# UCL-CCS/Nbed

Measured on AMD Instinct MI355X. Metric: embedded_scf_cycles_per_sec, higher is better.
Workload: dtype f64

## Files before the change

### include/nbx.h

```cpp
#ifndef NBX_H
#define NBX_H

#include <stddef.h>
#include <stdint.h>

#ifdef __cplusplus
extern "C" {
#endif

#define NBX_VERSION 3

#define NBX_OK 0
#define NBX_E_INVALID (-1)
#define NBX_E_HIP (-2)
#define NBX_E_NOMEM (-3)
#define NBX_E_NOCONV (-4)
#define NBX_E_UNSUPPORTED (-5)

typedef struct nbx_ctx nbx_ctx;

int nbx_version(void);
int nbx_experimental(void);
const char* nbx_last_error(void);
int nbx_device_count(int* count);
// ... 10 lines not shown
int nbx_memcpy_d2d(nbx_ctx* ctx, void* d_dst, const void* d_src, size_t bytes);
int nbx_memset(nbx_ctx* ctx, void* d_ptr, int value, size_t bytes);

size_t nbx_jk_df_worksize(int64_t nao, int64_t ndm, int64_t nocc_max);
int nbx_jk_df(nbx_ctx* ctx, int64_t nao, int64_t naux, const double* d_b, int64_t ndm, const double* d_c,
              const int64_t* nocc, double* d_jk, void* d_work, size_t work_bytes);
int nbx_df_synth(nbx_ctx* ctx, int64_t nao, int64_t l0, int64_t l1, uint64_t seed, double scale, double* d_b);

#define NBX_PROF_JK_DENSE 0
#define NBX_PROF_AO2MO_Q1 1
#define NBX_PROF_AO2MO 2
#define NBX_PROF_EIGH 3
#define NBX_PROF_SVD 4
#define NBX_PROF_GEMM 5
#define NBX_PROF_LOC 6
int nbx_profile_enable(nbx_ctx* ctx, int on);
int nbx_profile_sample(nbx_ctx* ctx, int every);
int nbx_debug_fill_lds(nbx_ctx* ctx, double value);
int nbx_profile_read(nbx_ctx* ctx, int slot, double* ms_sum, int64_t* count);
int nbx_profile_reset(nbx_ctx* ctx);

int nbx_synth_eri(nbx_ctx* ctx, int64_t nao, int64_t p0, int64_t p1, uint64_t seed, double* d_eri);

size_t nbx_jk_dense_worksize(int64_t nao, int64_t np, int64_t ndm);
int nbx_jk_dense(nbx_ctx* ctx, int64_t nao, int64_t p0, int64_t p1, const double* d_eri,
                 const double* d_dm, int64_t ndm, double* d_jk, void* d_work, size_t work_bytes);

size_t nbx_jk_dense_sym_worksize(int64_t nao, int64_t p0, int64_t p1, int64_t ndm);
int nbx_jk_dense_sym(nbx_ctx* ctx, int64_t nao, int64_t p0, int64_t p1, const double* d_eri,
                     const double* d_dm, int64_t ndm, double* d_jk, void* d_work, size_t work_bytes);

int nbx_jk_packed_supported(int64_t nao);
int nbx_jk_packed_fold(int64_t nao);
size_t nbx_eri_packed_bytes(int64_t nao, int64_t p0, int64_t p1);
int nbx_eri_pack(nbx_ctx* ctx, int64_t nao, int64_t p0, int64_t p1, const double* d_eri, double* d_packed);
size_t nbx_jk_packed_worksize(int64_t nao, int64_t p0, int64_t p1, int64_t ndm);
int nbx_jk_packed(nbx_ctx* ctx, int64_t nao, int64_t p0, int64_t p1, const double* d_packed,
                  const double* d_dm, int64_t ndm, double* d_jk, void* d_work, size_t work_bytes);

size_t nbx_jk_dts_bytes(int64_t nao);
int nbx_jk_dts_init(nbx_ctx* ctx, int64_t nao, double* d_dts);
int nbx_jk_packed_fock(nbx_ctx* ctx, int64_t nao, const double* d_packed, const double* d_dm,
                       const double* d_hv, double* d_jk, double* d_fock, double* d_vhf, void* d_work,
                       size_t work_bytes, const double* d_dts);

int nbx_jk_synth(nbx_ctx* ctx, int64_t nao, int64_t p0, int64_t p1, uint64_t seed, const double* d_dm,
                 int64_t ndm, double* d_jk, void* d_work, size_t work_bytes);

size_t nbx_jk_synth_sym_worksize(int64_t nao, int64_t p0, int64_t p1, int64_t ndm);
int nbx_jk_synth_sym(nbx_ctx* ctx, int64_t nao, int64_t p0, int64_t p1, uint64_t seed,
                     const double* d_dm, int64_t ndm, double* d_jk, void* d_work, size_t work_bytes);

int nbx_gemm(nbx_ctx* ctx, char trans_a, char trans_b, int64_t m, int64_t n, int64_t k,
             double alpha, const double* d_a, int64_t lda, int64_t stride_a,
             const double* d_b, int64_t ldb, int64_t stride_b, double beta,
             double* d_c, int64_t ldc, int64_t stride_c, int64_t batch);

int nbx_fock_uhf(nbx_ctx* ctx, int64_t nao, const double* d_hcore, int hcore_ndim,
                 const double* d_vemb, const double* d_jk, double* d_fock, double* d_vhf);
int nbx_huzinaga_sym(nbx_ctx* ctx, int64_t nao, int64_t batch, const double* d_fds, double kappa,
                     double* d_hz, double* d_fock_io);
int nbx_huzinaga_fused(nbx_ctx* ctx, int64_t nao, int64_t batch, const double* d_f, const double* d_ds, double kappa,
                       double* d_hz, double* d_fock_out);
int nbx_trace_prod(nbx_ctx* ctx, int64_t nao, int64_t batch, const double* d_a, const double* d_b,
                   double* h_out);
int nbx_huz_cycle_scalars(nbx_ctx* ctx, int64_t nao, const double* d_hcore, int hcore_ndim,
                          const double* d_vemb, const double* d_vhf, const double* d_hz,
                          const double* d_dm, const double* d_dm_old, double* h_out);
int nbx_huz_cycle_scalars_dev(nbx_ctx* ctx, int64_t nao, const double* d_hcore, int hcore_ndim,
                              const double* d_vemb, const double* d_vhf, const double* d_hz,
                              const double* d_dm, const double* d_dm_old, double* d_out,
                              const int* d_tail, int64_t tail_n);
int nbx_huz_cycle_scalars_dts(nbx_ctx* ctx, int64_t nao, const double* d_hcore, int hcore_ndim,
                              const double* d_vemb, const double* d_vhf, const double* d_hz,
                              const double* d_dm, const double* d_dm_old, double* d_out, const int* d_tail,
                              int64_t tail_n, double* d_dts);
size_t nbx_diis_coef_doubles(int64_t space);
int nbx_diis_update(nbx_ctx* ctx, int64_t n, int64_t space, int64_t slot, int64_t nd,
                    const double* d_x, double* d_xprev, double* d_xs, double* d_es, double* d_h,
                    double* d_coef);
int nbx_diis_update_err(nbx_ctx* ctx, int64_t n, int64_t space, int64_t slot, int64_t nd,
                        const double* d_x, const double* d_err, double* d_xprev, double* d_xs,
                        double* d_es, double* d_h, double* d_coef);
int nbx_vo_sumsq(nbx_ctx* ctx, int64_t nao, const double* d_fmo, int64_t nocc_a, int64_t nocc_b,
                 double* d_out);
int nbx_axpby(nbx_ctx* ctx, int64_t n, double a, const double* d_x, double b, double* d_y);
int nbx_lincomb(nbx_ctx* ctx, int64_t n, int64_t nvec, const double* h_coef, const double* d_vecs,
                int64_t stride, double* d_out);
int nbx_dots(nbx_ctx* ctx, int64_t n, int64_t nvec, const double* d_x, const double* d_vecs,
             int64_t stride, double* h_out);
int nbx_transpose(nbx_ctx* ctx, int64_t rows, int64_t cols, int64_t batch, const double* d_a,
                  double* d_b);
int nbx_scale_cols(nbx_ctx* ctx, int64_t rows, int64_t cols, int64_t batch, const double* d_s,
                   double* d_a);

size_t nbx_eigh_worksize(int64_t n, int64_t batch);
int nbx_eigh(nbx_ctx* ctx, int64_t n, int64_t batch, const double* d_a, double* d_w, double* d_v,
             void* d_work, size_t work_bytes);
int nbx_eigh_warm(nbx_ctx* ctx, int64_t n, int64_t batch, const double* d_a, const double* d_v0,
                  double* d_w, double* d_v, void* d_work, size_t work_bytes);
int nbx_eigh_warm_ex(nbx_ctx* ctx, int64_t n, int64_t batch, const double* d_a, const double* d_v0,
                     double* d_w, double* d_v, void* d_work, size_t work_bytes, int refine_iters);
size_t nbx_eigh_status_offset(int64_t n, int64_t batch);
int nbx_eigh_status(nbx_ctx* ctx, int64_t n, int64_t batch, const void* d_work, int* h_sweeps);
size_t nbx_eigh_approx_worksize(int64_t n, int64_t batch);
int nbx_eigh_approx(nbx_ctx* ctx, int64_t n, int64_t batch, const double* d_a, double* d_w, double* d_v,
                    void* d_work, size_t work_bytes, int* d_status);
size_t nbx_sym_pow_worksize(int64_t n);
size_t nbx_sym_pow_ns_worksize(int64_t n);
int nbx_sym_pow_ns(nbx_ctx* ctx, int64_t n, const double* d_s, double p, double c, double* d_out, void* d_work,
                   size_t work_bytes, int max_iter, int check_every, int* h_iters);
int nbx_sym_pow(nbx_ctx* ctx, int64_t n, const double* d_s, double p, double* d_out,
                void* d_work, size_t work_bytes);

size_t nbx_svd_worksize(int64_t m, int64_t n);
int nbx_svd_right(nbx_ctx* ctx, int64_t m, int64_t n, const double* d_a, double* d_s, double* d_vt,
                  void* d_work, size_t work_bytes);
size_t nbx_geig_refine_worksize(int64_t n, int64_t batch);
int nbx_geig_refine(nbx_ctx* ctx, int64_t n, int64_t batch, const double* d_f, const double* d_s,
                    const double* d_c0, double* d_w, double* d_c, int* d_status, void* d_work,
                    size_t work_bytes, int max_iter);

size_t nbx_ao2mo_pair_sym_worksize(int64_t nao, int64_t n, int64_t n4, int64_t n6);
size_t nbx_eri_rs_bytes(int64_t nao);
int nbx_eri_pack_rs(nbx_ctx* ctx, int64_t nao, const double* d_eri, double* d_out);
size_t nbx_ao2mo_pair_sym_rs_worksize(int64_t nao, int64_t n, int64_t n4, int64_t n6);
int nbx_ao2mo_pair_sym_rs(nbx_ctx* ctx, int64_t nao, const double* d_eri_rs, const double* d_c12, int64_t n,
                          const double* d_c3, int64_t n3, const double* d_c4, int64_t n4, double* d_out,
                          const double* d_c5, int64_t n5, const double* d_c6, int64_t n6, double* d_out2,
                          void* d_work, size_t work_bytes);
int nbx_ao2mo_pair_sym(nbx_ctx* ctx, int64_t nao, const double* d_eri, const double* d_c12, int64_t n,
                       const double* d_c3, int64_t n3, const double* d_c4, int64_t n4, double* d_out,
                       const double* d_c5, int64_t n5, const double* d_c6, int64_t n6, double* d_out2,
                       void* d_work, size_t work_bytes);

int nbx_svd_status(nbx_ctx* ctx, int64_t m, int64_t n, const void* d_work, int* h_sweeps);

#define NBX_LOC_PM 0
#define NBX_LOC_BOYS 1
size_t nbx_loc_worksize(int kind, int batch, int64_t nao, int64_t n, int64_t natm);
int nbx_loc_pm(nbx_ctx* ctx, int batch, int64_t nao, int64_t n, int64_t natm, const int64_t* h_ao_offsets,
               const double* d_x, const double* d_y, double* d_u, int max_sweeps, double tol, void* d_work,
               size_t work_bytes);
int nbx_loc_boys(nbx_ctx* ctx, int batch, int64_t n, const double* d_q, double* d_u, int max_sweeps, double tol,
                 void* d_work, size_t work_bytes);
int nbx_loc_status(nbx_ctx* ctx, int batch, const void* d_work, int* h_sweeps, double* h_f);

size_t nbx_ao2mo_worksize(int64_t nao, int64_t ni, int64_t n2, int64_t n3, int64_t n4);
int nbx_ao2mo(nbx_ctx* ctx, int64_t nao, const double* d_eri, const double* d_c1, int64_t n1,
              int64_t i0, int64_t i1, const double* d_c2, int64_t n2, const double* d_c3,
              int64_t n3, const double* d_c4, int64_t n4, double* d_out, void* d_work,
              size_t work_bytes);
size_t nbx_ao2mo_pair_worksize(int64_t nao, int64_t ni, int64_t n2, int64_t n4, int64_t n6);
int nbx_ao2mo_pair(nbx_ctx* ctx, int64_t nao, const double* d_eri, const double* d_c1, int64_t n1,
                   int64_t i0, int64_t i1, const double* d_c2, int64_t n2, const double* d_c3,
                   int64_t n3, const double* d_c4, int64_t n4, double* d_out, const double* d_c5,
                   int64_t n5, const double* d_c6, int64_t n6, double* d_out2, void* d_work,
                   size_t work_bytes);
size_t nbx_ao2mo_synth_worksize(int64_t nao, int64_t n1, int64_t n2, int64_t n3, int64_t n4);
size_t nbx_ao2mo_synth_pair_worksize(int64_t nao, int64_t n1, int64_t n2, int64_t n3, int64_t n4,
                                     int64_t n5, int64_t n6);
int nbx_ao2mo_synth_pair(nbx_ctx* ctx, int64_t nao, uint64_t seed, int64_t r0, int64_t r1,
                         const double* d_c1, int64_t n1, const double* d_c2, int64_t n2,
                         const double* d_c3, int64_t n3, const double* d_c4, int64_t n4, double* d_out,
                         const double* d_c5, int64_t n5, const double* d_c6, int64_t n6, double* d_out2,
                         void* d_work, size_t work_bytes);
// ... 104 lines not shown
```

### nbed_amd/_nbx.py

```python

from __future__ import annotations

import ctypes
import os
from ctypes import POINTER, c_char, c_char_p, c_double, c_int, c_int64, c_size_t, c_uint64, c_void_p
from pathlib import Path

LIB_NAME = "libnbx.so"
LIB_PATH = Path(__file__).resolve().parent / LIB_NAME

NBX_VERSION = 3
NBX_OK = 0
NBX_E_INVALID = -1
NBX_E_HIP = -2
NBX_E_NOMEM = -3
NBX_E_NOCONV = -4
NBX_E_UNSUPPORTED = -5
LOC_PM, LOC_BOYS = 0, 1

HUZ_JK_PACKED, HUZ_JK_SYM = 0, 1
XC_CODES = {"slater": 0, "lda": 1, "lda,vwn_rpa": 1, "lda,vwn": 2, "lda,vwn5": 2, "svwn": 2, "b3lyp": 3}

PROF_JK_DENSE, PROF_AO2MO_Q1, PROF_AO2MO, PROF_EIGH, PROF_SVD, PROF_GEMM = range(6)


class NbxError(RuntimeError):

    def __init__(self, code: int, message: str):
        super().__init__(f"libnbx error {code}: {message}")
        self.code = code


class NbxUnavailableError(RuntimeError):
    """libnbx.so is not built or no MI355X is visible: the HIP path cannot run."""


class HuzState(ctypes.Structure):

    _fields_ = [
        ("nao", c_int64), ("nocc_a", c_int64), ("nocc_b", c_int64),
        ("d_packed", c_void_p), ("d_hv", c_void_p), ("d_ds", c_void_p), ("d_sb", c_void_p), ("d_x", c_void_p),
        ("d_dts", c_void_p), ("d_jk", c_void_p), ("d_fock", c_void_p), ("d_vhf", c_void_p), ("d_fock2", c_void_p),
        ("d_tmp", c_void_p), ("d_fo", c_void_p),
        ("d_jk_work", c_void_p), ("jk_work_bytes", c_size_t),
        ("d_eig_work", c_void_p), ("eig_work_bytes", c_size_t),
        ("d_geig_work", c_void_p), ("geig_work_bytes", c_size_t),
        ("diis_space", c_int64), ("d_diis_xs", c_void_p), ("d_diis_es", c_void_p), ("d_diis_h", c_void_p),
        ("d_diis_coef", c_void_p), ("d_diis_xprev", c_void_p),
        ("jk_kind", c_int64), ("jk_p0", c_int64), ("jk_p1", c_int64), ("d_eri", c_void_p),
    ]


_P = c_void_p
SIGNATURES = {
    "nbx_version": (c_int, []),
    "nbx_experimental": (c_int, []),
    "nbx_last_error": (c_char_p, []),
    "nbx_device_count": (c_int, [POINTER(c_int)]),
    "nbx_ctx_create": (c_int, [c_int, _P, c_int, POINTER(_P)]),
    "nbx_ctx_destroy": (c_int, [_P]),
    "nbx_ctx_set_stream": (c_int, [_P, _P]),
    "nbx_sync": (c_int, [_P]),
    "nbx_malloc": (c_int, [_P, c_size_t, POINTER(_P)]),
    "nbx_free": (c_int, [_P, _P]),
    "nbx_memcpy_h2d": (c_int, [_P, _P, _P, c_size_t]),
    "nbx_memcpy_d2h": (c_int, [_P, _P, _P, c_size_t]),
    "nbx_gather_to_host": (c_int, [_P, c_int64, _P, _P, _P, c_int]),
    "nbx_jk_df_worksize": (c_size_t, [c_int64, c_int64, c_int64]),
    "nbx_jk_df": (c_int, [_P, c_int64, c_int64, _P, c_int64, _P, POINTER(c_int64), _P, _P, c_size_t]),
    "nbx_df_synth": (c_int, [_P, c_int64, c_int64, c_int64, c_uint64, c_double, _P]),
    "nbx_memcpy_d2d": (c_int, [_P, _P, _P, c_size_t]),
    "nbx_memset": (c_int, [_P, _P, c_int, c_size_t]),
    "nbx_profile_enable": (c_int, [_P, c_int]),
    "nbx_profile_sample": (c_int, [_P, c_int]),
    "nbx_debug_fill_lds": (c_int, [_P, c_double]),
    "nbx_profile_read": (c_int, [_P, c_int, POINTER(c_double), POINTER(c_int64)]),
    "nbx_profile_reset": (c_int, [_P]),
    "nbx_synth_eri": (c_int, [_P, c_int64, c_int64, c_int64, c_uint64, _P]),
    "nbx_jk_dense_worksize": (c_size_t, [c_int64, c_int64, c_int64]),
    "nbx_jk_dense": (c_int, [_P, c_int64, c_int64, c_int64, _P, _P, c_int64, _P, _P, c_size_t]),
    "nbx_jk_dense_sym_worksize": (c_size_t, [c_int64, c_int64, c_int64, c_int64]),
    "nbx_jk_packed_supported": (c_int, [c_int64]),
    "nbx_jk_packed_fold": (c_int, [c_int64]),
    "nbx_eri_packed_bytes": (c_size_t, [c_int64, c_int64, c_int64]),
    "nbx_eri_pack": (c_int, [_P, c_int64, c_int64, c_int64, _P, _P]),
    "nbx_jk_packed_worksize": (c_size_t, [c_int64, c_int64, c_int64, c_int64]),
    "nbx_huzinaga_fused": (c_int, [_P, c_int64, c_int64, _P, _P, c_double, _P, _P]),
    "nbx_jk_packed_fock": (c_int, [_P, c_int64, _P, _P, _P, _P, _P, _P, _P, c_size_t, _P]),
    "nbx_jk_dts_bytes": (c_size_t, [c_int64]),
    "nbx_jk_dts_init": (c_int, [_P, c_int64, _P]),
    "nbx_jk_packed": (c_int, [_P, c_int64, c_int64, c_int64, _P, _P, c_int64, _P, _P, c_size_t]),
    "nbx_jk_dense_sym": (c_int, [_P, c_int64, c_int64, c_int64, _P, _P, c_int64, _P, _P, c_size_t]),
    "nbx_jk_synth_sym_worksize": (c_size_t, [c_int64, c_int64, c_int64, c_int64]),
    "nbx_jk_synth_sym": (c_int, [_P, c_int64, c_int64, c_int64, c_uint64, _P, c_int64, _P, _P, c_size_t]),
    "nbx_jk_synth": (c_int, [_P, c_int64, c_int64, c_int64, c_uint64, _P, c_int64, _P, _P, c_size_t]),
    "nbx_gemm": (c_int, [_P, c_char, c_char, c_int64, c_int64, c_int64, c_double, _P, c_int64, c_int64,
                         _P, c_int64, c_int64, c_double, _P, c_int64, c_int64, c_int64]),
    "nbx_fock_uhf": (c_int, [_P, c_int64, _P, c_int, _P, _P, _P, _P]),
    "nbx_huzinaga_sym": (c_int, [_P, c_int64, c_int64, _P, c_double, _P, _P]),
    "nbx_trace_prod": (c_int, [_P, c_int64, c_int64, _P, _P, POINTER(c_double)]),
    "nbx_huz_cycle_scalars": (c_int, [_P, c_int64, _P, c_int, _P, _P, _P, _P, _P, POINTER(c_double)]),
    "nbx_huz_cycle_scalars_dev": (c_int, [_P, c_int64, _P, c_int, _P, _P, _P, _P, _P, _P, _P, c_int64]),
    "nbx_huz_cycle_scalars_dts": (c_int, [_P, c_int64, _P, c_int, _P, _P, _P, _P, _P, _P, _P, c_int64, _P]),
    "nbx_diis_coef_doubles": (c_size_t, [c_int64]),
    "nbx_diis_update": (c_int, [_P, c_int64, c_int64, c_int64, c_int64, _P, _P, _P, _P, _P, _P]),
    "nbx_diis_update_err": (c_int, [_P, c_int64, c_int64, c_int64, c_int64, _P, _P, _P, _P, _P, _P, _P]),
    "nbx_vo_sumsq": (c_int, [_P, c_int64, _P, c_int64, c_int64, _P]),
    "nbx_axpby": (c_int, [_P, c_int64, c_double, _P, c_double, _P]),
    "nbx_lincomb": (c_int, [_P, c_int64, c_int64, POINTER(c_double), _P, c_int64, _P]),
    "nbx_dots": (c_int, [_P, c_int64, c_int64, _P, _P, c_int64, POINTER(c_double)]),
    "nbx_transpose": (c_int, [_P, c_int64, c_int64, c_int64, _P, _P]),
    "nbx_scale_cols": (c_int, [_P, c_int64, c_int64, c_int64, _P, _P]),
    "nbx_eigh_worksize": (c_size_t, [c_int64, c_int64]),
    "nbx_eigh": (c_int, [_P, c_int64, c_int64, _P, _P, _P, _P, c_size_t]),
    "nbx_eigh_warm": (c_int, [_P, c_int64, c_int64, _P, _P, _P, _P, _P, c_size_t]),
    "nbx_geig_refine_worksize": (c_size_t, [c_int64, c_int64]),
    "nbx_geig_refine": (c_int, [_P, c_int64, c_int64, _P, _P, _P, _P, _P, _P, _P, c_size_t, c_int]),
    "nbx_eigh_warm_ex": (c_int, [_P, c_int64, c_int64, _P, _P, _P, _P, _P, c_size_t, c_int]),
    "nbx_eigh_status_offset": (c_size_t, [c_int64, c_int64]),
    "nbx_eigh_approx_worksize": (c_size_t, [c_int64, c_int64]),
    "nbx_eigh_approx": (c_int, [_P, c_int64, c_int64, _P, _P, _P, _P, c_size_t, _P]),
    "nbx_eigh_status": (c_int, [_P, c_int64, c_int64, _P, POINTER(c_int)]),
    "nbx_sym_pow_worksize": (c_size_t, [c_int64]),
    "nbx_sym_pow": (c_int, [_P, c_int64, _P, c_double, _P, _P, c_size_t]),
    "nbx_sym_pow_ns_worksize": (c_size_t, [c_int64]),
    "nbx_sym_pow_ns": (c_int, [_P, c_int64, _P, c_double, c_double, _P, _P, c_size_t, c_int, c_int, POINTER(c_int)]),
    "nbx_svd_worksize": (c_size_t, [c_int64, c_int64]),
    "nbx_svd_right": (c_int, [_P, c_int64, c_int64, _P, _P, _P, _P, c_size_t]),
    "nbx_svd_status": (c_int, [_P, c_int64, c_int64, _P, POINTER(c_int)]),
    "nbx_loc_worksize": (c_size_t, [c_int, c_int, c_int64, c_int64, c_int64]),
    "nbx_loc_pm": (c_int, [_P, c_int, c_int64, c_int64, c_int64, _P, _P, _P, _P, c_int, c_double, _P, c_size_t]),
    "nbx_loc_boys": (c_int, [_P, c_int, c_int64, _P, _P, c_int, c_double, _P, c_size_t]),
    "nbx_loc_status": (c_int, [_P, c_int, _P, POINTER(c_int), POINTER(c_double)]),
    "nbx_ao2mo_worksize": (c_size_t, [c_int64, c_int64, c_int64, c_int64, c_int64]),
    "nbx_ao2mo": (c_int, [_P, c_int64, _P, _P, c_int64, c_int64, c_int64, _P, c_int64, _P, c_int64, _P,
                          c_int64, _P, _P, c_size_t]),
    "nbx_ao2mo_pair_worksize": (c_size_t, [c_int64, c_int64, c_int64, c_int64, c_int64]),
    "nbx_ao2mo_pair": (c_int, [_P, c_int64, _P, _P, c_int64, c_int64, c_int64, _P, c_int64, _P, c_int64, _P, c_int64,
                               _P, _P, c_int64, _P, c_int64, _P, _P, c_size_t]),
    "nbx_ao2mo_pair_sym_worksize": (c_size_t, [c_int64, c_int64, c_int64, c_int64]),
    "nbx_ao2mo_pair_sym": (c_int, [_P, c_int64, _P, _P, c_int64, _P, c_int64, _P, c_int64, _P, _P, c_int64, _P, c_int64,
                                   _P, _P, c_size_t]),
    "nbx_eri_rs_bytes": (c_size_t, [c_int64]),
    "nbx_eri_pack_rs": (c_int, [_P, c_int64, _P, _P]),
    "nbx_ao2mo_pair_sym_rs_worksize": (c_size_t, [c_int64, c_int64, c_int64, c_int64]),
    "nbx_ao2mo_pair_sym_rs": (c_int, [_P, c_int64, _P, _P, c_int64, _P, c_int64, _P, c_int64, _P, _P, c_int64, _P,
                                      c_int64, _P, _P, c_size_t]),
    "nbx_ao2mo_synth_pair_worksize": (c_size_t, [c_int64] * 7),
    "nbx_ao2mo_synth_pair": (c_int, [_P, c_int64, c_uint64, c_int64, c_int64, _P, c_int64, _P, c_int64, _P, c_int64,
                                     _P, c_int64, _P, _P, c_int64, _P, c_int64, _P, _P, c_size_t]),
    "nbx_ao2mo_synth_worksize": (c_size_t, [c_int64, c_int64, c_int64, c_int64, c_int64]),
    "nbx_ao2mo_synth": (c_int, [_P, c_int64, c_uint64, c_int64, c_int64, _P, c_int64, _P, c_int64, _P, c_int64, _P,
                                c_int64, _P, _P, c_size_t]),
    "nbx_chem_to_phys": (c_int, [_P, c_int64, c_int64, c_int64, c_int64, _P, _P]),
    "nbx_spinorb_scatter_h1": (c_int, [_P, c_int64, _P, c_double, _P]),
    "nbx_spinorb_scatter_range": (c_int, [_P, c_int64, _P, c_double, c_double, c_int64, c_int64, _P]),
    "nbx_spinorb_scatter": (c_int, [_P, c_int64, _P, _P, c_double, c_double, _P, _P]),
    "nbx_threshold_scale": (c_int, [_P, c_int64, c_double, c_double, _P]),
    "nbx_becke_share": (c_int, [_P, c_int64, _P, c_int64, _P, _P, _P, c_int64, _P]),
    "nbx_eval_ao": (c_int, [_P, c_int64, _P, c_int64, _P, _P, _P, _P, _P, c_int64, c_int64, _P, _P]),
    "nbx_xc_rho": (c_int, [_P, c_int64, c_int64, _P, _P, _P, _P, _P]),
    "nbx_xc_functional_worksize": (c_size_t, [c_int64]),
    "nbx_xc_functional": (c_int, [_P, c_int, c_int64, _P, _P, _P, c_double, _P, _P, _P, _P, c_size_t]),
    "nbx_xc_vmat_worksize": (c_size_t, [c_int64, c_int64]),
    "nbx_xc_vmat": (c_int, [_P, c_int64, c_int64, _P, _P, _P, _P, _P, _P, c_size_t]),
    "nbx_purify_worksize": (c_size_t, [c_int64, c_int64]),
    "nbx_purify": (c_int, [_P, c_int64, c_int64, _P, c_int64, c_int64, _P, _P, c_size_t, c_int, _P]),
    "nbx_host_1e": (c_int, [c_int, _P, _P, _P, _P, _P, _P, _P, c_int, _P, _P, c_int, _P, _P, _P]),
    "nbx_host_eri": (c_int, [c_int, _P, _P, _P, _P, _P, _P, _P, c_double, c_int, _P]),
    "nbx_host_dipole": (c_int, [c_int, _P, _P, _P, _P, _P, _P, _P, c_int, _P]),
    "nbx_huz_cycle": (c_int, [_P, POINTER(HuzState), _P, _P, _P, _P, _P, _P, _P, c_int, c_int, c_int, c_int, c_int,
                              c_int, _P, _P]),
    "nbx_huz_cycle_jk": (c_int, [_P, POINTER(HuzState), _P]),
    "nbx_mu_cycle": (c_int, [_P, POINTER(HuzState), _P, _P, _P, _P, _P, _P, _P, _P, _P, c_int, c_int, c_int, c_int, c_int,
                             c_int, _P, _P]),
    "nbx_mu_cycle_solve": (c_int, [_P, POINTER(HuzState), _P, _P, _P, _P, _P, _P, _P, c_int, c_int, c_int, c_int, c_int,
                                   _P]),
    "nbx_mu_cycle_fock": (c_int, [_P, POINTER(HuzState), _P, _P, _P, _P, _P, c_int, _P, _P]),
    "nbx_mu_cycle_fock_post": (c_int, [_P, POINTER(HuzState), _P, _P, _P, _P, _P, c_int, _P, _P]),
    "nbx_huz_cycle_post": (c_int, [_P, POINTER(HuzState), _P, _P, _P, _P, _P, _P, _P, c_int, c_int, c_int, c_int, c_int,
                                   _P, _P]),
}

_lib = None


def load_library(path: os.PathLike | None = None) -> ctypes.CDLL:
    global _lib
    if _lib is not None and path is None:
# ... 34 lines not shown
```

### nbed_amd/backend.py

```python

from __future__ import annotations

import ctypes
import os
import time
from ctypes import c_double, c_int

import numpy as np

from . import _nbx
from ._nbx import NbxError, NbxUnavailableError

_default_backend = None


def get_backend(device: int | None = None):
    global _default_backend
    if _default_backend is None:
        _default_backend = HipBackend(device)
    return _default_backend


def set_backend(backend) -> None:
    global _default_backend
# ... 660 lines not shown
                       int(refine_iters), int(diis_mode), int(diis_slot), int(diis_nd), self._p(h_out),
                       self._p(out["status"]))
        return _PendingScalars(self.torch, None, 2, host=h_out)

    def mu_cycle_state(self, nao, nelec, packed, h1e, s_b, x, eri=None, p0: int = 0, p1: int | None = None):
        return self.huz_cycle_state(nao, nelec, packed, h1e, None, s_b, x, None, diis_space=8, eri=eri, p0=p0, p1=p1)

    def _pin_slot(self, n: int):
        h_out = self._pin_ring[self._pin_next][:n]
        h_out[n - 1] = 0.0
        self._pin_next = (self._pin_next + 1) % self._PIN_SLOTS
        return h_out

    def mu_cycle(self, h, dm_in, fock_in, c_in, out, tracked: bool, refine_iters: int, diis_on: bool, diis_slot: int,
                 diis_nd: int, want_grad: bool = True, reduce=None):
        ndt = 2 if want_grad else 0
        h_out = self._pin_slot(4 + 2 + ndt + 1)
        mode = 1 if tracked else 0
        if reduce is None:
            self._call("nbx_mu_cycle", ctypes.byref(h.st), self._p(dm_in), self._p(fock_in), self._p(c_in),
                       self._p(out["dm"]), self._p(out["fock"]), self._p(out["vhf"]), self._p(out["c"]), self._p(out["v"]),
                       self._p(out["w"]), mode, int(refine_iters), 1 if diis_on else 0, int(diis_slot), int(diis_nd),
                       1 if want_grad else 0, self._p(h_out), self._p(out["status"]))
        else:
            self._call("nbx_mu_cycle_solve", ctypes.byref(h.st), self._p(dm_in), self._p(fock_in), self._p(c_in),
                       self._p(out["dm"]), self._p(out["c"]), self._p(out["v"]), self._p(out["w"]), mode,
                       int(refine_iters), 1 if diis_on else 0, int(diis_slot), int(diis_nd), self._p(out["status"]))
            self._call("nbx_huz_cycle_jk", ctypes.byref(h.st), self._p(out["dm"]))
            reduce(h.jk)
            self._call("nbx_mu_cycle_fock_post", ctypes.byref(h.st), self._p(out["dm"]), self._p(dm_in),
                       self._p(out["c"]) if want_grad else None, self._p(out["fock"]), self._p(out["vhf"]), mode,
                       self._p(out["status"]), self._p(h_out))
        return _PendingScalars(self.torch, None, 2, host=h_out, ndtail=ndt)

    def mu_cycle_fock(self, h, dm, out, reduce=None):
        h_out = self._pin_slot(4 + 1)
        if reduce is None:
            self._call("nbx_mu_cycle_fock", ctypes.byref(h.st), self._p(dm), self._p(dm), None, self._p(out["fock"]),
                       self._p(out["vhf"]), -1, None, self._p(h_out))
        else:
            self._call("nbx_huz_cycle_jk", ctypes.byref(h.st), self._p(dm))
            reduce(h.jk)
            self._call("nbx_mu_cycle_fock_post", ctypes.byref(h.st), self._p(dm), self._p(dm), None,
                       self._p(out["fock"]), self._p(out["vhf"]), -1, None, self._p(h_out))
        return _PendingScalars(self.torch, None, 0, host=h_out)

    def df_synth(self, nao: int, l0: int, l1: int, scale: float | None = None, seed: int | None = None):
        from . import synth

        out = self.empty((l1 - l0, nao, nao))
        chunk = 32768
        for a in range(l0, l1, chunk):
            b = min(l1, a + chunk)
            self._call("nbx_df_synth", nao, a, b, int(synth.SEED if seed is None else seed),
                       float(synth.df_scale(nao) if scale is None else scale), self._p(out[a - l0:]))
        return out

    def jk_df(self, b, c, nocc):
        c3 = c if c.dim() == 3 else c.unsqueeze(0)
        ndm, n = int(c3.shape[0]), int(c3.shape[-1])
        occ = [int(x) for x in (nocc if hasattr(nocc, "__len__") else [nocc])]
        if len(occ) != ndm:
            raise ValueError(f"jk_df: {ndm} coefficient matrices but {len(occ)} occupation counts")
        out = self.empty((1 + ndm, n, n))
        nbytes = int(self.lib.nbx_jk_df_worksize(n, ndm, max(occ) if occ else 0))
        work = self._workspace("jk_df", nbytes)
        self._call("nbx_jk_df", n, int(b.shape[0]), self._p(b), ndm, self._p(c3), (ctypes.c_int64 * ndm)(*occ), self._p(out),
                   self._p(work), nbytes)
        return out

    def async_to_host(self, d_vals):
        return _PendingScalars(self.torch, d_vals, 0, ncore=int(d_vals.numel()))

    def diis_coef_buffer(self, space: int):
        return self.zeros(int(self.lib.nbx_diis_coef_doubles(space)))

    def diis_update(self, space: int, slot: int, nd: int, x, xprev, xs, es, h, coef):
        self._call("nbx_diis_update", x.numel(), space, slot, nd, self._p(x), self._p(xprev), self._p(xs),
                   self._p(es), self._p(h), self._p(coef))
        return xprev

    def diis_update_err(self, space: int, slot: int, nd: int, x, err, out, xs, es, h, coef):
        self._call("nbx_diis_update_err", x.numel(), space, slot, nd, self._p(x), self._p(err), self._p(out),
                   self._p(xs), self._p(es), self._p(h), self._p(coef))
        return out

    def vo_sumsq(self, fmo, nocc):
        out = self.empty(2)
        self._call("nbx_vo_sumsq", fmo.shape[-1], self._p(fmo), int(nocc[0]), int(nocc[1]), self._p(out))
        return out

    def axpby(self, a: float, x, b: float, y):
        self._call("nbx_axpby", x.numel(), a, self._p(x), b, self._p(y))
        return y

    def add(self, x, y):
        out = y.clone()
        return self.axpby(1.0, x, 1.0, out)

    def lincomb(self, coef, vecs, out=None):
        nvec, n = vecs.shape[0], vecs[0].numel()
        if out is None:
            out = self.empty(vecs.shape[1:])
        c = (c_double * nvec)(*[float(x) for x in coef])
        self._call("nbx_lincomb", n, nvec, c, self._p(vecs), n, self._p(out))
        return out

    def dots(self, x, vecs) -> np.ndarray:
        nvec, n = vecs.shape[0], x.numel()
        out = (c_double * nvec)()
        self._call("nbx_dots", n, nvec, self._p(x), self._p(vecs), vecs[0].numel(), out)
        return np.array(out[:], dtype=np.float64)

    def transpose(self, a):
        if a.dim() == 2:
            rows, cols, batch = a.shape[0], a.shape[1], 1
            out = self.empty((cols, rows))
        else:
            batch, rows, cols = a.shape
            out = self.empty((batch, cols, rows))
        self._call("nbx_transpose", rows, cols, batch, self._p(a), self._p(out))
        return out

    def scale_cols(self, a, s):
        rows, cols = a.shape[-2], a.shape[-1]
        batch = 1 if a.dim() == 2 else a.shape[0]
        self._call("nbx_scale_cols", rows, cols, batch, self._p(s), self._p(a))
        return a

    def eigh(self, a, check: bool = False, v0=None, refine_iters: int = 3):
        n = a.shape[-1]
        batch = 1 if a.dim() == 2 else a.shape[0]
        nbytes = self.lib.nbx_eigh_worksize(n, batch)
        work = self._workspace("eigh", nbytes)
        w = self.empty(a.shape[:-1])
        v = self.torch.empty_like(a)
        self._call("nbx_eigh_warm_ex", n, batch, self._p(a), self._p(v0), self._p(w), self._p(v), self._p(work),
                   work.numel(), int(refine_iters))
        off = self.lib.nbx_eigh_status_offset(n, batch)
        self.last_eigh_status_d = work[off:off + 4 * batch].view(self.torch.int32)
        if check:
            sweeps = (c_int * batch)()
            self._call("nbx_eigh_status", n, batch, self._p(work), sweeps)
            self.last_eigh_sweeps = list(sweeps)
        return w, v

    def eigh_approx(self, a):
        torch = self.torch
        a3 = a if a.dim() == 3 else a.reshape(1, *a.shape)
        batch, n = int(a3.shape[0]), int(a3.shape[-1])
        nbytes = int(self.lib.nbx_eigh_approx_worksize(n, batch))
        work = self._workspace("eigh_approx", nbytes)
        w = self.empty(a.shape[:-1])
        v = torch.empty_like(a)
        status = torch.empty(batch, dtype=torch.int32, device=self.device)
        self._call("nbx_eigh_approx", n, batch, self._p(a), self._p(w), self._p(v), self._p(work), nbytes, self._p(status))
        return w, v, status

    def geig_refine(self, fock, ovlp_b, c0, refine_iters: int = 1):
        n = fock.shape[-1]
        batch = 1 if fock.dim() == 2 else fock.shape[0]
        nbytes = self.lib.nbx_geig_refine_worksize(n, batch)
        work = self._workspace("geig", nbytes)
        w = self.empty(fock.shape[:-1])
        c = self.torch.empty_like(fock)
        status = self.torch.empty(batch, dtype=self.torch.int32, device=self.device)
# ... 346 lines not shown
```

### nbed_amd/csrc/ctx.hip

```cpp
#include "nbx_common.h"

static thread_local char g_err[512] = "";

void nbx_set_error(const char* fmt, ...) {
    va_list ap;
    va_start(ap, fmt);
    vsnprintf(g_err, sizeof(g_err), fmt, ap);
    va_end(ap);
}

extern "C" {

int nbx_version(void) { return NBX_VERSION; }

int nbx_experimental(void) {
#ifdef NBX_EXPERIMENTAL
    return 1;
#else
    return 0;
#endif
}

const char* nbx_last_error(void) { return g_err; }

int nbx_device_count(int* count) {
    NBX_CHECK_ARG(count != nullptr);
    int n = 0;
    hipError_t e = hipGetDeviceCount(&n);
    if (e != hipSuccess) {
        *count = 0;
        nbx_set_error("nbx_device_count: %s", hipGetErrorString(e));
        (void)hipGetLastError();
        return NBX_E_HIP;
    }
    *count = n;
    return NBX_OK;
}

int nbx_ctx_create(int device, void* stream, int private_stream, nbx_ctx** out) {
    NBX_CHECK_ARG(out != nullptr);
    NBX_CHECK_ARG(device >= 0);
    int n = 0;
    NBX_HIP(hipGetDeviceCount(&n));
    if (device >= n) {
        nbx_set_error("nbx_ctx_create: device %d not present (%d visible)", device, n);
        return NBX_E_INVALID;
    }
    NBX_HIP(hipSetDevice(device));
    {
        int lds_per_cu = 0;
        NBX_HIP(hipDeviceGetAttribute(&lds_per_cu, hipDeviceAttributeMaxSharedMemoryPerMultiprocessor, device));
        if (lds_per_cu <= 0 || lds_per_cu > 0x28000) {
            nbx_set_error("nbx_ctx_create: device %d reports %d bytes of LDS per CU; libnbx is built for gfx950 (163840) and "
                          "its packed J/K kernel relies on reads beyond 0x30000 returning zero", device, lds_per_cu);
            return NBX_E_UNSUPPORTED;
        }
    }
    nbx_ctx* c = new nbx_ctx();
    c->device = device;
    c->own_stream = (private_stream != 0);
    if (c->own_stream) {
        hipError_t e = hipStreamCreateWithFlags(&c->stream, hipStreamNonBlocking);
        if (e != hipSuccess) {
            delete c;
            nbx_set_error("nbx_ctx_create: hipStreamCreate -> %s", hipGetErrorString(e));
            return NBX_E_HIP;
        }
    } else {
        c->stream = reinterpret_cast<hipStream_t>(stream);
    }
    c->d_scratch = nullptr;
    c->h_pinned = nullptr;
    c->d_counters = nullptr;
    if (hipMalloc(reinterpret_cast<void**>(&c->d_scratch), NBX_SCRATCH_DOUBLES * sizeof(double)) != hipSuccess ||
        hipHostMalloc(reinterpret_cast<void**>(&c->h_pinned), NBX_SCRATCH_DOUBLES * sizeof(double), 0) != hipSuccess ||
        hipMalloc(reinterpret_cast<void**>(&c->d_counters), NBX_COUNTERS * sizeof(int)) != hipSuccess ||
        hipMemsetAsync(c->d_counters, 0, NBX_COUNTERS * sizeof(int), c->stream) != hipSuccess) {
        nbx_set_error("nbx_ctx_create: scratch allocation failed");
        if (c->d_scratch) (void)hipFree(c->d_scratch);
        if (c->h_pinned) (void)hipHostFree(c->h_pinned);
        if (c->d_counters) (void)hipFree(c->d_counters);
        if (c->own_stream) (void)hipStreamDestroy(c->stream);
        delete c;
        return NBX_E_NOMEM;
    }
    *out = c;
    return NBX_OK;
}

int nbx_ctx_destroy(nbx_ctx* ctx) {
    if (ctx == nullptr) return NBX_OK;
    (void)hipSetDevice(ctx->device);
    (void)hipStreamSynchronize(ctx->stream);
    (void)nbx_profile_reset(ctx);
    if (ctx->d_scratch) (void)hipFree(ctx->d_scratch);
    if (ctx->h_pinned) (void)hipHostFree(ctx->h_pinned);
    if (ctx->d_counters) (void)hipFree(ctx->d_counters);
    if (ctx->own_stream) (void)hipStreamDestroy(ctx->stream);
    delete ctx;
    return NBX_OK;
}

int nbx_ctx_set_stream(nbx_ctx* ctx, void* stream) {
    NBX_CHECK_ARG(ctx != nullptr);
    if (ctx->own_stream) {
        (void)hipStreamSynchronize(ctx->stream);
        (void)hipStreamDestroy(ctx->stream);
        ctx->own_stream = false;
    }
    ctx->stream = reinterpret_cast<hipStream_t>(stream);
    return NBX_OK;
}

int nbx_sync(nbx_ctx* ctx) {
    NBX_CHECK_ARG(ctx != nullptr);
    NBX_HIP(hipStreamSynchronize(ctx->stream));
    return NBX_OK;
}

int nbx_malloc(nbx_ctx* ctx, size_t bytes, void** d_ptr) {
    NBX_CHECK_ARG(ctx != nullptr && d_ptr != nullptr);
    NBX_HIP(hipSetDevice(ctx->device));
    hipError_t e = hipMalloc(d_ptr, bytes ? bytes : 8);
    if (e != hipSuccess) {
        nbx_set_error("nbx_malloc(%zu bytes): %s", bytes, hipGetErrorString(e));
        (void)hipGetLastError();
        return NBX_E_NOMEM;
    }
    return NBX_OK;
}

int nbx_free(nbx_ctx* ctx, void* d_ptr) {
    NBX_CHECK_ARG(ctx != nullptr);
    if (d_ptr == nullptr) return NBX_OK;
    NBX_HIP(hipFree(d_ptr));
    return NBX_OK;
}

int nbx_memcpy_h2d(nbx_ctx* ctx, void* d_dst, const void* h_src, size_t bytes) {
    NBX_CHECK_ARG(ctx != nullptr && (bytes == 0 || (d_dst != nullptr && h_src != nullptr)));
    if (bytes == 0) return NBX_OK;
    NBX_HIP(hipMemcpyAsync(d_dst, h_src, bytes, hipMemcpyHostToDevice, ctx->stream));
// ... 148 lines not shown
```

### nbed_amd/csrc/eigh_refine.hip

```cpp
#include "nbx_common.h"

namespace {

constexpr int RF_THREADS = 256;
constexpr int RF_WGS = 16;
constexpr int RF_MAX_ITER = 6;
constexpr int RF_UNROLL = 4;
constexpr double RF_TOL = 3.0e-8;
constexpr double RF_GIVE_UP = 0.25;
constexpr double RF_CLUSTER_NOISE = 1.0e-14;
constexpr double RF_NOISE = 8.0 * 1.1102230246251565e-16;
constexpr int RF_PART = 6;

__device__ __forceinline__ void publish(double* p, double v) {
    __hip_atomic_store(p, v, __ATOMIC_RELAXED, __HIP_MEMORY_SCOPE_AGENT);
}
__device__ __forceinline__ double peek(const double* p) {
    return __hip_atomic_load(p, __ATOMIC_RELAXED, __HIP_MEMORY_SCOPE_AGENT);
}

__global__ __launch_bounds__(RF_THREADS) void refine_e_kernel(int N, const double* __restrict__ A,
                                                              const double* __restrict__ S,
                                                              const double* __restrict__ G, double* __restrict__ Ep,
                                                              double* __restrict__ lam_out, int* __restrict__ status,
                                                              double* __restrict__ norm_a, int iter, int max_iter,
                                                              double* __restrict__ partial, int* __restrict__ counters,
                                                              int* __restrict__ final_status = nullptr,
                                                              const double* __restrict__ norm_part = nullptr,
                                                              int norm_tiles = 0) {
    extern __shared__ double sm[];
    double* lam = sm;
    double* red = sm + N;
    const int b = blockIdx.y, wg = blockIdx.x, nwg = gridDim.x;
    if (iter > 0 && status[b] != 0) return;
    const int64_t n2 = (int64_t)N * N;
    if (A != nullptr) A += b * n2;
    S += b * n2;
    G += b * n2;
    Ep += b * n2;
    double* part = partial + (int64_t)b * nwg * RF_PART;
    int* counter = counters + b;
    for (int i = threadIdx.x; i < N; i += RF_THREADS) lam[i] = S[(int64_t)i * N + i] / G[(int64_t)i * N + i];
    const int wave = threadIdx.x >> 6, lane = threadIdx.x & 63;
    constexpr int NW = RF_THREADS / 64;
    const int total = N * N;
    const int first = wg * RF_THREADS + threadIdx.x, stride = nwg * RF_THREADS;
    const float inv_n = 1.0f / (float)N;
    auto row_of = [&](int e) {
        int i = (int)((float)e * inv_n);
        i -= (i * N > e) ? 1 : 0;
        i += ((i + 1) * N <= e) ? 1 : 0;
        return i;
    };
    double off2 = 0.0, r2 = 0.0, a2 = 0.0;
    if (norm_part != nullptr) {
        const double* ps = norm_part + (int64_t)b * 2 * norm_tiles * 2;
        const double* pg = ps + (int64_t)norm_tiles * 2;
        for (int w = threadIdx.x; w < norm_tiles; w += RF_THREADS) {
            off2 += ps[2 * w];
            a2 += ps[2 * w + 1];
            r2 += pg[2 * w];
        }
    }
    __syncthreads();
    for (int e0 = first; e0 < total && norm_part == nullptr; e0 += stride * RF_UNROLL) {
        double sv[RF_UNROLL], gv[RF_UNROLL], av[RF_UNROLL];
#pragma unroll
        for (int u = 0; u < RF_UNROLL; ++u) {
            const int e = e0 + u * stride;
            const bool in = e < total;
            sv[u] = in ? S[e] : 0.0;
            gv[u] = in ? G[e] : 0.0;
            av[u] = (in && iter == 0) ? (A != nullptr ? A[e] : sv[u]) : 0.0;
        }
#pragma unroll
        for (int u = 0; u < RF_UNROLL; ++u) {
            const int e = e0 + u * stride;
            if (e < total) {
                const int i = row_of(e), j = e - i * N;
                const double r = (i == j) ? 1.0 - gv[u] : -gv[u];
                if (i != j) {
                    const double n1 = fabs(sv[u] - lam[j] * gv[u]), n2 = fabs(sv[u] - lam[i] * gv[u]);
                    const double nm = fmin(n1, n2);
                    off2 = fma(nm, nm, off2);
                }
                r2 = fma(r, r, r2);
                a2 = fma(av[u], av[u], a2);
            }
        }
    }
    off2 = nbx_wave_sum_dpp(off2);
    r2 = nbx_wave_sum_dpp(r2);
    a2 = nbx_wave_sum_dpp(a2);
    __syncthreads();
    if (lane == 0) {
        red[wave] = off2;
        red[NW + wave] = r2;
        red[2 * NW + wave] = a2;
    }
    __syncthreads();
    if (threadIdx.x == 0 && norm_part != nullptr) {
        double t0 = 0.0, t1 = 0.0, t2 = 0.0;
        for (int w = 0; w < NW; ++w) {
            t0 += red[w];
            t1 += red[NW + w];
            t2 += red[2 * NW + w];
        }
        red[3 * NW + 3] = 0.0;
        red[3 * NW + 0] = t0;
        red[3 * NW + 1] = t1;
        red[3 * NW + 2] = t2;
    } else if (threadIdx.x == 0) {
        double t0 = 0.0, t1 = 0.0, t2 = 0.0;
        for (int w = 0; w < NW; ++w) {
            t0 += red[w];
            t1 += red[NW + w];
            t2 += red[2 * NW + w];
        }
        publish(part + wg * RF_PART + 0, t0);
        publish(part + wg * RF_PART + 1, t1);
        publish(part + wg * RF_PART + 2, t2);
        __hip_atomic_fetch_add(counter, 1, __ATOMIC_RELEASE, __HIP_MEMORY_SCOPE_AGENT);
        int spins = 0;
        while (__hip_atomic_load(counter, __ATOMIC_ACQUIRE, __HIP_MEMORY_SCOPE_AGENT) < nwg && ++spins < (1 << 20))
            __builtin_amdgcn_s_sleep(2);
        red[3 * NW + 3] = (spins >= (1 << 20)) ? 1.0 : 0.0;
        t0 = t1 = t2 = 0.0;
        for (int w = 0; w < nwg; ++w) {
            t0 += peek(part + w * RF_PART + 0);
            t1 += peek(part + w * RF_PART + 1);
            t2 += peek(part + w * RF_PART + 2);
        }
        red[3 * NW + 0] = t0;
        red[3 * NW + 1] = t1;
        red[3 * NW + 2] = t2;
    }
    int unsorted = 0;
    if (final_status != nullptr)
        for (int i = threadIdx.x + 1; i < N; i += RF_THREADS) unsorted |= lam[i - 1] > lam[i] ? 1 : 0;
    unsorted = __syncthreads_or(unsorted);
    off2 = red[3 * NW + 0];
    r2 = red[3 * NW + 1];
    a2 = red[3 * NW + 2];
    double na;
    if (iter == 0) {
        na = sqrt(a2);
        if (wg == 0 && threadIdx.x == 0) norm_a[b] = na;
    } else {
        na = norm_a[b];
    }
    const double om_s = 2.0 * sqrt(off2), om_r = 2.0 * sqrt(r2);
    double emax = 0.0, cmax = 0.0, nmax = 0.0;
    for (int e0 = first; e0 < total; e0 += stride * RF_UNROLL) {
        double sv[RF_UNROLL], gv[RF_UNROLL], st[RF_UNROLL];
        int ri[RF_UNROLL];
#pragma unroll
        for (int u = 0; u < RF_UNROLL; ++u) {
            const int e = e0 + u * stride;
            const bool in = e < total;
            ri[u] = in ? row_of(e) : 0;
            sv[u] = in ? S[e] : 0.0;
            gv[u] = in ? G[e] : 0.0;
            st[u] = in ? S[(int64_t)(e - ri[u] * N) * N + ri[u]] : 0.0;
        }
#pragma unroll
        for (int u = 0; u < RF_UNROLL; ++u) {
            const int e = e0 + u * stride;
            if (e < total) {
                const int i = ri[u], j = e - i * N;
                const double sx = 0.5 * (sv[u] + st[u]), g = gv[u];
                double ev;
                if (i == j) {
                    ev = 0.5 * (1.0 - g);
                    emax = fmax(emax, fabs(ev));
                    Ep[e] = 1.0 + ev;
                } else {
                    const double li = lam[i], lj = lam[j];
                    const double d = lj - li;
                    if (fabs(d) > om_s + fmax(fabs(li), fabs(lj)) * om_r) {
                        const double num = sx - lj * g;
                        ev = num / d;
                        nmax = fmax(nmax, fabs(num));
                    } else {
                        ev = -0.5 * g;
                        cmax = fmax(cmax, fabs(sx));
                    }
                    emax = fmax(emax, fabs(ev));
                    Ep[e] = ev;
                }
            }
        }
    }
    emax = -nbx_wave_min_dpp(-emax);
    cmax = -nbx_wave_min_dpp(-cmax);
    nmax = -nbx_wave_min_dpp(-nmax);
    __syncthreads();
    if (lane == 0) {
        red[wave] = emax;
        red[NW + wave] = cmax;
        red[2 * NW + wave] = nmax;
    }
    __syncthreads();
    if (threadIdx.x == 0) {
        for (int w = 0; w < NW; ++w) {
            emax = fmax(emax, red[w]);
            cmax = fmax(cmax, red[NW + w]);
            nmax = fmax(nmax, red[2 * NW + w]);
        }
        if (red[3 * NW + 3] != 0.0) emax = 1.0e300;
        publish(part + wg * RF_PART + 3, emax);
        publish(part + wg * RF_PART + 4, cmax);
        publish(part + wg * RF_PART + 5, nmax);
        const int arrived = __hip_atomic_fetch_add(counter, 1, __ATOMIC_ACQ_REL, __HIP_MEMORY_SCOPE_AGENT);
        if (arrived == (norm_part != nullptr ? 1 : 2) * nwg - 1) {
            for (int w = 0; w < nwg; ++w) {
                emax = fmax(emax, peek(part + w * RF_PART + 3));
                cmax = fmax(cmax, peek(part + w * RF_PART + 4));
                nmax = fmax(nmax, peek(part + w * RF_PART + 5));
            }
            const bool at_noise = nmax <= RF_NOISE * sqrt((double)N) * na && emax < 1.0e-3;
            int st = 0;
            if (!(emax < RF_GIVE_UP)) st = -1;
            else if ((emax < RF_TOL || at_noise) && cmax <= RF_CLUSTER_NOISE * na) st = iter + 1;
            else if (iter == max_iter - 1) st = -1;
            if (final_status != nullptr) {
                if (st > 0 && unsorted) st = -3;
                final_status[b] = st > 0 ? 1000 + st : (st < 0 ? st : -2);
            }
            status[b] = st;
            __hip_atomic_store(counter, 0, __ATOMIC_RELEASE, __HIP_MEMORY_SCOPE_AGENT);
        }
    }
    if (wg == 0)
        for (int i = threadIdx.x; i < N; i += RF_THREADS) lam_out[(int64_t)b * N + i] = lam[i];
}

constexpr int RF_ROWS = 8;
__global__ __launch_bounds__(256) void refine_finish_kernel(int N, const double* __restrict__ xb0,
                                                            const double* __restrict__ xb1,
                                                            const double* __restrict__ lam_in,
                                                            const int* __restrict__ status, double* __restrict__ w,
                                                            double* __restrict__ v, int* __restrict__ jacobi_status) {
    extern __shared__ double sm[];
    double* lam = sm;
    int* rank = reinterpret_cast<int*>(sm + N);
    const int b = blockIdx.y;
    const int st = status[b];
    if (st <= 0) {
        if (blockIdx.x == 0 && threadIdx.x == 0 && jacobi_status != nullptr) jacobi_status[b] = st < 0 ? st : -2;
        return;
    }
    const int64_t n2 = (int64_t)N * N;
    const double* X = ((st & 1) ? xb1 : xb0) + b * n2;
    for (int i = threadIdx.x; i < N; i += blockDim.x) lam[i] = lam_in[(int64_t)b * N + i];
    __syncthreads();
    int unsorted = 0;
    for (int i = threadIdx.x + 1; i < N; i += blockDim.x) unsorted |= lam[i - 1] > lam[i] ? 1 : 0;
    unsorted = __syncthreads_or(unsorted);
    for (int i = threadIdx.x; i < N; i += blockDim.x) {
        const double li = lam[i];
        int r = i;
        if (unsorted) {
            r = 0;
            for (int j = 0; j < N; ++j) {
                const double lj = lam[j];
                r += (lj < li || (lj == li && j < i)) ? 1 : 0;
            }
        }
        rank[i] = r;
        if (blockIdx.x == 0) w[(int64_t)b * N + r] = li;
    }
    if (blockIdx.x == 0 && threadIdx.x == 0 && jacobi_status != nullptr) jacobi_status[b] = 1000 + st;
    __syncthreads();
    const int r0 = blockIdx.x * RF_ROWS;
    for (int rr = 0; rr < RF_ROWS; ++rr) {
        const int r = r0 + rr;
        if (r >= N) break;
        for (int i = threadIdx.x; i < N; i += blockDim.x)
            v[b * n2 + (int64_t)r * N + rank[i]] = X[(int64_t)r * N + i];
    }
}

size_t align256(size_t x) { return (x + 255) & ~(size_t)255; }

struct RefineLayout {
    size_t xb0, xb1, y, s, g, ep, lam, norm, partial, status, npart, total;
};

RefineLayout rlayout(int64_t n, int64_t batch) {
    RefineLayout L;
    const size_t mat = align256((size_t)(n * n * batch) * sizeof(double));
    size_t off = 0;
    L.xb0 = off; off += mat;
    L.xb1 = off; off += mat;
    L.y = off; off += mat;
    L.s = off; off += mat;
    L.g = off; off += mat;
    L.ep = off; off += mat;
    L.lam = off; off += align256((size_t)(n * batch) * sizeof(double));
    L.norm = off; off += align256((size_t)batch * sizeof(double));
    L.partial = off; off += align256((size_t)(batch * RF_WGS * RF_PART) * sizeof(double));
    L.status = off; off += align256((size_t)batch * sizeof(int));
    L.npart = off; off += align256((size_t)nbx_gemm_small_norm_doubles(n, n, batch) * sizeof(double));
    L.total = off;
    return L;
}

}

bool nbx_eigh_refine_supported(int64_t n, int64_t batch) {
    return n >= 2 && n <= 4096 && batch <= NBX_COUNTERS;
}

size_t nbx_eigh_refine_worksize(int64_t n, int64_t batch) { return rlayout(n, batch).total; }

int nbx_eigh_refine(nbx_ctx* ctx, int64_t n, int64_t batch, const double* d_a, const double* d_v0, double* d_w,
                    double* d_v, void* d_work, int* d_jacobi_status, const int** d_status_out, int max_iter) {
    NBX_CHECK_ARG(max_iter >= 1 && max_iter <= RF_MAX_ITER);
    const RefineLayout L = rlayout(n, batch);
    char* base = static_cast<char*>(d_work);
    double* xb[2] = {reinterpret_cast<double*>(base + L.xb0), reinterpret_cast<double*>(base + L.xb1)};
    double* y = reinterpret_cast<double*>(base + L.y);
    double* s = reinterpret_cast<double*>(base + L.s);
    double* g = reinterpret_cast<double*>(base + L.g);
    double* ep = reinterpret_cast<double*>(base + L.ep);
    double* lam = reinterpret_cast<double*>(base + L.lam);
    double* norm = reinterpret_cast<double*>(base + L.norm);
    double* partial = reinterpret_cast<double*>(base + L.partial);
    int* status = reinterpret_cast<int*>(base + L.status);
    double* npart = reinterpret_cast<double*>(base + L.npart);
    const int norm_tiles = (int)(nbx_cdiv(n, 16) * nbx_cdiv(n, 16));
    const int64_t n2 = n * n;
    const bool small = nbx_gemm_small_supported(n, n, n, batch);
    for (int it = 0; it < max_iter; ++it) {
        const double* src = (it == 0) ? d_v0 : xb[it & 1];
        double* dst = xb[(it + 1) & 1];
        const int* gate = (it == 0) ? nullptr : status;
        int rc = nbx_gemm_gated(ctx, 'N', 'N', n, n, n, 1.0, d_a, n, n2, src, n, n2, 0.0, y, n, n2, batch, gate, 0, 0);
        if (rc != NBX_OK) return rc;
        if (small) {
            rc = nbx_gemm_small_gated(ctx, 'T', 'N', n, n, n, 1.0, src, n, n2, y, n, n2, 0.0, s, n, n2, batch, gate, 0, 0,
                                      src, g, npart);
            if (rc != NBX_OK) return rc;
        } else {
            rc = nbx_gemm_gated(ctx, 'T', 'N', n, n, n, 1.0, src, n, n2, y, n, n2, 0.0, s, n, n2, batch, gate, 0, 0);
            if (rc != NBX_OK) return rc;
            rc = nbx_gemm_gated(ctx, 'T', 'N', n, n, n, 1.0, src, n, n2, src, n, n2, 0.0, g, n, n2, batch, gate, 0, 0);
            if (rc != NBX_OK) return rc;
        }
        hipLaunchKernelGGL(refine_e_kernel, dim3(RF_WGS, (unsigned)batch), dim3(RF_THREADS),
                           (size_t)(n + 3 * (RF_THREADS / 64) + 8) * sizeof(double), ctx->stream, (int)n, d_a, s, g, ep,
                           lam, status, norm, it, max_iter, partial, ctx->d_counters, static_cast<int*>(nullptr),
                           small ? npart : static_cast<const double*>(nullptr), norm_tiles);
        NBX_LAUNCH_CHECK();
        rc = nbx_gemm_gated(ctx, 'N', 'N', n, n, n, 1.0, src, n, n2, ep, n, n2, 0.0, dst, n, n2, batch, status, 0, it + 1);
        if (rc != NBX_OK) return rc;
    }
    hipLaunchKernelGGL(refine_finish_kernel, dim3((unsigned)nbx_cdiv(n, RF_ROWS), (unsigned)batch), dim3(256),
                       (size_t)n * sizeof(double) + (size_t)n * sizeof(int), ctx->stream, (int)n, xb[0], xb[1], lam,
                       status, d_w, d_v, d_jacobi_status);
    NBX_LAUNCH_CHECK();
    *d_status_out = status;
    return NBX_OK;
}

namespace {
struct GeigLayout {
    size_t cb0, cb1, yt, zt, s, g, ep, lam, norm, partial, status, npart, total;
};
GeigLayout glayout(int64_t n, int64_t batch) {
    GeigLayout L;
    const size_t mat = align256((size_t)(n * n * batch) * sizeof(double));
    size_t off = 0;
    L.cb0 = off; off += mat;
    L.cb1 = off; off += mat;
    L.yt = off; off += mat;
    L.zt = off; off += mat;
    L.s = off; off += mat;
    L.g = off; off += mat;
    L.ep = off; off += mat;
    L.lam = off; off += align256((size_t)(n * batch) * sizeof(double));
    L.norm = off; off += align256((size_t)batch * sizeof(double));
    L.partial = off; off += align256((size_t)(batch * RF_WGS * RF_PART) * sizeof(double));
    L.status = off; off += align256((size_t)batch * sizeof(int));
    L.npart = off; off += align256((size_t)nbx_gemm_small_norm_doubles(n, n, batch) * sizeof(double));
    L.total = off;
    return L;
}
}

extern "C" size_t nbx_geig_refine_worksize(int64_t n, int64_t batch) {
    if (n <= 0 || batch <= 0) return 0;
    return glayout(n, batch).total;
}

extern "C" int nbx_geig_refine(nbx_ctx* ctx, int64_t n, int64_t batch, const double* d_f, const double* d_s,
                               const double* d_c0, double* d_w, double* d_c, int* d_status, void* d_work,
                               size_t work_bytes, int max_iter) {
    NBX_CHECK_ARG(ctx && d_f && d_s && d_c0 && d_w && d_c && d_status);
    NBX_CHECK_ARG(n >= 2 && n <= 4096 && batch >= 1 && batch <= NBX_COUNTERS);
    NBX_CHECK_ARG(max_iter >= 1 && max_iter <= RF_MAX_ITER);
    const GeigLayout L = glayout(n, batch);
    if (d_work == nullptr || work_bytes < L.total) {
        nbx_set_error("nbx_geig_refine: workspace %zu < %zu bytes", work_bytes, L.total);
        return NBX_E_NOMEM;
    }
    char* base = static_cast<char*>(d_work);
    double* cb[2] = {reinterpret_cast<double*>(base + L.cb0), reinterpret_cast<double*>(base + L.cb1)};
    double* yt = reinterpret_cast<double*>(base + L.yt);
    double* zt = reinterpret_cast<double*>(base + L.zt);
    double* s = reinterpret_cast<double*>(base + L.s);
    double* g = reinterpret_cast<double*>(base + L.g);
    double* ep = reinterpret_cast<double*>(base + L.ep);
    double* lam = reinterpret_cast<double*>(base + L.lam);
    double* norm = reinterpret_cast<double*>(base + L.norm);
    double* partial = reinterpret_cast<double*>(base + L.partial);
    int* status = reinterpret_cast<int*>(base + L.status);
    double* npart = reinterpret_cast<double*>(base + L.npart);
    const int norm_tiles = (int)(nbx_cdiv(n, 16) * nbx_cdiv(n, 16));
    const int64_t n2 = n * n;
    const bool pair = nbx_gemm_small_supported(n, n, n, 2 * batch);
    const bool direct = max_iter == 1 && d_c != d_c0;
    for (int it = 0; it < max_iter; ++it) {
        const double* src = (it == 0) ? d_c0 : cb[it & 1];
        double* dst = direct ? d_c : cb[(it + 1) & 1];
        const int* gate = (it == 0) ? nullptr : status;
        int rc;
        if (pair) {
            rc = nbx_gemm_small_gated(ctx, 'T', 'N', n, n, n, 1.0, src, n, n2, d_f, n, n2, 0.0, yt, n, n2, batch, gate, 0,
                                      0, d_s, zt);
            if (rc != NBX_OK) return rc;
            rc = nbx_gemm_small_gated(ctx, 'T', 'T', n, n, n, 1.0, src, n, n2, yt, n, n2, 0.0, s, n, n2, batch, gate, 0, 0,
                                      zt, g, npart);
            if (rc != NBX_OK) return rc;
        } else {
            rc = nbx_gemm_gated(ctx, 'T', 'N', n, n, n, 1.0, src, n, n2, d_f, n, n2, 0.0, yt, n, n2, batch, gate, 0, 0);
            if (rc != NBX_OK) return rc;
            rc = nbx_gemm_gated(ctx, 'T', 'N', n, n, n, 1.0, src, n, n2, d_s, n, n2, 0.0, zt, n, n2, batch, gate, 0, 0);
            if (rc != NBX_OK) return rc;
            rc = nbx_gemm_gated(ctx, 'T', 'T', n, n, n, 1.0, src, n, n2, yt, n, n2, 0.0, s, n, n2, batch, gate, 0, 0);
            if (rc != NBX_OK) return rc;
            rc = nbx_gemm_gated(ctx, 'T', 'T', n, n, n, 1.0, src, n, n2, zt, n, n2, 0.0, g, n, n2, batch, gate, 0, 0);
            if (rc != NBX_OK) return rc;
        }
        hipLaunchKernelGGL(refine_e_kernel, dim3(RF_WGS, (unsigned)batch), dim3(RF_THREADS),
                           (size_t)(n + 3 * (RF_THREADS / 64) + 8) * sizeof(double), ctx->stream, (int)n,
                           static_cast<const double*>(nullptr), s, g, ep, direct ? d_w : lam, status, norm, it, max_iter,
                           partial, ctx->d_counters, direct ? d_status : static_cast<int*>(nullptr),
                           pair ? npart : static_cast<const double*>(nullptr), norm_tiles);
        NBX_LAUNCH_CHECK();
        rc = nbx_gemm_gated(ctx, 'N', 'N', n, n, n, 1.0, src, n, n2, ep, n, n2, 0.0, dst, n, n2, batch, status, 0, it + 1);
        if (rc != NBX_OK) return rc;
    }
    if (direct) return NBX_OK;
    hipLaunchKernelGGL(refine_finish_kernel, dim3((unsigned)nbx_cdiv(n, RF_ROWS), (unsigned)batch), dim3(256),
                       (size_t)n * sizeof(double) + (size_t)n * sizeof(int), ctx->stream, (int)n, cb[0], cb[1], lam,
                       status, d_w, d_c, d_status);
    NBX_LAUNCH_CHECK();
    return NBX_OK;
}
```

### nbed_amd/csrc/elementwise.hip

```cpp
#include "nbx_common.h"
#include "jk_m4_layout.h"
#include "jk_s4_layout.h"

namespace {

constexpr int TILE = 32;

__global__ void final_reduce_kernel(const double* __restrict__ partial, int nblocks, int nout,
                                    double* __restrict__ out, int sqrt_from, const int* __restrict__ tail = nullptr,
                                    int tail_n = 0) {
    __shared__ double red[17];
    if ((int)threadIdx.x < tail_n) out[nout + threadIdx.x] = (double)tail[threadIdx.x];
    for (int o = 0; o < nout; ++o) {
        double t = 0.0;
        for (int b = threadIdx.x; b < nblocks; b += blockDim.x) t += partial[(int64_t)b * nout + o];
        t = nbx_block_sum(t, red);
        if (threadIdx.x == 0) out[o] = (o >= sqrt_from) ? sqrt(t) : t;
        __syncthreads();
    }
}

__device__ __forceinline__ void load_tile(const double* __restrict__ M, int N, int r0, int c0,
                                          double (*lds)[TILE + 1]) {
    for (int r = threadIdx.y; r < TILE; r += blockDim.y) {
// ... 628 lines not shown
                    const double tmp = A0[k][lane];
                    A0[k][lane] = A0[piv][lane];
                    A0[piv][lane] = tmp;
                }
                if (lane == 0) {
                    const double tmp = rhs_s[k];
                    rhs_s[k] = rhs_s[piv];
                    rhs_s[piv] = tmp;
                }
            }
            __syncthreads();
            const double inv = 1.0 / A0[k][k];
            const int rem = m - 1 - k;
            double upd[DIIS_SLOTS];
            double rupd = 0.0;
#pragma unroll
            for (int e = 0; e < DIIS_SLOTS; ++e) {
                const int idx = lane + 64 * e;
                upd[e] = 0.0;
                if (idx < rem * rem) {
                    const int i = k + 1 + idx / rem, jj = k + 1 + idx % rem;
                    const double f = A0[i][k] * inv;
                    upd[e] = A0[i][jj] - f * A0[k][jj];
                }
            }
            if (lane < rem) {
                const double f = A0[k + 1 + lane][k] * inv;
                rupd = rhs_s[k + 1 + lane] - f * rhs_s[k];
            }
            __syncthreads();
#pragma unroll
            for (int e = 0; e < DIIS_SLOTS; ++e) {
                const int idx = lane + 64 * e;
                if (idx < rem * rem) A0[k + 1 + idx / rem][k + 1 + idx % rem] = upd[e];
            }
            if (lane < rem) rhs_s[k + 1 + lane] = rupd;
            __syncthreads();
        }
        __syncthreads();
        if (!lu_failed) {
            for (int i = m - 1; i >= 0; --i) {
                double t = (lane > i && lane < m) ? A0[i][lane] * c_out[lane] : 0.0;
                t = nbx_wave_sum(t);
                if (lane == 0) c_out[i] = (rhs_s[i] - t) / A0[i][i];
                __syncthreads();
            }
        }
        __syncthreads();
    }
    if (singular || lu_failed) {
        if (lane < m) {
            double t = 0.0;
            for (int k = 0; k < m; ++k)
                if (!singular || fabs(w[k]) > 1e-14) t += V[lane][k] * (1.0 / w[k]) * V[0][k];
            c_out[lane] = t;
        }
        __syncthreads();
    }
    if (lane >= 1 && lane < m) coef[lane - 1] = c_out[lane];
}

__device__ __forceinline__ void diis_rotation(double app, double aqq, double apq, double& cs, double& sn) {
    const double d = aqq - app, b = 2.0 * apq;
    const double inv = __builtin_amdgcn_rcp(fmax(fabs(d), fabs(b)));
    const double ds = d * inv, bs = b * inv;
    const float dsf = (float)ds, bsf = (float)bs;
    const float rt = __builtin_amdgcn_sqrtf(fmaf(dsf, dsf, bsf * bsf));
    const float den = dsf + (ds >= 0.0 ? rt : -rt);
    double t = (double)(bsf * __builtin_amdgcn_rcpf(den));
    const float rgp = __builtin_amdgcn_rcpf((float)fma(bs, t, ds));
    double g = fma(fma(bs, t, 2.0 * ds), t, -bs);
    t = fma(-0.5 * g, (double)rgp, t);
    g = fma(fma(bs, t, 2.0 * ds), t, -bs);
    t = fma(-0.5 * g, (double)rgp, t);
    const double x = fma(t, t, 1.0), h = 0.5 * x;
    double y = (double)__builtin_amdgcn_rsqf((float)x);
    y = y * fma(-(h * y), y, 1.5);
    y = y * fma(-(h * y), y, 1.5);
    const bool rot = fabs(apq) > 1e-290;
    cs = rot ? y : 1.0;
    sn = rot ? t * y : 0.0;
}

__device__ __forceinline__ void diis_jacobi8(double& a, double& v, int m, double fro, int lane, double* As,
                                             double* Vs) {
    const int r = lane >> 3, c = lane & 7;
    for (int sweep = 0; sweep < 40; ++sweep) {
        const double off = nbx_wave_sum_dpp((r < c) ? a * a : 0.0);
        if (off <= 1e-31 * fro) break;
        const double mind = nbx_wave_min_dpp((r == c && r < m) ? fabs(a) : 1.0e300);
        if (mind - sqrt(2.0 * off) > 1.0e-14) break;
#pragma unroll
        for (int step = 0; step < 7; ++step) {
            auto mate = [&](int k) {
                int x = 2 * step - k;
                x += x < 0 ? 7 : 0;
                x -= x >= 7 ? 7 : 0;
                return k == 7 ? step : (k == step ? 7 : x);
            };
            const int mc = mate(c), mr = mate(r);
            As[lane] = a;
            Vs[lane] = v;
            __syncthreads();
            const double a_cc = As[9 * c], a_mm = As[9 * mc], a_cm = As[8 * min(c, mc) + max(c, mc)];
            const double a_rr = As[9 * r], a_nn = As[9 * mr], a_rn = As[8 * min(r, mr) + max(r, mr)];
            const double a_rmc = As[8 * r + mc], a_mrc = As[8 * mr + c], a_mrmc = As[8 * mr + mc];
            const double v_rmc = Vs[8 * r + mc];
            __syncthreads();
            double cc, sc, cr, sr;
            diis_rotation(c < mc ? a_cc : a_mm, c < mc ? a_mm : a_cc, a_cm, cc, sc);
            diis_rotation(r < mr ? a_rr : a_nn, r < mr ? a_nn : a_rr, a_rn, cr, sr);
            const double ks_c = (c < mc) ? -sc : sc, ks_r = (r < mr) ? -sr : sr;
            const double x = cc * a + ks_c * a_rmc;
            const double y = cc * a_mrc + ks_c * a_mrmc;
            a = (ks_r != 0.0 && mr == c) ? 0.0 : cr * x + ks_r * y;
            v = cc * v + ks_c * v_rmc;
        }
    }
}

constexpr int DIIS8_PER_LANE = 4;
__global__ __launch_bounds__(64) void diis_solve8_lincomb_kernel(const double* __restrict__ partial, int nblocks,
                                                                 int nd, int slot, double* __restrict__ H, int ldh,
                                                                 double* __restrict__ coef,
                                                                 double* __restrict__ state, int64_t n,
                                                                 const double* __restrict__ vecs, int64_t stride,
                                                                 double* __restrict__ out) {
    __shared__ double As[64], Vs[64], Ts[64];
    __shared__ double A0[8][9], rhs_s[8], c_out[8];
    __shared__ int lu_failed;
    const int lane = threadIdx.x, r = lane >> 3, c = lane & 7;
    const int m = nd + 1;
    const int64_t i0 = (int64_t)blockIdx.x * (64 * DIIS8_PER_LANE) + lane;
    const bool inside = r < m && c < m;
    const bool new_row = inside && r == slot + 1 && c >= 1, new_col = inside && c == slot + 1 && r >= 1;
    const double hold = (inside && !new_row && !new_col) ? H[(int64_t)r * ldh + c] : 0.0;
    double xv[DIIS8_PER_LANE][7];
#pragma unroll
    for (int j = 0; j < DIIS8_PER_LANE; ++j)
#pragma unroll
        for (int k = 0; k < 7; ++k) xv[j][k] = (k < nd && i0 + 64 * j < n) ? vecs[k * stride + i0 + 64 * j] : 0.0;
    const double v_prev = state[lane];
    const bool warm = __double_as_longlong(state[64]) == DIIS_STATE_MAGIC && state[65] <= (double)(nd + 1);
    double acc = 0.0;
    if (c >= 1 && c <= nd) {
#pragma unroll 4
        for (int b = r; b < nblocks; b += 8) acc += partial[(int64_t)b * nd + c - 1];
    }
    As[lane] = acc;
    __syncthreads();
    double row_c = 0.0, row_r = 0.0;
#pragma unroll
    for (int g = 0; g < 8; ++g) {
        row_c += As[8 * g + c];
        row_r += As[8 * g + r];
    }
    __syncthreads();
    double a = new_row ? row_c : (new_col ? row_r : hold);
    if (blockIdx.x == 0 && (new_row || new_col)) H[(int64_t)r * ldh + c] = a;
    A0[r][c] = a;
    if (lane == 0) lu_failed = 0;
    double v = (r == c) ? 1.0 : 0.0;
    if (warm) {
        Vs[lane] = v_prev;
        __syncthreads();
        double gram = 0.0;
#pragma unroll
        for (int k = 0; k < 8; ++k) gram = fma(Vs[8 * k + r], Vs[8 * k + c], gram);
        Ts[lane] = gram;
        __syncthreads();
        double vg = 0.0;
#pragma unroll
        for (int k = 0; k < 8; ++k) vg = fma(Vs[8 * r + k], Ts[8 * k + c], vg);
        v = 1.5 * v_prev - 0.5 * vg;
        __syncthreads();
        Vs[lane] = v;
        As[lane] = a;
        __syncthreads();
        double hv = 0.0;
#pragma unroll
        for (int k = 0; k < 8; ++k) hv = fma(As[8 * r + k], Vs[8 * k + c], hv);
        Ts[lane] = hv;
        __syncthreads();
        double vhv = 0.0;
#pragma unroll
        for (int k = 0; k < 8; ++k) vhv = fma(Vs[8 * k + r], Ts[8 * k + c], vhv);
        __syncthreads();
        Ts[lane] = vhv;
        __syncthreads();
        a = 0.5 * (vhv + Ts[8 * c + r]);
        __syncthreads();
    }
    const double fro = nbx_wave_sum_dpp(a * a);
    diis_jacobi8(a, v, m, fro, lane, As, Vs);
    As[lane] = a;
    Vs[lane] = v;
    if (blockIdx.x == 0) {
        state[DIIS_STATE_HALF + lane] = v;
        if (lane == 0) state[DIIS_STATE_HALF + 64] = __longlong_as_double(DIIS_STATE_MAGIC);
        if (lane == 1) state[DIIS_STATE_HALF + 65] = (double)m;
    }
    __syncthreads();
    const bool singular = __any(r == c && r < m && fabs(a) < 1e-14);
    if (!singular) {
        if (lane < m) rhs_s[lane] = (lane == 0) ? 1.0 : 0.0;
        __syncthreads();
        for (int k = 0; k < m; ++k) {
            double best = (lane >= k && lane < m) ? fabs(A0[lane][k]) : -1.0;
            int piv = lane;
#pragma unroll
            for (int o = 4; o > 0; o >>= 1) {
                const double ob = __shfl_xor(best, o);
                const int op = __shfl_xor(piv, o);
                if (ob > best || (ob == best && op < piv)) {
                    best = ob;
                    piv = op;
                }
            }
            best = nbx_readlane_f64(best, 0);
            piv = __builtin_amdgcn_readlane(piv, 0);
            if (best == 0.0) {
                if (lane == 0) lu_failed = 1;
                break;
            }
            if (piv != k) {
                if (lane < m) {
                    const double tmp = A0[k][lane];
                    A0[k][lane] = A0[piv][lane];
                    A0[piv][lane] = tmp;
                }
                if (lane == 0) {
                    const double tmp = rhs_s[k];
                    rhs_s[k] = rhs_s[piv];
                    rhs_s[piv] = tmp;
                }
            }
            __syncthreads();
            const double inv = 1.0 / A0[k][k];
            const bool below = r > k && r < m, right = c > k && c < m;
            double upd = 0.0, rupd = 0.0;
            if (below && right) upd = A0[r][c] - (A0[r][k] * inv) * A0[k][c];
            if (below && c == 0) rupd = rhs_s[r] - (A0[r][k] * inv) * rhs_s[k];
            __syncthreads();
            if (below && right) A0[r][c] = upd;
            if (below && c == 0) rhs_s[r] = rupd;
            __syncthreads();
        }
        __syncthreads();
        if (!lu_failed) {
            for (int i = m - 1; i >= 0; --i) {
                const double t = nbx_wave_sum_dpp((lane > i && lane < m) ? A0[i][lane] * c_out[lane] : 0.0);
                if (lane == 0) c_out[i] = (rhs_s[i] - t) / A0[i][i];
                __syncthreads();
            }
        }
        __syncthreads();
    }
    if (singular || lu_failed) {
        const double w = As[9 * c], v0 = Vs[c];
        const bool keep = c < m && (!singular || fabs(w) > 1e-14);
        const double t = nbx_sum8_dpp(keep ? v * (1.0 / w) * v0 : 0.0);
        if (c == 0 && r < m) c_out[r] = t;
        __syncthreads();
    }
    if (blockIdx.x == 0 && lane >= 1 && lane < m) coef[lane - 1] = c_out[lane];
    double cf[7];
#pragma unroll
    for (int k = 0; k < 7; ++k) cf[k] = (k < nd) ? c_out[k + 1] : 0.0;
#pragma unroll
    for (int j = 0; j < DIIS8_PER_LANE; ++j) {
        const int64_t i = i0 + 64 * j;
        if (i < n) {
            double t = 0.0;
#pragma unroll
            for (int k = 0; k < 7; ++k)
                if (k < nd) t = fma(cf[k], xv[j][k], t);
            out[i] = t;
        }
    }
}

__global__ void lincomb_dev_kernel(int64_t n, int nvec, const double* __restrict__ coef,
                                   const double* __restrict__ vecs, int64_t stride, double* __restrict__ out) {
    for (int64_t i = (int64_t)blockIdx.x * blockDim.x + threadIdx.x; i < n; i += (int64_t)gridDim.x * blockDim.x) {
        double t = 0.0;
        for (int k = 0; k < nvec; ++k) t = fma(coef[k], vecs[k * stride + i], t);
        out[i] = t;
    }
}

__global__ void transpose_kernel(const double* __restrict__ A, double* __restrict__ B, int64_t rows, int64_t cols) {
    __shared__ double t[TILE][TILE + 1];
    const int64_t b = blockIdx.z;
    A += b * rows * cols;
    B += b * rows * cols;
    const int64_t r0 = (int64_t)blockIdx.y * TILE, c0 = (int64_t)blockIdx.x * TILE;
    for (int r = threadIdx.y; r < TILE; r += blockDim.y) {
        const int64_t gr = r0 + r, gc = c0 + threadIdx.x;
        if (gr < rows && gc < cols) t[r][threadIdx.x] = A[gr * cols + gc];
    }
    __syncthreads();
    for (int c = threadIdx.y; c < TILE; c += blockDim.y) {
        const int64_t gc = c0 + c, gr = r0 + threadIdx.x;
        if (gr < rows && gc < cols) B[gc * rows + gr] = t[threadIdx.x][c];
    }
}

__global__ void vo_sumsq_kernel(const double* __restrict__ fmo, int N, int nocc_a, int nocc_b,
                                double* __restrict__ partial) {
    __shared__ double red[17];
    const int x = blockIdx.y;
    const int nocc = x == 0 ? nocc_a : nocc_b;
    const int nvir = N - nocc;
    const int64_t total = (int64_t)nvir * nocc;
    double t = 0.0;
    for (int64_t e = (int64_t)blockIdx.x * blockDim.x + threadIdx.x; e < total; e += (int64_t)gridDim.x * blockDim.x) {
        const int a = nocc + (int)(e / nocc), i = (int)(e % nocc);
        const double v = fmo[((int64_t)x * N + a) * N + i];
        t = fma(v, v, t);
    }
    t = nbx_block_sum(t, red);
    if (threadIdx.x == 0) partial[(int64_t)blockIdx.x * 2 + x] = t;
}

__global__ void scale_cols_kernel(int64_t rows, int64_t cols, const double* __restrict__ s, double* __restrict__ a) {
    const int64_t b = blockIdx.y;
    const int64_t i = (int64_t)blockIdx.x * blockDim.x + threadIdx.x;
    if (i >= rows * cols) return;
    a[b * rows * cols + i] *= s[b * cols + (i % cols)];
}

__global__ void spinorb_h2_kernel(int n, const double* __restrict__ tb, double tol, double scale,
                                  double* __restrict__ h2, int64_t idx0, int64_t count) {
    const int64_t nq = 2 * (int64_t)n;
    const int64_t n4 = (int64_t)n * n * n * n;
    for (int64_t off = (int64_t)blockIdx.x * blockDim.x + threadIdx.x; off < count;
         off += (int64_t)gridDim.x * blockDim.x) {
        const int64_t idx = idx0 + off;
        const int64_t S = idx % nq;
        int64_t t = idx / nq;
        const int64_t R = t % nq;
        t /= nq;
        const int64_t Q = t % nq;
        const int64_t P = t / nq;
        const int sp = (int)(P & 1), sq = (int)(Q & 1), sr = (int)(R & 1), ss = (int)(S & 1);
        int blk = -1;
        if (sp == sq && sq == sr && sr == ss) blk = sp;
        else if (sp == 0 && sq == 1 && sr == 1 && ss == 0) blk = 2;
        else if (sp == 1 && sq == 0 && sr == 0 && ss == 1) blk = 3;
        double v = 0.0;
        if (blk >= 0) {
            const int64_t p = P >> 1, q = Q >> 1, r = R >> 1, s = S >> 1;
            v = tb[blk * n4 + ((p * n + q) * n + r) * n + s];
            if (fabs(v) < tol) v = 0.0;
            v *= scale;
        }
        h2[off] = v;
    }
}

// ... 136 lines not shown
        m4 = (wl[2] << 8) | wl[3];
    }
    NBX_CHECK_ARG(d_dts == nullptr || lpt4 > 0);
    NBX_CHECK_ARG(tail_n >= 0 && tail_n <= 64 && (tail_n == 0 || d_tail != nullptr));
    NBX_CHECK_ARG(dtail_n >= 0 && dtail_n <= 64 && (dtail_n == 0 || d_dtail != nullptr));
    NBX_CHECK_ARG(hcore_ndim == 2 || hcore_ndim == 3);
    const bool fine = nbx_cdiv(nao, 16) * nbx_cdiv(nao, 16) * 4 <= NBX_SCRATCH_DOUBLES - 64;
    const int64_t g = nbx_cdiv(nao, fine ? 16 : TILE);
    NBX_CHECK_ARG(g * g * 4 <= NBX_SCRATCH_DOUBLES - 64);
    if (fine)
        hipLaunchKernelGGL(huz_scalars_kernel<16>, dim3((unsigned)g, (unsigned)g), dim3(16, 8), 0, ctx->stream, d_hcore,
                           hcore_ndim == 3 ? 1 : 0, d_vemb, d_vhf, d_hz, d_dm, d_dm_old, (int)nao, ctx->d_scratch,
                           d_out, d_tail, (int)tail_n, ctx->d_counters + NBX_COUNTERS - 1, d_dts, nb4, lpt4, m4, d_dtail,
                           (int)dtail_n);
    else
        hipLaunchKernelGGL(huz_scalars_kernel<TILE>, dim3((unsigned)g, (unsigned)g), dim3(TILE, 8), 0, ctx->stream,
                           d_hcore, hcore_ndim == 3 ? 1 : 0, d_vemb, d_vhf, d_hz, d_dm, d_dm_old, (int)nao,
                           ctx->d_scratch, d_out, d_tail, (int)tail_n, ctx->d_counters + NBX_COUNTERS - 1, d_dts, nb4,
                           lpt4, m4, d_dtail, (int)dtail_n);
    NBX_LAUNCH_CHECK();
    return NBX_OK;
}

int nbx_density_scalars_launch(nbx_ctx* ctx, int64_t nao, const double* d_hcore, int hcore_ndim, const double* d_vemb,
                               const double* d_vhf, const double* d_hz, const double* d_c, int64_t nocc_a, int64_t nocc_b,
                               double* d_dm_out, const double* d_dm_old, double* d_out, const int* d_tail, int64_t tail_n,
                               double* d_dts) {
    NBX_CHECK_ARG(ctx && d_hcore && d_vhf && d_c && d_dm_out && d_dm_old && d_out && nao > 0);
    const bool fine = nbx_cdiv(nao, 16) * nbx_cdiv(nao, 16) * 4 <= NBX_SCRATCH_DOUBLES - 64;
    if (!fine || nocc_a <= 0 || nocc_b <= 0 || nocc_a > 64 || nocc_b > 64) return NBX_E_UNSUPPORTED;
    int m4 = 0, nb4 = d_dts ? s4_nb(nao) : 0, lpt4 = d_dts ? s4_lpt(nao) : 0;
    if (d_dts && (nbx_jk_m8_covers(nao) || nbx_jk_m4_covers(nao))) {
        int wl[4];
        if (nbx_jk_m8_covers(nao)) nbx_jk_m8_weight_layout(nao, wl);
        else nbx_jk_m4_weight_layout(nao, wl);
        nb4 = wl[0];
        lpt4 = wl[1];
        m4 = (wl[2] << 8) | wl[3];
    }
    NBX_CHECK_ARG(d_dts == nullptr || lpt4 > 0);
    NBX_CHECK_ARG(tail_n >= 0 && tail_n <= 64 && (tail_n == 0 || d_tail != nullptr));
    NBX_CHECK_ARG(hcore_ndim == 2 || hcore_ndim == 3);
    const int64_t g = nbx_cdiv(nao, 16);
    hipLaunchKernelGGL((huz_scalars_kernel<16, true>), dim3((unsigned)g, (unsigned)g), dim3(16, 8), 0, ctx->stream, d_hcore,
                       hcore_ndim == 3 ? 1 : 0, d_vemb, d_vhf, d_hz, d_dm_out, d_dm_old, (int)nao, ctx->d_scratch, d_out,
                       d_tail, (int)tail_n, ctx->d_counters + NBX_COUNTERS - 1, d_dts, nb4, lpt4, m4, nullptr, 0, d_c,
                       (int)nocc_a, (int)nocc_b, d_dm_out);
    NBX_LAUNCH_CHECK();
    return NBX_OK;
}

int nbx_antisym(nbx_ctx* ctx, int64_t nao, int64_t batch, const double* d_a, double* d_out) {
    NBX_CHECK_ARG(ctx && d_a && d_out && d_a != d_out && nao > 0 && batch > 0 && batch < 65536);
    const unsigned g = (unsigned)nbx_cdiv(nao, TILE);
    hipLaunchKernelGGL(antisym_kernel, dim3(g, g, (unsigned)batch), dim3(TILE, 8), 0, ctx->stream, d_a, (int)nao, d_out);
    NBX_LAUNCH_CHECK();
    return NBX_OK;
}

extern "C" {

size_t nbx_diis_coef_doubles(int64_t space) { return space > 0 ? (size_t)(space + DIIS_STATE_DOUBLES) : 0; }

int nbx_diis_update(nbx_ctx* ctx, int64_t n, int64_t space, int64_t slot, int64_t nd, const double* d_x,
                    double* d_xprev, double* d_xs, double* d_es, double* d_h, double* d_coef) {
    return nbx_diis_update_err(ctx, n, space, slot, nd, d_x, nullptr, d_xprev, d_xs, d_es, d_h, d_coef);
}

int nbx_diis_update_err(nbx_ctx* ctx, int64_t n, int64_t space, int64_t slot, int64_t nd, const double* d_x,
                        const double* d_err, double* d_xprev, double* d_xs, double* d_es, double* d_h,
                        double* d_coef) {
    return nbx_diis_update_anti(ctx, n, space, slot, nd, d_x, d_err, 0, d_xprev, d_xs, d_es, d_h, d_coef);
}

}

int nbx_diis_update_anti(nbx_ctx* ctx, int64_t n, int64_t space, int64_t slot, int64_t nd, const double* d_x,
                         const double* d_err, int64_t anti_n, double* d_xprev, double* d_xs, double* d_es, double* d_h,
                         double* d_coef) {
    NBX_CHECK_ARG(ctx && d_x && d_xprev && d_xs && d_es && d_h && d_coef && n > 0);
    NBX_CHECK_ARG(anti_n == 0 || (d_err != nullptr && anti_n > 0 && n % (anti_n * anti_n) == 0));
    NBX_CHECK_ARG(space >= 1 && space <= DIIS_MAX_SPACE && slot >= 0 && slot < space && nd >= 1 && nd <= space &&
                  slot < nd);
    const unsigned blocks = grid1d(n, 256, 128);
    NBX_CHECK_ARG((int64_t)blocks * nd <= NBX_SCRATCH_DOUBLES - 64);
    hipLaunchKernelGGL(diis_push_kernel, dim3(blocks), dim3(256), 0, ctx->stream, n, (int)nd, (int)slot, d_x,
                       d_xprev, d_err, d_xs, d_es, ctx->d_scratch, d_coef + space, (int)anti_n);
    NBX_LAUNCH_CHECK();
    if (nd <= 7 && nbx_cdiv(n, 64 * DIIS8_PER_LANE) <= 65535) {
        hipLaunchKernelGGL(diis_solve8_lincomb_kernel, dim3((unsigned)nbx_cdiv(n, 64 * DIIS8_PER_LANE)), dim3(64), 0,
                           ctx->stream, ctx->d_scratch, (int)blocks, (int)nd, (int)slot, d_h, (int)(space + 1), d_coef,
                           d_coef + space, n, d_xs, n, d_xprev);
        NBX_LAUNCH_CHECK();
        return NBX_OK;
    }
    hipLaunchKernelGGL(diis_solve_kernel, dim3(1), dim3(64), 0, ctx->stream, ctx->d_scratch, (int)blocks, (int)nd,
                       (int)slot, d_h, (int)(space + 1), d_coef);
    NBX_LAUNCH_CHECK();
    hipLaunchKernelGGL(lincomb_dev_kernel, dim3(grid1d(n, 256)), dim3(256), 0, ctx->stream, n, (int)nd, d_coef, d_xs,
                       n, d_xprev);
    NBX_LAUNCH_CHECK();
    return NBX_OK;
}

extern "C" {

int nbx_vo_sumsq(nbx_ctx* ctx, int64_t nao, const double* d_fmo, int64_t nocc_a, int64_t nocc_b, double* d_out) {
    NBX_CHECK_ARG(ctx && d_fmo && d_out && nao > 0 && nocc_a >= 0 && nocc_a <= nao && nocc_b >= 0 && nocc_b <= nao);
    const int64_t na = (nao - nocc_a) * nocc_a, nb = (nao - nocc_b) * nocc_b;
    if ((na > nb ? na : nb) <= 16384) {
        hipLaunchKernelGGL(vo_sumsq_kernel, dim3(1, 2), dim3(256), 0, ctx->stream, d_fmo, (int)nao, (int)nocc_a, (int)nocc_b,
                           d_out);
        NBX_LAUNCH_CHECK();
        return NBX_OK;
    }
    const int blocks = 32;
    hipLaunchKernelGGL(vo_sumsq_kernel, dim3(blocks, 2), dim3(256), 0, ctx->stream, d_fmo, (int)nao, (int)nocc_a,
                       (int)nocc_b, ctx->d_scratch);
    NBX_LAUNCH_CHECK();
    hipLaunchKernelGGL(final_reduce_kernel, dim3(1), dim3(256), 0, ctx->stream, ctx->d_scratch, blocks, 2, d_out, 2);
    NBX_LAUNCH_CHECK();
    return NBX_OK;
}

int nbx_axpby(nbx_ctx* ctx, int64_t n, double a, const double* d_x, double b, double* d_y) {
    NBX_CHECK_ARG(ctx && n >= 0);
    if (n == 0) return NBX_OK;
    NBX_CHECK_ARG(d_x && d_y);
    hipLaunchKernelGGL(axpby_kernel, dim3(grid1d(n, 256)), dim3(256), 0, ctx->stream, n, a, d_x, b, d_y);
    NBX_LAUNCH_CHECK();
    return NBX_OK;
}

int nbx_lincomb(nbx_ctx* ctx, int64_t n, int64_t nvec, const double* h_coef, const double* d_vecs,
                int64_t stride, double* d_out) {
    NBX_CHECK_ARG(ctx && n >= 0 && nvec > 0 && nvec <= MAX_LINCOMB && h_coef && d_vecs && d_out);
    if (n == 0) return NBX_OK;
    Coefs cf;
    for (int k = 0; k < MAX_LINCOMB; ++k) cf.c[k] = k < nvec ? h_coef[k] : 0.0;
    hipLaunchKernelGGL(lincomb_kernel, dim3(grid1d(n, 256)), dim3(256), 0, ctx->stream, n, (int)nvec, cf, d_vecs,
                       stride, d_out);
    NBX_LAUNCH_CHECK();
    return NBX_OK;
}

int nbx_dots(nbx_ctx* ctx, int64_t n, int64_t nvec, const double* d_x, const double* d_vecs, int64_t stride,
             double* h_out) {
    NBX_CHECK_ARG(ctx && n > 0 && nvec > 0 && nvec <= MAX_LINCOMB && d_x && d_vecs && h_out);
    const unsigned blocks = grid1d(n, 256, 128);
    hipLaunchKernelGGL(dots_kernel, dim3(blocks), dim3(256), 0, ctx->stream, n, (int)nvec, d_x, d_vecs, stride,
                       ctx->d_scratch);
    NBX_LAUNCH_CHECK();
    return finish_reduction(ctx, (int)blocks, (int)nvec, h_out);
}

int nbx_transpose(nbx_ctx* ctx, int64_t rows, int64_t cols, int64_t batch, const double* d_a, double* d_b) {
    NBX_CHECK_ARG(ctx && rows >= 0 && cols >= 0 && batch >= 0);
    if (rows == 0 || cols == 0 || batch == 0) return NBX_OK;
    NBX_CHECK_ARG(d_a && d_b && d_a != d_b);
    const int64_t gy = nbx_cdiv(rows, TILE), gx = nbx_cdiv(cols, TILE);
    if (gy > 65535) {
        nbx_set_error("nbx_transpose: more than 65535*32 rows per matrix is unsupported");
        return NBX_E_UNSUPPORTED;
    }
    for (int64_t b0 = 0; b0 < batch; b0 += 65535) {
        const int64_t nb = (batch - b0) < 65535 ? (batch - b0) : 65535;
        hipLaunchKernelGGL(transpose_kernel, dim3((unsigned)gx, (unsigned)gy, (unsigned)nb), dim3(TILE, 8), 0,
                           ctx->stream, d_a + b0 * rows * cols, d_b + b0 * rows * cols, rows, cols);
// ... 66 lines not shown
```

### nbed_amd/csrc/jk_m8.hip

```cpp
#include <cstdlib>
#include <type_traits>

#include "jk_m8_layout.h"
#include "jk_m4_walk.h"
#include "nbx_common.h"

#pragma clang diagnostic ignored "-Winline-asm"

namespace {

constexpr int M8_THREADS = 512;
typedef __attribute__((address_space(3))) void* m8_lds_vp;
typedef double m8_d2 __attribute__((ext_vector_type(2)));

__host__ __device__ __forceinline__ int m8_tri_row(int64_t T) {
    int64_t p = (int64_t)((sqrt(8.0 * (double)T + 1.0) - 1.0) * 0.5);
    while (p * (p + 1) / 2 > T) --p;
    while ((p + 1) * (p + 2) / 2 <= T) ++p;
    return (int)p;
}

template <int K0, int K1, class F>
__device__ __forceinline__ void m8_for(F&& f) {
    if constexpr (K0 < K1) {
// ... 386 lines not shown
                sy += v[u].y;
            }
        }
        for (; w < W; w += 16) {
            const double2 v = at(w);
            sx += v.x;
            sy += v.y;
        }
        part[grp][l] = sx;
        part[grp][32 + l] = sy;
        __syncthreads();
        if (grp == 0) {
            double tx = part[0][l], ty = part[0][32 + l];
#pragma unroll
            for (int g = 1; g < 16; ++g) {
                tx += part[g][l];
                ty += part[g][32 + l];
            }
            *reinterpret_cast<double2*>(j2sum + e) = make_double2(tx, ty);
        }
        return;
    }
    const int row = (int)blockIdx.x % N, x = ((int)blockIdx.x / N) % ndm, bz = (int)blockIdx.x / (N * ndm);
    const int lane = threadIdx.x & 63, chunk = threadIdx.x >> 6;
    const int c = bz * 64 + lane;
    double t = 0.0;
    if (c < N) {
        const double* src = kpart2 + (int64_t)x * N + c;
        const int64_t stride = (int64_t)ndm * N;
        const int first = max(max(row + 1, c), p0);
        auto at = [&](int P) { return src[((int64_t)P * (P + 1) / 2 + row - t_begin) * stride]; };
        int P = first + chunk;
        for (; P + 7 * 8 < p0 + np; P += 8 * 8) {
            double v[8];
#pragma unroll
            for (int u = 0; u < 8; ++u) v[u] = at(P + 8 * u);
#pragma unroll
            for (int u = 0; u < 8; ++u) t += v[u];
        }
        for (; P < p0 + np; P += 8) t += at(P);
    }
    part[chunk][lane] = t;
    __syncthreads();
    if (chunk == 0 && c < N) {
        double tot = ((part[0][lane] + part[1][lane]) + (part[2][lane] + part[3][lane])) +
                     ((part[4][lane] + part[5][lane]) + (part[6][lane] + part[7][lane]));
        if (row >= p0 && row < p0 + np && c <= row) {
            const int trow = (int)(m4_tri(row) - t_begin);
            const int w_lo = m8_wg_of(rg, W, trow), w_hi = m8_wg_of(rg, W, trow + row);
            for (int w = w_lo; w <= w_hi; ++w) {
                if (rg.first[w + 1] <= rg.first[w]) continue;
                const int slot = row - m8_tri_row(t_begin + rg.first[w]);
                tot += kpart1[(((int64_t)w * S + slot) * ndm + x) * N + c];
            }
        }
        kpf[((int64_t)x * N + row) * N + c] = tot;
    }
}

template <class G>
__global__ __launch_bounds__(256) void m8_finish_kernel(const double* __restrict__ kpf, const double* __restrict__ j2sum,
                                                        double* __restrict__ jout, double* __restrict__ kout, int ndm,
                                                        const double* __restrict__ hv, double* __restrict__ fock,
                                                        double* __restrict__ vhf) {
    constexpr int N = G::N;
    const int i = blockIdx.x * 256 + threadIdx.x;
    if (i >= N * N) return;
    const int r = i / N, c = i - r * N;
    const int hi = r > c ? r : c, lo = r > c ? c : r;
    const double j = jout[i] + j2sum[m8_stage_index<G>(hi, lo)];
    for (int x = 0; x < ndm; ++x) {
        const double k = kpf[((int64_t)x * N + r) * N + c] + kpf[((int64_t)x * N + c) * N + r];
        const int64_t o = (int64_t)x * N * N + i;
        kout[o] = k;
        if (fock != nullptr) {
            const double v = j - k;
            fock[o] = hv[o] + v;
            if (vhf != nullptr) vhf[o] = v;
        }
    }
    jout[i] = j;
}

size_t m8_align256(size_t x) { return (x + 255) & ~(size_t)255; }

struct M8Plan {
    int wgs, S, lmax;
    size_t wt_off, k1_off, k2_off, jp_off, js_off, kpf_off, total, lds_bytes;
};

template <class G>
const M8Ranges& m8_ranges(int64_t p0, int64_t np, int* wgs_out) {
    static thread_local M8Ranges rg;
    static thread_local int64_t key_p0 = -1, key_np = -1;
    static thread_local int wgs = 0;
    if (key_p0 != p0 || key_np != np) {
        static const int tile_cost = getenv("NBX_M8_TC") ? atoi(getenv("NBX_M8_TC")) : 120;
        const int64_t t_begin = m4_tri((int)p0), t_end = m4_tri((int)(p0 + np));
        const int64_t ntiles = t_end - t_begin;
        wgs = (int)(ntiles < M8_CUS ? (ntiles > 0 ? ntiles : 1) : M8_CUS);
        auto cost_of_row = [&](int p) {
            return (int64_t)(m8_len<G>(p) / 16 + tile_cost);
        };
        int64_t total = 0;
        for (int p = (int)p0; p < (int)(p0 + np); ++p) total += (int64_t)(p + 1) * cost_of_row(p);
        int w = 0;
        int64_t before = 0;
        int64_t trel = 0;
        for (int p = (int)p0; p < (int)(p0 + np); ++p) {
            const int64_t c = cost_of_row(p);
            for (int q = 0; q <= p; ++q, ++trel) {
                while (w < wgs && before * wgs >= (int64_t)w * total) rg.first[w++] = (int)trel;
                before += c;
            }
        }
        while (w <= M8_CUS) rg.first[w++] = (int)ntiles;
        for (int k = 0; k < M8_MAXCH; ++k) rg.wmin[k] = wgs;
        for (int v = wgs - 1; v >= 0; --v) {
            if (rg.first[v + 1] <= rg.first[v]) continue;
            const int nkmax = m8_nk<G>(m8_tri_row(t_begin + rg.first[v + 1] - 1));
            for (int k = 0; k < nkmax && k < M8_MAXCH; ++k) rg.wmin[k] = v;
        }
        key_p0 = p0;
        key_np = np;
    }
    *wgs_out = wgs;
    return rg;
}

template <class G>
M8Plan m8_plan(int64_t p0, int64_t np, int64_t ndm) {
    M8Plan pl;
    const int64_t t_begin = m4_tri((int)p0), t_end = m4_tri((int)(p0 + np));
    const int64_t ntiles = t_end - t_begin;
    const M8Ranges& rg = m8_ranges<G>(p0, np, &pl.wgs);
    int S = 1, lmax = 1;
    for (int w = 0; w < pl.wgs; ++w) {
        const int64_t a = t_begin + rg.first[w], b = t_begin + rg.first[w + 1];
        if (b <= a) continue;
        const int rows = m8_tri_row(b - 1) - m8_tri_row(a) + 1;
        S = rows > S ? rows : S;
        lmax = (int)(b - a) > lmax ? (int)(b - a) : lmax;
    }
    pl.S = S;
    pl.lmax = lmax;
    pl.lds_bytes = (size_t)(G::RING * G::BUF + G::FIXED) * sizeof(double);
    const size_t jlen = (size_t)G::NCH * G::LP * M4_PROD_THREADS * 2;
    size_t off = 0;
    pl.wt_off = off; off += m8_align256(jlen * sizeof(double));
    pl.k1_off = off; off += m8_align256((size_t)((int64_t)pl.wgs * pl.S * ndm * G::N) * sizeof(double));
    pl.k2_off = off; off += m8_align256((size_t)(ntiles * ndm * G::N) * sizeof(double));
    pl.jp_off = off; off += m8_align256((size_t)pl.wgs * jlen * sizeof(double));
    pl.js_off = off; off += m8_align256(jlen * sizeof(double));
    pl.kpf_off = off; off += m8_align256((size_t)(ndm * G::N * G::N) * sizeof(double));
    pl.total = off;
    return pl;
}

template <int NB, int LP>
int m8_run(nbx_ctx* ctx, int64_t p0, int64_t p1, const double* d_packed, const double* d_dm, int64_t ndm, double* d_jk,
           void* d_work, const double* d_hv, double* d_fock, double* d_vhf, const double* d_wt_in) {
    using G = M8Geom<NB, LP>;
    const int64_t np = p1 - p0, N = G::N, n2 = N * N;
    const M8Plan pl = m8_plan<G>(p0, np, ndm);
    int wgs_;
    const M8Ranges& rg = m8_ranges<G>(p0, np, &wgs_);
    if (pl.lds_bytes > (size_t)M8_LDS_BYTES) {
        nbx_set_error("nbx_jk_m8: %zu bytes of LDS for N = %lld", pl.lds_bytes, (long long)N);
        return NBX_E_UNSUPPORTED;
    }
    char* base = static_cast<char*>(d_work);
    double* wt = reinterpret_cast<double*>(base + pl.wt_off);
    double* k1 = reinterpret_cast<double*>(base + pl.k1_off);
    double* k2 = reinterpret_cast<double*>(base + pl.k2_off);
    double* jp = reinterpret_cast<double*>(base + pl.jp_off);
    double* js = reinterpret_cast<double*>(base + pl.js_off);
    double* kpf = reinterpret_cast<double*>(base + pl.kpf_off);
    if (np < N) {
        const int rc = nbx_memset(ctx, d_jk, 0, (size_t)n2 * sizeof(double));
        if (rc != NBX_OK) return rc;
    }
    constexpr int JSLOTS = G::NCH * G::LP * M4_PROD_THREADS;
    if (d_wt_in != nullptr) {
        wt = const_cast<double*>(d_wt_in);
    } else {
        hipLaunchKernelGGL(m8_weights_kernel<G>, dim3((unsigned)nbx_cdiv(JSLOTS, 256)), dim3(256), 0, ctx->stream, d_dm, (int)ndm, wt);
        NBX_LAUNCH_CHECK();
    }
    const int64_t t_begin = m4_tri((int)p0);
    {
        nbx_prof_scope prof(ctx, NBX_PROF_JK_DENSE);
        static bool attr_set = false;
        if (!attr_set) {
            const hipError_t e1 = hipFuncSetAttribute(reinterpret_cast<const void*>(&jk_m8_kernel<NB, 1, LP>),
                                                      hipFuncAttributeMaxDynamicSharedMemorySize, M8_LDS_BYTES);
            const hipError_t e2 = hipFuncSetAttribute(reinterpret_cast<const void*>(&jk_m8_kernel<NB, 2, LP>),
                                                      hipFuncAttributeMaxDynamicSharedMemorySize, M8_LDS_BYTES);
            if (e1 != hipSuccess || e2 != hipSuccess) {
                nbx_set_error("nbx_jk_m8: hipFuncSetAttribute(%d bytes of LDS): %s", M8_LDS_BYTES,
                              hipGetErrorString(e1 != hipSuccess ? e1 : e2));
                return NBX_E_HIP;
            }
            attr_set = true;
        }
        if (ndm == 2)
            hipLaunchKernelGGL((jk_m8_kernel<NB, 2, LP>), dim3((unsigned)pl.wgs), dim3(M8_THREADS), pl.lds_bytes, ctx->stream,
                               d_packed, d_dm, wt, d_jk, k1, k2, jp, t_begin, rg, pl.S);
        else
            hipLaunchKernelGGL((jk_m8_kernel<NB, 1, LP>), dim3((unsigned)pl.wgs), dim3(M8_THREADS), pl.lds_bytes, ctx->stream,
                               d_packed, d_dm, wt, d_jk, k1, k2, jp, t_begin, rg, pl.S);
    }
    NBX_LAUNCH_CHECK();
    {
        const int jblocks = (int)nbx_cdiv(JSLOTS, 32);
        const int nkb = (int)(N * ndm * nbx_cdiv(N, 64));
        hipLaunchKernelGGL(m8_reduce_kernel<G>, dim3((unsigned)(nkb + jblocks)), dim3(512), 0, ctx->stream, k1, k2, jp, kpf, js,
                           (int)p0, (int)np, (int)ndm, t_begin, rg, pl.wgs, pl.S);
        NBX_LAUNCH_CHECK();
    }
    hipLaunchKernelGGL(m8_finish_kernel<G>, dim3((unsigned)nbx_cdiv(n2, 256)), dim3(256), 0, ctx->stream, kpf, js, d_jk, d_jk + n2,
                       (int)ndm, d_hv, d_fock, d_vhf);
    NBX_LAUNCH_CHECK();
    return NBX_OK;
}

}

#ifndef NBX_M8_SIZES
#define NBX_M8_SIZES(X) X(25) X(26) X(27) X(28) X(29) X(30) X(31) X(32) X(33) X(34) X(35) X(36) X(37)
#endif
#ifdef NBX_M8_LP
#define M8_LP(NB_) NBX_M8_LP
#else
#define M8_LP(NB_) m8_lp(NB_)
#endif
#define M8_DISPATCH(N_, EXPR)            \
    switch ((int)((N_) / 4)) {           \
        NBX_M8_SIZES(M8_CASE_##EXPR)     \
        default: break;                  \
    }
bool nbx_jk_m8_covers(int64_t N) {
    static const bool on = getenv("NBX_JK_M8") == nullptr || atoi(getenv("NBX_JK_M8")) != 0;
    if (!on || N % 4 != 0) return false;
#define M8_CASE_covers(NB_) case NB_: return true;
    M8_DISPATCH(N, covers)
#undef M8_CASE_covers
    return false;
}

size_t nbx_jk_m8_packed_bytes(int64_t N, int64_t p0, int64_t p1) {
    const int64_t t0 = m4_tri((int)p0), t1 = m4_tri((int)p1);
#define M8_CASE_bytes(NB_) \
    case NB_: return (size_t)(m8_tile_offset<M8Geom<NB_, M8_LP(NB_)>>(t1) - m8_tile_offset<M8Geom<NB_, M8_LP(NB_)>>(t0)) * sizeof(double) + 256;
    M8_DISPATCH(N, bytes)
#undef M8_CASE_bytes
    return 0;
}

size_t nbx_jk_m8_worksize(int64_t N, int64_t p0, int64_t p1, int64_t ndm) {
#define M8_CASE_work(NB_) case NB_: return m8_plan<M8Geom<NB_, M8_LP(NB_)>>(p0, p1 - p0, ndm).total;
    M8_DISPATCH(N, work)
#undef M8_CASE_work
    return 0;
}

int nbx_jk_m8_pack(nbx_ctx* ctx, int64_t N, int64_t nsrc, int64_t p0, int64_t p1, const double* d_eri, double* d_packed) {
    NBX_CHECK_ARG(nbx_jk_m8_covers(N) && d_eri && d_packed && nsrc <= N && nsrc > N - 4 && p1 <= nsrc);
    const int64_t ntiles = m4_tri((int)p1) - m4_tri((int)p0);
#define M8_CASE_pack(NB_)                                                                                                  \
    case NB_:                                                                                                              \
        hipLaunchKernelGGL((m8_pack_kernel<M8Geom<NB_, M8_LP(NB_)>>), dim3((unsigned)ntiles), dim3(256), 0, ctx->stream, d_eri, \
                           d_packed, (int)p0, (int64_t)m4_tri((int)p0), (int)nsrc);                                        \
        break;
    M8_DISPATCH(N, pack)
#undef M8_CASE_pack
    NBX_LAUNCH_CHECK();
    return NBX_OK;
}

size_t nbx_jk_m8_weights_bytes(int64_t N) {
#define M8_CASE_wbytes(NB_) \
    case NB_: return (size_t)(M8Geom<NB_, M8_LP(NB_)>::NCH * M8_LP(NB_) * M4_PROD_THREADS * 2) * sizeof(double);
    M8_DISPATCH(N, wbytes)
#undef M8_CASE_wbytes
    return 0;
}

void nbx_jk_m8_weight_layout(int64_t N, int out[4]) {
    out[0] = out[1] = out[2] = out[3] = 0;
#define M8_CASE_wl(NB_)                                   \
    case NB_: {                                           \
        using G = M8Geom<NB_, M8_LP(NB_)>;                 \
        if (G::NCH <= 4) {                                \
            out[0] = G::row0(1);                          \
            out[1] = G::row0(2);                          \
            out[2] = G::row0(3);                          \
            out[3] = G::LP;                               \
        }                                                 \
        break;                                            \
    }
    M8_DISPATCH(N, wl)
#undef M8_CASE_wl
}

int nbx_jk_m8(nbx_ctx* ctx, int64_t N, int64_t p0, int64_t p1, const double* d_packed, const double* d_dm, int64_t ndm,
              double* d_jk, void* d_work, const double* d_hv, double* d_fock, double* d_vhf, const double* d_wt) {
    NBX_CHECK_ARG(nbx_jk_m8_covers(N));
#define M8_CASE_run(NB_) \
    case NB_: return m8_run<NB_, M8_LP(NB_)>(ctx, p0, p1, d_packed, d_dm, ndm, d_jk, d_work, d_hv, d_fock, d_vhf, d_wt);
    M8_DISPATCH(N, run)
#undef M8_CASE_run
    return NBX_E_UNSUPPORTED;
}
```

### nbed_amd/csrc/nbx_common.h

```cpp
#pragma once

#include <hip/hip_runtime.h>

#include <cstdarg>
#include <cstdint>
#include <cstdio>
#include <cstring>
#include <vector>

#include "nbx.h"

constexpr int NBX_PROF_SLOTS = 8;
constexpr int NBX_PROF_MAX_EVENTS = 4096;

struct nbx_prof_slot {
    std::vector<hipEvent_t> start, stop;
    double ms_sum = 0.0;
    int64_t count = 0;
    int64_t seen = 0;
};

struct nbx_ctx {
    int device;
    hipStream_t stream;
    bool own_stream;
    double* d_scratch;
    double* h_pinned;
    int* d_counters;
    bool profiling = false;
    unsigned prof_mask = ~0u;
    int prof_every = 1;
    nbx_prof_slot prof[NBX_PROF_SLOTS];
};

bool nbx_eigh_lds_supported(int64_t n);
size_t nbx_eigh_lds_worksize(int64_t n, int64_t batch);
int nbx_eigh_lds(nbx_ctx* ctx, int64_t n, int64_t batch, const double* d_a, const double* d_v0, double* d_w,
                 double* d_v, void* d_work, size_t work_bytes, int refine_iters, const int* d_skip = nullptr);
const int* nbx_eigh_lds_status_ptr(int64_t n, int64_t batch, const void* d_work);
size_t nbx_eigh_lds_status_offset(int64_t n, int64_t batch);
int* nbx_eigh_lds_skip_ptr(int64_t n, int64_t batch, void* d_work);
int nbx_apply_rotation_log_t(nbx_ctx* ctx, int n, int np_even, int steps, const void* d_rot, const int* d_flags,
                             const int* d_nsteps, const int* d_rank, double* d_vt);

int nbx_jk_dense_sym_fock(nbx_ctx* ctx, int64_t nao, const double* d_eri, const double* d_dm, const double* d_hv, double* d_jk,
                          double* d_fock, double* d_vhf, void* d_work, size_t work_bytes);

int nbx_gemm_q1_synth(nbx_ctx* ctx, int64_t m, int64_t n, int64_t k, const double* d_a, int64_t lda, uint64_t seed,
                      double scale, int64_t r, int64_t s0, double* d_y, int64_t ldy, int64_t stride_y, int64_t batch);
bool nbx_gemm_small_supported(int64_t m, int64_t n, int64_t k, int64_t batch);
int nbx_gemm_pair_scatter(nbx_ctx* ctx, int64_t pair_n, int64_t m, int64_t n, int64_t k, const double* d_a, int64_t lda,
                          const double* d_b, int64_t ldb, int64_t stride_b, double* d_c);
int nbx_gemm_tri(nbx_ctx* ctx, int64_t unit, int64_t tri_m0, int64_t nbatch, int64_t n, int64_t k, const double* d_a,
                 int64_t lda, int64_t stride_a, const double* d_b, int64_t ldb, double* d_c, int64_t ldc,
                 int64_t a_symn = 0);
int nbx_gemm_gated(nbx_ctx* ctx, char trans_a, char trans_b, int64_t m, int64_t n, int64_t k, double alpha,
                   const double* d_a, int64_t lda, int64_t stride_a, const double* d_b, int64_t ldb, int64_t stride_b,
                   double beta, double* d_c, int64_t ldc, int64_t stride_c, int64_t batch, const int* d_gate,
                   int gate_a, int gate_b);
int nbx_gemm_small_gated(nbx_ctx* ctx, char trans_a, char trans_b, int64_t m, int64_t n, int64_t k, double alpha,
                         const double* d_a, int64_t lda, int64_t stride_a, const double* d_b, int64_t ldb,
                         int64_t stride_b, double beta, double* d_c, int64_t ldc, int64_t stride_c, int64_t batch,
                         const int* d_gate, int gate_a, int gate_b, const double* d_b2 = nullptr,
                         double* d_c2 = nullptr, double* d_norm_part = nullptr);
inline int64_t nbx_gemm_small_norm_doubles(int64_t m, int64_t n, int64_t batch) {
    return batch * 2 * ((m + 15) / 16) * ((n + 15) / 16) * 2;
}

int nbx_density_scalars_launch(nbx_ctx* ctx, int64_t nao, const double* d_hcore, int hcore_ndim, const double* d_vemb,
                               const double* d_vhf, const double* d_hz, const double* d_c, int64_t nocc_a, int64_t nocc_b,
                               double* d_dm_out, const double* d_dm_old, double* d_out, const int* d_tail, int64_t tail_n,
                               double* d_dts);
int nbx_diis_update_anti(nbx_ctx* ctx, int64_t n, int64_t space, int64_t slot, int64_t nd, const double* d_x,
                         const double* d_err, int64_t anti_n, double* d_xprev, double* d_xs, double* d_es, double* d_h,
                         double* d_coef);
int nbx_cycle_scalars_launch(nbx_ctx* ctx, int64_t nao, const double* d_hcore, int hcore_ndim, const double* d_vemb,
                             const double* d_vhf, const double* d_hz, const double* d_dm, const double* d_dm_old,
                             double* d_out, const int* d_tail, int64_t tail_n, double* d_dts, const double* d_dtail,
                             int64_t dtail_n);
int nbx_antisym(nbx_ctx* ctx, int64_t nao, int64_t batch, const double* d_a, double* d_out);

bool nbx_jk_sym_supported(int64_t nao);
int nbx_jk_sym_reduce(nbx_ctx* ctx, const double* k1, const double* k2, double* d_k, int64_t N, int64_t p0, int64_t np,
                      int64_t ndm, int64_t t_begin, int L, int S, const double* d_j = nullptr,
                      const double* d_hv = nullptr, double* d_fock = nullptr, double* d_vhf = nullptr,
                      int k2_tile_order = 0, int k_lower = 0);

bool nbx_eigh_refine_supported(int64_t n, int64_t batch);
size_t nbx_eigh_refine_worksize(int64_t n, int64_t batch);
int nbx_eigh_refine(nbx_ctx* ctx, int64_t n, int64_t batch, const double* d_a, const double* d_v0, double* d_w,
                    double* d_v, void* d_work, int* d_jacobi_status, const int** d_status_out, int max_iter);
constexpr int NBX_EIGH_REFINE_ITERS = 3;
constexpr int NBX_EIGH_REFINE_MAX = 6;

size_t nbx_eigh_tridiag_worksize(int64_t n, int64_t batch);
int nbx_eigh_tridiag(nbx_ctx* ctx, int64_t n, int64_t batch, const double* d_a, double* d_w, double* d_v,
                     void* d_work, size_t work_bytes, double* h_quality);
int nbx_eigh_tridiag_dev(nbx_ctx* ctx, int64_t n, int64_t batch, const double* d_a, double* d_w, double* d_v,
                         void* d_work, size_t work_bytes, int* d_status, int* d_skip);

struct nbx_prof_scope {
    nbx_ctx* ctx;
    int slot;
    hipEvent_t stop = nullptr;
    nbx_prof_scope(nbx_ctx* c, int s) : ctx(c), slot(s) {
        if (!ctx->profiling || !((ctx->prof_mask >> slot) & 1u) ||
            (int)ctx->prof[slot].start.size() >= NBX_PROF_MAX_EVENTS)
            return;
        if (ctx->prof[slot].seen++ % ctx->prof_every != 0) return;
        hipEvent_t a, b;
        if (hipEventCreate(&a) != hipSuccess) return;
        if (hipEventCreate(&b) != hipSuccess) { (void)hipEventDestroy(a); return; }
        (void)hipEventRecord(a, ctx->stream);
        ctx->prof[slot].start.push_back(a);
        ctx->prof[slot].stop.push_back(b);
        stop = b;
    }
    ~nbx_prof_scope() {
        if (stop) (void)hipEventRecord(stop, ctx->stream);
    }
};

constexpr int NBX_SCRATCH_DOUBLES = 4096;
constexpr int NBX_COUNTERS = 1024;

void nbx_set_error(const char* fmt, ...);

#define NBX_CHECK_ARG(cond)                                                     \
    do {                                                                        \
        if (!(cond)) {                                                          \
            nbx_set_error("%s: invalid argument: %s", __func__, #cond);         \
            return NBX_E_INVALID;                                               \
        }                                                                       \
    } while (0)

#define NBX_HIP(call)                                                           \
    do {                                                                        \
        hipError_t e_ = (call);                                                 \
        if (e_ != hipSuccess) {                                                 \
            nbx_set_error("%s: %s -> %s", __func__, #call, hipGetErrorString(e_)); \
            return NBX_E_HIP;                                                   \
        }                                                                       \
    } while (0)

#define NBX_LAUNCH_CHECK() NBX_HIP(hipGetLastError())

static inline int64_t nbx_cdiv(int64_t a, int64_t b) { return (a + b - 1) / b; }

__device__ __forceinline__ double nbx_wave_sum(double v) {
#pragma unroll
    for (int off = 32; off > 0; off >>= 1) v += __shfl_xor(v, off, 64);
    return v;
}

template <int CTRL>
__device__ __forceinline__ double nbx_dpp_f64(double v) {
    const int lo = __builtin_amdgcn_update_dpp(0, __double2loint(v), CTRL, 0xf, 0xf, false);
    const int hi = __builtin_amdgcn_update_dpp(0, __double2hiint(v), CTRL, 0xf, 0xf, false);
    return __hiloint2double(hi, lo);
}
constexpr int NBX_DPP_XOR1 = 0xB1, NBX_DPP_XOR2 = 0x4E, NBX_DPP_HALF_MIRROR = 0x141, NBX_DPP_MIRROR = 0x140;

__device__ __forceinline__ double nbx_readlane_f64(double v, int l) {
    return __hiloint2double(__builtin_amdgcn_readlane(__double2hiint(v), l),
                            __builtin_amdgcn_readlane(__double2loint(v), l));
}

__device__ __forceinline__ double nbx_sum8_dpp(double v) {
    v += nbx_dpp_f64<NBX_DPP_XOR1>(v);
    v += nbx_dpp_f64<NBX_DPP_XOR2>(v);
    v += nbx_dpp_f64<NBX_DPP_HALF_MIRROR>(v);
    return v;
}

__device__ __forceinline__ double nbx_wave_sum_dpp(double v) {
    v = nbx_sum8_dpp(v);
    v += nbx_dpp_f64<NBX_DPP_MIRROR>(v);
    return (nbx_readlane_f64(v, 0) + nbx_readlane_f64(v, 16)) + (nbx_readlane_f64(v, 32) + nbx_readlane_f64(v, 48));
}

__device__ __forceinline__ double nbx_wave_min_dpp(double v) {
    v = fmin(v, nbx_dpp_f64<NBX_DPP_XOR1>(v));
    v = fmin(v, nbx_dpp_f64<NBX_DPP_XOR2>(v));
    v = fmin(v, nbx_dpp_f64<NBX_DPP_HALF_MIRROR>(v));
    v = fmin(v, nbx_dpp_f64<NBX_DPP_MIRROR>(v));
    return fmin(fmin(nbx_readlane_f64(v, 0), nbx_readlane_f64(v, 16)),
                fmin(nbx_readlane_f64(v, 32), nbx_readlane_f64(v, 48)));
}

__device__ __forceinline__ double nbx_block_sum(double v, double* smem) {
    const int lane = threadIdx.x & 63;
    const int wave = threadIdx.x >> 6;
    const int nwave = (blockDim.x + 63) >> 6;
    v = nbx_wave_sum(v);
    __syncthreads();
    if (lane == 0) smem[wave] = v;
    __syncthreads();
    if (threadIdx.x == 0) {
        double t = 0.0;
        for (int w = 0; w < nwave; ++w) t += smem[w];
        smem[16] = t;
    }
    __syncthreads();
    return smem[16];
}
```

### nbed_amd/csrc/scf_cycle.hip

```cpp
#include <cstdlib>

#include "nbx_common.h"

static int huz_jk_slab(nbx_ctx* ctx, const nbx_huz_state* st, const double* d_dm_in, int64_t p0, int64_t p1) {
    const int64_t N = st->nao;
    if (st->jk_kind == NBX_HUZ_JK_PACKED) {
        NBX_CHECK_ARG(st->d_packed || p0 == p1);
        return nbx_jk_packed(ctx, N, p0, p1, st->d_packed, d_dm_in, 2, st->d_jk, st->d_jk_work, st->jk_work_bytes);
    }
    NBX_CHECK_ARG(st->jk_kind == NBX_HUZ_JK_SYM);
    NBX_CHECK_ARG(st->d_eri || p0 == p1);
    return nbx_jk_dense_sym(ctx, N, p0, p1, st->d_eri, d_dm_in, 2, st->d_jk, st->d_jk_work, st->jk_work_bytes);
}

static bool huz_whole_tensor(const nbx_huz_state* st) { return st->jk_p0 == 0 && st->jk_p1 == st->nao; }

static int huz_cycle_rest(nbx_ctx* ctx, const nbx_huz_state* st, const double* d_dm_in, const double* d_c_in,
                          double* d_dm_out, double* d_c_out, double* d_v_out, double* d_w_out, double* d_hz_out,
                          int mode, int refine_iters, int diis_mode, int diis_slot, int diis_nd, double* h_out,
                          int* d_status_out);

static int cycle_density(nbx_ctx* ctx, int64_t N, int64_t nocc_a, int64_t nocc_b, const double* d_c, double* d_dm) {
    const int64_t n2 = N * N;
    int rc = NBX_OK;
    if (nocc_a == nocc_b && nocc_a > 0)
        return nbx_gemm(ctx, 'N', 'T', N, N, nocc_a, 1.0, d_c, N, n2, d_c, N, n2, 0.0, d_dm, N, n2, 2);
    const int64_t nocc[2] = {nocc_a, nocc_b};
    for (int x = 0; x < 2; ++x) {
        if (nocc[x] > 0) {
            rc = nbx_gemm(ctx, 'N', 'T', N, N, nocc[x], 1.0, d_c + x * n2, N, 0, d_c + x * n2, N, 0, 0.0, d_dm + x * n2,
                          N, 0, 1);
        } else {
            rc = nbx_memset(ctx, d_dm + x * n2, 0, (size_t)n2 * sizeof(double));
        }
        if (rc != NBX_OK) return rc;
    }
    return rc;
}

extern "C" int nbx_huz_cycle_jk(nbx_ctx* ctx, const nbx_huz_state* st, const double* d_dm_in) {
    NBX_CHECK_ARG(ctx && st && d_dm_in);
    NBX_CHECK_ARG(st->nao > 0 && st->d_jk && st->d_jk_work);
    const int64_t p0 = st->jk_p0, p1 = st->jk_p1;
    NBX_CHECK_ARG(p0 >= 0 && p0 <= p1 && p1 <= st->nao);
    return huz_jk_slab(ctx, st, d_dm_in, p0, p1);
}

extern "C" int nbx_huz_cycle_post(nbx_ctx* ctx, const nbx_huz_state* st, const double* d_dm_in, const double* d_c_in,
                                  double* d_dm_out, double* d_c_out, double* d_v_out, double* d_w_out, double* d_hz_out,
                                  int mode, int refine_iters, int diis_mode, int diis_slot, int diis_nd, double* h_out,
                                  int* d_status_out) {
    NBX_CHECK_ARG(ctx && st && d_dm_in && d_dm_out && d_c_out && d_w_out && d_hz_out && h_out);
    NBX_CHECK_ARG(st->nao > 0 && st->d_hv && st->d_ds && st->d_jk && st->d_fock && st->d_vhf && st->d_fock2);
    int rc = nbx_fock_uhf(ctx, st->nao, st->d_hv, 3, nullptr, st->d_jk, st->d_fock, st->d_vhf);
    if (rc != NBX_OK) return rc;
    return huz_cycle_rest(ctx, st, d_dm_in, d_c_in, d_dm_out, d_c_out, d_v_out, d_w_out, d_hz_out, mode, refine_iters,
                          diis_mode, diis_slot, diis_nd, h_out, d_status_out);
}

extern "C" int nbx_huz_cycle(nbx_ctx* ctx, const nbx_huz_state* st, const double* d_dm_in, const double* d_c_in,
                             double* d_dm_out, double* d_c_out, double* d_v_out, double* d_w_out, double* d_hz_out,
                             int mode, int refine_iters, int diis_mode, int diis_slot, int diis_nd, int dts_ready,
                             double* h_out, int* d_status_out) {
    NBX_CHECK_ARG(ctx && st && d_dm_in && d_dm_out && d_c_out && d_w_out && d_hz_out && h_out);
    NBX_CHECK_ARG(st->nao > 0 && st->d_hv && st->d_ds && st->d_jk && st->d_fock && st->d_vhf && st->d_fock2 &&
                  st->d_jk_work);
    const int64_t N = st->nao;
    int rc;

    if (st->jk_kind == NBX_HUZ_JK_PACKED && huz_whole_tensor(st)) {
        NBX_CHECK_ARG(st->d_packed);
        rc = nbx_jk_packed_fock(ctx, N, st->d_packed, d_dm_in, st->d_hv, st->d_jk, st->d_fock, st->d_vhf, st->d_jk_work,
                                st->jk_work_bytes, (dts_ready && st->d_dts) ? st->d_dts : nullptr);
        if (rc != NBX_OK) return rc;
    } else {
        rc = NBX_E_UNSUPPORTED;
        if (st->jk_kind == NBX_HUZ_JK_SYM && huz_whole_tensor(st) && st->d_eri)
            rc = nbx_jk_dense_sym_fock(ctx, N, st->d_eri, d_dm_in, st->d_hv, st->d_jk, st->d_fock, st->d_vhf, st->d_jk_work,
                                       st->jk_work_bytes);
        if (rc == NBX_E_UNSUPPORTED) {
            rc = nbx_huz_cycle_jk(ctx, st, d_dm_in);
            if (rc != NBX_OK) return rc;
            rc = nbx_fock_uhf(ctx, N, st->d_hv, 3, nullptr, st->d_jk, st->d_fock, st->d_vhf);
        }
        if (rc != NBX_OK) return rc;
    }
    return huz_cycle_rest(ctx, st, d_dm_in, d_c_in, d_dm_out, d_c_out, d_v_out, d_w_out, d_hz_out, mode, refine_iters,
                          diis_mode, diis_slot, diis_nd, h_out, d_status_out);
}

static int huz_cycle_rest(nbx_ctx* ctx, const nbx_huz_state* st, const double* d_dm_in, const double* d_c_in,
                          double* d_dm_out, double* d_c_out, double* d_v_out, double* d_w_out, double* d_hz_out,
                          int mode, int refine_iters, int diis_mode, int diis_slot, int diis_nd, double* h_out,
                          int* d_status_out) {
    NBX_CHECK_ARG(mode == 0 || mode == 1 || mode == 2);
    NBX_CHECK_ARG(diis_mode >= 0 && diis_mode <= 2);
    const int64_t N = st->nao, n2 = N * N;
    int rc;
    rc = nbx_huzinaga_fused(ctx, N, 2, st->d_fock, st->d_ds, 1.0, d_hz_out, st->d_fock2);
    if (rc != NBX_OK) return rc;

    const double* f_use = st->d_fock2;
    if (diis_mode == 1) {
        NBX_CHECK_ARG(st->d_diis_xprev);
        rc = nbx_memcpy_d2d(ctx, st->d_diis_xprev, st->d_fock2, (size_t)(2 * n2) * sizeof(double));
        if (rc != NBX_OK) return rc;
    } else if (diis_mode == 2) {
        NBX_CHECK_ARG(st->d_diis_xprev && st->d_diis_xs && st->d_diis_es && st->d_diis_h && st->d_diis_coef);
        rc = nbx_diis_update(ctx, 2 * n2, st->diis_space, diis_slot, diis_nd, st->d_fock2, st->d_diis_xprev,
                             st->d_diis_xs, st->d_diis_es, st->d_diis_h, st->d_diis_coef);
        if (rc != NBX_OK) return rc;
        f_use = st->d_diis_xprev;
    }

    const int* d_status = nullptr;
    if (mode == 2) {
        NBX_CHECK_ARG(st->d_x && st->d_eig_work && st->d_tmp && st->d_fo && d_status_out);
        NBX_CHECK_ARG(st->eig_work_bytes >= nbx_purify_worksize(N, 2));
        double* fo = d_v_out ? d_v_out : st->d_fo;
        rc = nbx_gemm(ctx, 'N', 'N', N, N, N, 1.0, st->d_x, N, 0, f_use, N, n2, 0.0, st->d_tmp, N, n2, 2);
        if (rc != NBX_OK) return rc;
        rc = nbx_gemm(ctx, 'N', 'N', N, N, N, 1.0, st->d_tmp, N, n2, st->d_x, N, 0, 0.0, fo, N, n2, 2);
        if (rc != NBX_OK) return rc;
        rc = nbx_purify(ctx, N, 2, fo, st->nocc_a, st->nocc_b, st->d_tmp, st->d_eig_work, st->eig_work_bytes,
                        refine_iters, d_status_out);
        if (rc != NBX_OK) return rc;
        rc = nbx_gemm(ctx, 'N', 'N', N, N, N, 1.0, st->d_x, N, 0, st->d_tmp, N, n2, 0.0, st->d_fo, N, n2, 2);
        if (rc != NBX_OK) return rc;
        rc = nbx_gemm(ctx, 'N', 'N', N, N, N, 1.0, st->d_fo, N, n2, st->d_x, N, 0, 0.0, d_dm_out, N, n2, 2);
        if (rc != NBX_OK) return rc;
        return nbx_huz_cycle_scalars_dts(ctx, N, st->d_hv, 3, nullptr, st->d_vhf, d_hz_out, d_dm_out, d_dm_in, h_out,
                                         d_status_out, 2, st->d_dts);
    }
    if (mode == 1) {
        NBX_CHECK_ARG(d_c_in && st->d_sb && st->d_geig_work && d_status_out);
        rc = nbx_geig_refine(ctx, N, 2, f_use, st->d_sb, d_c_in, d_w_out, d_c_out, d_status_out, st->d_geig_work,
                             st->geig_work_bytes, refine_iters);
        if (rc != NBX_OK) return rc;
        d_status = d_status_out;
    } else {
        NBX_CHECK_ARG(st->d_x && st->d_eig_work && st->d_tmp && st->d_fo && d_v_out);
        rc = nbx_gemm(ctx, 'N', 'N', N, N, N, 1.0, st->d_x, N, 0, f_use, N, n2, 0.0, st->d_tmp, N, n2, 2);
        if (rc != NBX_OK) return rc;
        rc = nbx_gemm(ctx, 'N', 'N', N, N, N, 1.0, st->d_tmp, N, n2, st->d_x, N, 0, 0.0, st->d_fo, N, n2, 2);
        if (rc != NBX_OK) return rc;
        rc = nbx_eigh_warm_ex(ctx, N, 2, st->d_fo, d_c_in, d_w_out, d_v_out, st->d_eig_work, st->eig_work_bytes,
                              refine_iters);
        if (rc != NBX_OK) return rc;
        rc = nbx_gemm(ctx, 'N', 'N', N, N, N, 1.0, st->d_x, N, 0, d_v_out, N, n2, 0.0, d_c_out, N, n2, 2);
        if (rc != NBX_OK) return rc;
        d_status = reinterpret_cast<const int*>(static_cast<const char*>(st->d_eig_work) +
                                                nbx_eigh_status_offset(N, 2));
    }

    static const bool fused_density = getenv("NBX_FUSED_DENSITY") == nullptr || atoi(getenv("NBX_FUSED_DENSITY")) != 0;
    if (fused_density) {
        rc = nbx_density_scalars_launch(ctx, N, st->d_hv, 3, nullptr, st->d_vhf, d_hz_out, d_c_out, st->nocc_a, st->nocc_b,
                                        d_dm_out, d_dm_in, h_out, d_status, 2, st->d_dts);
        if (rc != NBX_E_UNSUPPORTED) return rc;
    }
    rc = cycle_density(ctx, N, st->nocc_a, st->nocc_b, d_c_out, d_dm_out);
    if (rc != NBX_OK) return rc;
    return nbx_huz_cycle_scalars_dts(ctx, N, st->d_hv, 3, nullptr, st->d_vhf, d_hz_out, d_dm_out, d_dm_in, h_out,
                                     d_status, 2, st->d_dts);
}


extern "C" int nbx_mu_cycle_solve(nbx_ctx* ctx, const nbx_huz_state* st, const double* d_dm_in, const double* d_fock_in,
                                  const double* d_c_in, double* d_dm_out, double* d_c_out, double* d_v_out,
                                  double* d_w_out, int mode, int refine_iters, int diis_on, int diis_slot, int diis_nd,
                                  int* d_status_out) {
    NBX_CHECK_ARG(ctx && st && d_dm_in && d_fock_in && d_dm_out && d_c_out && d_w_out);
    NBX_CHECK_ARG(st->nao > 0 && st->d_sb && st->d_tmp && st->d_fo && st->d_fock2);
    NBX_CHECK_ARG(mode == 0 || mode == 1);
    const int64_t N = st->nao, n2 = N * N;
    int rc;
    const double* f_use = d_fock_in;
    if (diis_on) {
        NBX_CHECK_ARG(st->d_diis_xprev && st->d_diis_xs && st->d_diis_es && st->d_diis_h && st->d_diis_coef);
        rc = nbx_gemm(ctx, 'N', 'N', N, N, N, 1.0, st->d_sb, N, 0, d_dm_in, N, n2, 0.0, st->d_tmp, N, n2, 2);
        if (rc != NBX_OK) return rc;
        rc = nbx_gemm(ctx, 'N', 'N', N, N, N, 1.0, st->d_tmp, N, n2, d_fock_in, N, n2, 0.0, st->d_fo, N, n2, 2);
// ... 103 lines not shown
```

Measured before the change: 4404.

## Fuse Huzinaga projection into JK finish and add single-kernel refine update

Adds a fused m8 JK path whose finish kernel also applies the Huzinaga projection, so the cycle skips the separate huzinaga_fused launch. Adds a refine_update kernel that computes the correction matrix and applies it through an MFMA f64 product in one launch when a single refine iteration is requested. Also adds a one-wave DIIS Jacobi variant that uses wave barriers instead of block syncs, and a DIIS update using an antisymmetric error. The aim is fewer kernel launches and fewer full-matrix round trips per SCF cycle, at the cost of more specialised code paths and extra workspace.

```diff
diff --git a/include/nbx.h b/include/nbx.h
--- a/include/nbx.h
+++ b/include/nbx.h
@@ -116,6 +116,9 @@
 int nbx_diis_update_err(nbx_ctx* ctx, int64_t n, int64_t space, int64_t slot, int64_t nd,
                         const double* d_x, const double* d_err, double* d_xprev, double* d_xs,
                         double* d_es, double* d_h, double* d_coef);
+int nbx_diis_update_anti(nbx_ctx* ctx, int64_t n, int64_t space, int64_t slot, int64_t nd,
+                         const double* d_x, const double* d_err, int64_t anti_n, double* d_xprev,
+                         double* d_xs, double* d_es, double* d_h, double* d_coef);
 int nbx_vo_sumsq(nbx_ctx* ctx, int64_t nao, const double* d_fmo, int64_t nocc_a, int64_t nocc_b,
                  double* d_out);
 int nbx_axpby(nbx_ctx* ctx, int64_t n, double a, const double* d_x, double b, double* d_y);
diff --git a/nbed_amd/_nbx.py b/nbed_amd/_nbx.py
--- a/nbed_amd/_nbx.py
+++ b/nbed_amd/_nbx.py
@@ -105,6 +105,7 @@
     "nbx_diis_coef_doubles": (c_size_t, [c_int64]),
     "nbx_diis_update": (c_int, [_P, c_int64, c_int64, c_int64, c_int64, _P, _P, _P, _P, _P, _P]),
     "nbx_diis_update_err": (c_int, [_P, c_int64, c_int64, c_int64, c_int64, _P, _P, _P, _P, _P, _P, _P]),
+    "nbx_diis_update_anti": (c_int, [_P, c_int64, c_int64, c_int64, c_int64, _P, _P, c_int64, _P, _P, _P, _P, _P]),
     "nbx_vo_sumsq": (c_int, [_P, c_int64, _P, c_int64, c_int64, _P]),
     "nbx_axpby": (c_int, [_P, c_int64, c_double, _P, c_double, _P]),
     "nbx_lincomb": (c_int, [_P, c_int64, c_int64, POINTER(c_double), _P, c_int64, _P]),
diff --git a/nbed_amd/backend.py b/nbed_amd/backend.py
--- a/nbed_amd/backend.py
+++ b/nbed_amd/backend.py
@@ -766,6 +766,11 @@
 
     def diis_update_err(self, space: int, slot: int, nd: int, x, err, out, xs, es, h, coef):
         self._call("nbx_diis_update_err", x.numel(), space, slot, nd, self._p(x), self._p(err), self._p(out),
+                   self._p(xs), self._p(es), self._p(h), self._p(coef))
+        return out
+
+    def diis_update_anti(self, space: int, slot: int, nd: int, x, a, out, xs, es, h, coef):
+        self._call("nbx_diis_update_anti", x.numel(), space, slot, nd, self._p(x), self._p(a), a.shape[-1], self._p(out),
                    self._p(xs), self._p(es), self._p(h), self._p(coef))
         return out
 
diff --git a/nbed_amd/csrc/ctx.hip b/nbed_amd/csrc/ctx.hip
--- a/nbed_amd/csrc/ctx.hip
+++ b/nbed_amd/csrc/ctx.hip
@@ -58,6 +58,8 @@
     }
     nbx_ctx* c = new nbx_ctx();
     c->device = device;
+    if (hipDeviceGetAttribute(&c->compute_units, hipDeviceAttributeMultiprocessorCount, device) != hipSuccess)
+        c->compute_units = 0;
     c->own_stream = (private_stream != 0);
     if (c->own_stream) {
         hipError_t e = hipStreamCreateWithFlags(&c->stream, hipStreamNonBlocking);
diff --git a/nbed_amd/csrc/eigh_refine.hip b/nbed_amd/csrc/eigh_refine.hip
--- a/nbed_amd/csrc/eigh_refine.hip
+++ b/nbed_amd/csrc/eigh_refine.hip
@@ -17,6 +17,46 @@
 }
 __device__ __forceinline__ double peek(const double* p) {
     return __hip_atomic_load(p, __ATOMIC_RELAXED, __HIP_MEMORY_SCOPE_AGENT);
+}
+
+struct refine_e_elem {
+    double ep, e_abs, c_abs, n_abs;
+};
+__device__ __forceinline__ refine_e_elem refine_e_element(int i, int j, double s_ij, double s_ji, double g,
+                                                          const double* lam, double om_s, double om_r) {
+    const double sx = 0.5 * (s_ij + s_ji);
+    refine_e_elem o;
+    o.c_abs = o.n_abs = 0.0;
+    if (i == j) {
+        const double ev = 0.5 * (1.0 - g);
+        o.e_abs = fabs(ev);
+        o.ep = 1.0 + ev;
+        return o;
+    }
+    const double li = lam[i], lj = lam[j];
+    const double d = lj - li;
+    double ev;
+    if (fabs(d) > om_s + fmax(fabs(li), fabs(lj)) * om_r) {
+        const double num = sx - lj * g;
+        ev = num / d;
+        o.n_abs = fabs(num);
+    } else {
+        ev = -0.5 * g;
+        o.c_abs = fabs(sx);
+    }
+    o.e_abs = fabs(ev);
+    o.ep = ev;
+    return o;
+}
+
+__device__ __forceinline__ int refine_verdict(double emax, double cmax, double nmax, int N, double na, int iter,
+                                              int max_iter) {
+    const bool at_noise = nmax <= RF_NOISE * sqrt((double)N) * na && emax < 1.0e-3;
+    int st = 0;
+    if (!(emax < RF_GIVE_UP)) st = -1;
+    else if ((emax < RF_TOL || at_noise) && cmax <= RF_CLUSTER_NOISE * na) st = iter + 1;
+    else if (iter == max_iter - 1) st = -1;
+    return st;
 }
 
 __global__ __launch_bounds__(RF_THREADS) void refine_e_kernel(int N, const double* __restrict__ A,
@@ -168,26 +208,11 @@
             const int e = e0 + u * stride;
             if (e < total) {
                 const int i = ri[u], j = e - i * N;
-                const double sx = 0.5 * (sv[u] + st[u]), g = gv[u];
-                double ev;
-                if (i == j) {
-                    ev = 0.5 * (1.0 - g);
-                    emax = fmax(emax, fabs(ev));
-                    Ep[e] = 1.0 + ev;
-                } else {
-                    const double li = lam[i], lj = lam[j];
-                    const double d = lj - li;
-                    if (fabs(d) > om_s + fmax(fabs(li), fabs(lj)) * om_r) {
-                        const double num = sx - lj * g;
-                        ev = num / d;
-                        nmax = fmax(nmax, fabs(num));
-                    } else {
-                        ev = -0.5 * g;
-                        cmax = fmax(cmax, fabs(sx));
-                    }
-                    emax = fmax(emax, fabs(ev));
-                    Ep[e] = ev;
-                }
+                const refine_e_elem el = refine_e_element(i, j, sv[u], st[u], gv[u], lam, om_s, om_r);
+                Ep[e] = el.ep;
+                emax = fmax(emax, el.e_abs);
+                cmax = fmax(cmax, el.c_abs);
+                nmax = fmax(nmax, el.n_abs);
             }
         }
     }
@@ -218,11 +243,7 @@
                 cmax = fmax(cmax, peek(part + w * RF_PART + 4));
                 nmax = fmax(nmax, peek(part + w * RF_PART + 5));
             }
-            const bool at_noise = nmax <= RF_NOISE * sqrt((double)N) * na && emax < 1.0e-3;
-            int st = 0;
-            if (!(emax < RF_GIVE_UP)) st = -1;
-            else if ((emax < RF_TOL || at_noise) && cmax <= RF_CLUSTER_NOISE * na) st = iter + 1;
-            else if (iter == max_iter - 1) st = -1;
+            int st = refine_verdict(emax, cmax, nmax, N, na, iter, max_iter);
             if (final_status != nullptr) {
                 if (st > 0 && unsorted) st = -3;
                 final_status[b] = st > 0 ? 1000 + st : (st < 0 ? st : -2);
@@ -233,6 +254,162 @@
     }
     if (wg == 0)
         for (int i = threadIdx.x; i < N; i += RF_THREADS) lam_out[(int64_t)b * N + i] = lam[i];
+}
+
+constexpr int RU_MAX_N = 256;
+constexpr int RU_WAVES = RF_THREADS / 64;
+typedef double rf_v4f64 __attribute__((ext_vector_type(4)));
+__global__ __launch_bounds__(RF_THREADS) void refine_update_kernel(int N, const double* __restrict__ X,
+                                                                   const double* __restrict__ S,
+                                                                   const double* __restrict__ G, double* __restrict__ Xout,
+                                                                   double* __restrict__ lam_out, int* __restrict__ status,
+                                                                   int* __restrict__ final_status,
+                                                                   double* __restrict__ partial, int* __restrict__ counters,
+                                                                   const double* __restrict__ norm_part, int norm_tiles) {
+    __shared__ double lam[RU_MAX_N];
+    __shared__ double Es[RU_MAX_N * 16];
+    __shared__ double red[3 * RU_WAVES];
+    const int b = blockIdx.z, tid = threadIdx.x, wave = tid >> 6, lane = tid & 63, fr = lane & 15, fk = lane >> 4;
+    const int64_t n2 = (int64_t)N * N;
+    X += b * n2;
+    S += b * n2;
+    G += b * n2;
+    Xout += b * n2;
+    const int kpad = (N + 15) & ~15;
+    const int ic = tid < N ? tid : N - 1;
+    const double sd = S[(int64_t)ic * N + ic], gd = G[(int64_t)ic * N + ic];
+    const double* ps = norm_part + (int64_t)b * 2 * norm_tiles * 2;
+    const double* pg = ps + (int64_t)norm_tiles * 2;
+    const int wc = tid < norm_tiles ? tid : norm_tiles - 1;
+    const double po = ps[2 * wc], pa = ps[2 * wc + 1], pr = pg[2 * wc];
+    const int ec = tid & 15, ek = tid >> 4;
+    const int col_e = blockIdx.x * 16 + ec;
+    const bool e_ok = col_e < N;
+    const int je = e_ok ? col_e : 0;
+    double sv[RU_MAX_N / 16], st[RU_MAX_N / 16], gv[RU_MAX_N / 16];
+#pragma unroll
+    for (int m = 0; m < RU_MAX_N / 16; ++m) {
+        if (16 * m < kpad) {
+            const int k = ek + 16 * m, kc = k < N ? k : N - 1;
+            sv[m] = S[(int64_t)kc * N + je];
+            st[m] = S[(int64_t)je * N + kc];
+            gv[m] = G[(int64_t)kc * N + je];
+        }
+    }
+    const int trow = blockIdx.y * RU_WAVES + wave;
+    const bool tile = trow * 16 < N;
+    const int row_a = trow * 16 + fr;
+    const bool a_ok = row_a < N;
+    const double* ap = X + (int64_t)(a_ok ? row_a : 0) * N;
+    double a[RU_MAX_N / 4];
+#pragma unroll
+    for (int j = 0; j < RU_MAX_N / 4; ++j) {
+        if (tile && 4 * j < kpad) {
+            const int k = 4 * j + fk;
+            a[j] = ap[k < N ? k : N - 1];
+        }
+    }
+    lam[tid] = sd / gd;
+    {
+        const bool in = tid < norm_tiles;
+        const double o = nbx_wave_sum_dpp(in ? 0.0 + po : 0.0), r = nbx_wave_sum_dpp(in ? 0.0 + pr : 0.0),
+                     q = nbx_wave_sum_dpp(in ? 0.0 + pa : 0.0);
+        if (lane == 0) {
+            red[wave] = o;
+            red[RU_WAVES + wave] = r;
+            red[2 * RU_WAVES + wave] = q;
+        }
+    }
+    __syncthreads();
+    double off2 = 0.0, r2 = 0.0, a2 = 0.0;
+#pragma unroll
+    for (int w = 0; w < RU_WAVES; ++w) {
+        off2 += red[w];
+        r2 += red[RU_WAVES + w];
+        a2 += red[2 * RU_WAVES + w];
+    }
+    const double na = sqrt(a2);
+    const double om_s = 2.0 * sqrt(off2), om_r = 2.0 * sqrt(r2);
+    double emax = 0.0, cmax = 0.0, nmax = 0.0;
+#pragma unroll
+    for (int m = 0; m < RU_MAX_N / 16; ++m) {
+        if (16 * m < kpad) {
+            const int k = ek + 16 * m;
+            double ev = 0.0;
+            if (k < N && e_ok) {
+                const refine_e_elem el = refine_e_element(k, je, sv[m], st[m], gv[m], lam, om_s, om_r);
+                ev = el.ep;
+                emax = fmax(emax, el.e_abs);
+                cmax = fmax(cmax, el.c_abs);
+                nmax = fmax(nmax, el.n_abs);
+            }
+            Es[k * 16 + ec] = ev;
+        }
+    }
+    __syncthreads();
+    if (tile) {
+        rf_v4f64 acc = (rf_v4f64){0.0, 0.0, 0.0, 0.0};
+#pragma unroll
+        for (int j = 0; j < RU_MAX_N / 4; ++j) {
+            if (4 * j < kpad) {
+                const int k = 4 * j + fk;
+                acc = __builtin_amdgcn_mfma_f64_16x16x4f64((k < N && a_ok) ? a[j] : 0.0, Es[k * 16 + fr], acc, 0, 0, 0);
+            }
+        }
+        const int col_b = blockIdx.x * 16 + fr;
+        if (col_b < N) {
+#pragma unroll
+            for (int r = 0; r < 4; ++r) {
+                const int row = trow * 16 + fk + 4 * r;
+                if (row < N) Xout[(int64_t)row * N + col_b] = acc[r];
+            }
+        }
+    }
+    if (blockIdx.y != 0) return;
+    emax = -nbx_wave_min_dpp(-emax);
+    cmax = -nbx_wave_min_dpp(-cmax);
+    nmax = -nbx_wave_min_dpp(-nmax);
+    if (lane == 0) {
+        red[wave] = emax;
+        red[RU_WAVES + wave] = cmax;
+        red[2 * RU_WAVES + wave] = nmax;
+    }
+    __syncthreads();
+    if (wave != 0) return;
+#pragma unroll
+    for (int w = 0; w < RU_WAVES; ++w) {
+        emax = fmax(emax, red[w]);
+        cmax = fmax(cmax, red[RU_WAVES + w]);
+        nmax = fmax(nmax, red[2 * RU_WAVES + w]);
+    }
+    if (blockIdx.x == 0)
+        for (int i = lane; i < N; i += 64) lam_out[(int64_t)b * N + i] = lam[i];
+    const int ncol = gridDim.x;
+    double* part = partial + (int64_t)b * RF_WGS * RF_PART;
+    int* counter = counters + b;
+    int last = 0;
+    if (lane == 0) {
+        publish(part + 3 * blockIdx.x + 0, emax);
+        publish(part + 3 * blockIdx.x + 1, cmax);
+        publish(part + 3 * blockIdx.x + 2, nmax);
+        last = __hip_atomic_fetch_add(counter, 1, __ATOMIC_ACQ_REL, __HIP_MEMORY_SCOPE_AGENT) == ncol - 1 ? 1 : 0;
+    }
+    if (!__builtin_amdgcn_readfirstlane(last)) return;
+    int unsorted = 0;
+    for (int i = lane + 1; i < N; i += 64) unsorted |= lam[i - 1] > lam[i] ? 1 : 0;
+    unsorted = __any(unsorted);
+    if (lane == 0) {
+        for (int w = 0; w < ncol; ++w) {
+            emax = fmax(emax, peek(part + 3 * w + 0));
+            cmax = fmax(cmax, peek(part + 3 * w + 1));
+            nmax = fmax(nmax, peek(part + 3 * w + 2));
+        }
+        int st = refine_verdict(emax, cmax, nmax, N, na, 0, 1);
+        if (st > 0 && unsorted) st = -3;
+        final_status[b] = st > 0 ? 1000 + st : (st < 0 ? st : -2);
+        status[b] = st;
+        __hip_atomic_store(counter, 0, __ATOMIC_RELEASE, __HIP_MEMORY_SCOPE_AGENT);
+    }
 }
 
 constexpr int RF_ROWS = 8;
@@ -309,7 +486,7 @@
 }
 
 bool nbx_eigh_refine_supported(int64_t n, int64_t batch) {
-    return n >= 2 && n <= 4096 && batch <= NBX_COUNTERS;
+    return n >= 2 && n <= 4096 && batch <= NBX_COUNTERS_BATCH;
 }
 
 size_t nbx_eigh_refine_worksize(int64_t n, int64_t batch) { return rlayout(n, batch).total; }
@@ -398,7 +575,7 @@
                                const double* d_c0, double* d_w, double* d_c, int* d_status, void* d_work,
                                size_t work_bytes, int max_iter) {
     NBX_CHECK_ARG(ctx && d_f && d_s && d_c0 && d_w && d_c && d_status);
-    NBX_CHECK_ARG(n >= 2 && n <= 4096 && batch >= 1 && batch <= NBX_COUNTERS);
+    NBX_CHECK_ARG(n >= 2 && n <= 4096 && batch >= 1 && batch <= NBX_COUNTERS_BATCH);
     NBX_CHECK_ARG(max_iter >= 1 && max_iter <= RF_MAX_ITER);
     const GeigLayout L = glayout(n, batch);
     if (d_work == nullptr || work_bytes < L.total) {
@@ -421,6 +598,20 @@
     const int64_t n2 = n * n;
     const bool pair = nbx_gemm_small_supported(n, n, n, 2 * batch);
     const bool direct = max_iter == 1 && d_c != d_c0;
+    if (direct && pair && n <= RU_MAX_N) {
+        int rc = nbx_gemm_small_gated(ctx, 'T', 'N', n, n, n, 1.0, d_c0, n, n2, d_f, n, n2, 0.0, yt, n, n2, batch, nullptr,
+                                      0, 0, d_s, zt);
+        if (rc != NBX_OK) return rc;
+        rc = nbx_gemm_small_gated(ctx, 'T', 'T', n, n, n, 1.0, d_c0, n, n2, yt, n, n2, 0.0, s, n, n2, batch, nullptr, 0, 0,
+                                  zt, g, npart);
+        if (rc != NBX_OK) return rc;
+        hipLaunchKernelGGL(refine_update_kernel,
+                           dim3((unsigned)nbx_cdiv(n, 16), (unsigned)nbx_cdiv(n, 16 * RU_WAVES), (unsigned)batch),
+                           dim3(RF_THREADS), 0, ctx->stream, (int)n, d_c0, s, g, d_c, d_w, status, d_status, partial,
+                           ctx->d_counters, npart, norm_tiles);
+        NBX_LAUNCH_CHECK();
+        return NBX_OK;
+    }
     for (int it = 0; it < max_iter; ++it) {
         const double* src = (it == 0) ? d_c0 : cb[it & 1];
         double* dst = direct ? d_c : cb[(it + 1) & 1];
diff --git a/nbed_amd/csrc/elementwise.hip b/nbed_amd/csrc/elementwise.hip
--- a/nbed_amd/csrc/elementwise.hip
+++ b/nbed_amd/csrc/elementwise.hip
@@ -734,6 +734,16 @@
     sn = rot ? t * y : 0.0;
 }
 
+template <bool ONE_WAVE>
+__device__ __forceinline__ void diis8_sync() {
+    if constexpr (ONE_WAVE) {
+        __syncthreads();
+    } else {
+        __builtin_amdgcn_fence(__ATOMIC_ACQ_REL, "wavefront");
+        __builtin_amdgcn_wave_barrier();
+    }
+}
+template <bool ONE_WAVE>
 __device__ __forceinline__ void diis_jacobi8(double& a, double& v, int m, double fro, int lane, double* As,
                                              double* Vs) {
     const int r = lane >> 3, c = lane & 7;
@@ -753,12 +763,12 @@
             const int mc = mate(c), mr = mate(r);
             As[lane] = a;
             Vs[lane] = v;
-            __syncthreads();
+            diis8_sync<ONE_WAVE>();
             const double a_cc = As[9 * c], a_mm = As[9 * mc], a_cm = As[8 * min(c, mc) + max(c, mc)];
             const double a_rr = As[9 * r], a_nn = As[9 * mr], a_rn = As[8 * min(r, mr) + max(r, mr)];
             const double a_rmc = As[8 * r + mc], a_mrc = As[8 * mr + c], a_mrmc = As[8 * mr + mc];
             const double v_rmc = Vs[8 * r + mc];
-            __syncthreads();
+            diis8_sync<ONE_WAVE>();
             double cc, sc, cr, sr;
             diis_rotation(c < mc ? a_cc : a_mm, c < mc ? a_mm : a_cc, a_cm, cc, sc);
             diis_rotation(r < mr ? a_rr : a_nn, r < mr ? a_nn : a_rr, a_rn, cr, sr);
@@ -771,6 +781,149 @@
     }
 }
 
+struct diis8_lds {
+    double As[64], Vs[64], Ts[64];
+    double A0[8][9], rhs_s[8], c_out[8];
+    int lu_failed;
+};
+template <bool ONE_WAVE>
+__device__ __forceinline__ double diis8_partial(const double* p) {
+    if constexpr (ONE_WAVE) return *p;
+    else return __hip_atomic_load(p, __ATOMIC_RELAXED, __HIP_MEMORY_SCOPE_AGENT);
+}
+
+template <bool ONE_WAVE>
+__device__ __forceinline__ void diis_solve8(const double* partial, int nblocks, int nd, int slot, double* H, int ldh,
+                                            double* coef, double* state_out, double hold, double v_prev, bool warm,
+                                            bool store, diis8_lds& L) {
+    const int lane = threadIdx.x & 63, r = lane >> 3, c = lane & 7;
+    const int m = nd + 1;
+    const bool inside = r < m && c < m;
+    const bool new_row = inside && r == slot + 1 && c >= 1, new_col = inside && c == slot + 1 && r >= 1;
+    double acc = 0.0;
+    if (c >= 1 && c <= nd) {
+#pragma unroll 4
+        for (int b = r; b < nblocks; b += 8) acc += diis8_partial<ONE_WAVE>(partial + (int64_t)b * nd + c - 1);
+    }
+    L.As[lane] = acc;
+    diis8_sync<ONE_WAVE>();
+    double row_c = 0.0, row_r = 0.0;
+#pragma unroll
+    for (int g = 0; g < 8; ++g) {
+        row_c += L.As[8 * g + c];
+        row_r += L.As[8 * g + r];
+    }
+    diis8_sync<ONE_WAVE>();
+    double a = new_row ? row_c : (new_col ? row_r : hold);
+    if (store && (new_row || new_col)) H[(int64_t)r * ldh + c] = a;
+    L.A0[r][c] = a;
+    if (lane == 0) L.lu_failed = 0;
+    double v = (r == c) ? 1.0 : 0.0;
+    if (warm) {
+        L.Vs[lane] = v_prev;
+        diis8_sync<ONE_WAVE>();
+        double gram = 0.0;
+#pragma unroll
+        for (int k = 0; k < 8; ++k) gram = fma(L.Vs[8 * k + r], L.Vs[8 * k + c], gram);
+        L.Ts[lane] = gram;
+        diis8_sync<ONE_WAVE>();
+        double vg = 0.0;
+#pragma unroll
+        for (int k = 0; k < 8; ++k) vg = fma(L.Vs[8 * r + k], L.Ts[8 * k + c], vg);
+        v = 1.5 * v_prev - 0.5 * vg;
+        diis8_sync<ONE_WAVE>();
+        L.Vs[lane] = v;
+        L.As[lane] = a;
+        diis8_sync<ONE_WAVE>();
+        double hv = 0.0;
+#pragma unroll
+        for (int k = 0; k < 8; ++k) hv = fma(L.As[8 * r + k], L.Vs[8 * k + c], hv);
+        L.Ts[lane] = hv;
+        diis8_sync<ONE_WAVE>();
+        double vhv = 0.0;
+#pragma unroll
+        for (int k = 0; k < 8; ++k) vhv = fma(L.Vs[8 * k + r], L.Ts[8 * k + c], vhv);
+        diis8_sync<ONE_WAVE>();
+        L.Ts[lane] = vhv;
+        diis8_sync<ONE_WAVE>();
+        a = 0.5 * (vhv + L.Ts[8 * c + r]);
+        diis8_sync<ONE_WAVE>();
+    }
+    const double fro = nbx_wave_sum_dpp(a * a);
+    diis_jacobi8<ONE_WAVE>(a, v, m, fro, lane, L.As, L.Vs);
+    L.As[lane] = a;
+    L.Vs[lane] = v;
+    if (store) {
+        state_out[lane] = v;
+        if (lane == 0) state_out[64] = __longlong_as_double(DIIS_STATE_MAGIC);
+        if (lane == 1) state_out[65] = (double)m;
+    }
+    diis8_sync<ONE_WAVE>();
+    const bool singular = __any(r == c && r < m && fabs(a) < 1e-14);
+    if (!singular) {
+        if (lane < m) L.rhs_s[lane] = (lane == 0) ? 1.0 : 0.0;
+        diis8_sync<ONE_WAVE>();
+        for (int k = 0; k < m; ++k) {
+            double best = (lane >= k && lane < m) ? fabs(L.A0[lane][k]) : -1.0;
+            int piv = lane;
+#pragma unroll
+            for (int o = 4; o > 0; o >>= 1) {
+                const double ob = __shfl_xor(best, o);
+                const int op = __shfl_xor(piv, o);
+                if (ob > best || (ob == best && op < piv)) {
+                    best = ob;
+                    piv = op;
+                }
+            }
+            best = nbx_readlane_f64(best, 0);
+            piv = __builtin_amdgcn_readlane(piv, 0);
+            if (best == 0.0) {
+                if (lane == 0) L.lu_failed = 1;
+                break;
+            }
+            if (piv != k) {
+                if (lane < m) {
+                    const double tmp = L.A0[k][lane];
+                    L.A0[k][lane] = L.A0[piv][lane];
+                    L.A0[piv][lane] = tmp;
+                }
+                if (lane == 0) {
+                    const double tmp = L.rhs_s[k];
+                    L.rhs_s[k] = L.rhs_s[piv];
+                    L.rhs_s[piv] = tmp;
+                }
+            }
+            diis8_sync<ONE_WAVE>();
+            const double inv = 1.0 / L.A0[k][k];
+            const bool below = r > k && r < m, right = c > k && c < m;
+            double upd = 0.0, rupd = 0.0;
+            if (below && right) upd = L.A0[r][c] - (L.A0[r][k] * inv) * L.A0[k][c];
+            if (below && c == 0) rupd = L.rhs_s[r] - (L.A0[r][k] * inv) * L.rhs_s[k];
+            diis8_sync<ONE_WAVE>();
+            if (below && right) L.A0[r][c] = upd;
+            if (below && c == 0) L.rhs_s[r] = rupd;
+            diis8_sync<ONE_WAVE>();
+        }
+        diis8_sync<ONE_WAVE>();
+        if (!L.lu_failed) {
+            for (int i = m - 1; i >= 0; --i) {
+                const double t = nbx_wave_sum_dpp((lane > i && lane < m) ? L.A0[i][lane] * L.c_out[lane] : 0.0);
+                if (lane == 0) L.c_out[i] = (L.rhs_s[i] - t) / L.A0[i][i];
+                diis8_sync<ONE_WAVE>();
+            }
+        }
+        diis8_sync<ONE_WAVE>();
+    }
+    if (singular || L.lu_failed) {
+        const double w = L.As[9 * c], v0 = L.Vs[c];
+        const bool keep = c < m && (!singular || fabs(w) > 1e-14);
+        const double t = nbx_sum8_dpp(keep ? v * (1.0 / w) * v0 : 0.0);
+        if (c == 0 && r < m) L.c_out[r] = t;
+        diis8_sync<ONE_WAVE>();
+    }
+    if (store && lane >= 1 && lane < m) coef[lane - 1] = L.c_out[lane];
+}
+
 constexpr int DIIS8_PER_LANE = 4;
 __global__ __launch_bounds__(64) void diis_solve8_lincomb_kernel(const double* __restrict__ partial, int nblocks,
                                                                  int nd, int slot, double* __restrict__ H, int ldh,
@@ -778,9 +931,7 @@
                                                                  double* __restrict__ state, int64_t n,
                                                                  const double* __restrict__ vecs, int64_t stride,
                                                                  double* __restrict__ out) {
-    __shared__ double As[64], Vs[64], Ts[64];
-    __shared__ double A0[8][9], rhs_s[8], c_out[8];
-    __shared__ int lu_failed;
+    __shared__ diis8_lds L;
     const int lane = threadIdx.x, r = lane >> 3, c = lane & 7;
     const int m = nd + 1;
     const int64_t i0 = (int64_t)blockIdx.x * (64 * DIIS8_PER_LANE) + lane;
@@ -794,131 +945,11 @@
         for (int k = 0; k < 7; ++k) xv[j][k] = (k < nd && i0 + 64 * j < n) ? vecs[k * stride + i0 + 64 * j] : 0.0;
     const double v_prev = state[lane];
     const bool warm = __double_as_longlong(state[64]) == DIIS_STATE_MAGIC && state[65] <= (double)(nd + 1);
-    double acc = 0.0;
-    if (c >= 1 && c <= nd) {
-#pragma unroll 4
-        for (int b = r; b < nblocks; b += 8) acc += partial[(int64_t)b * nd + c - 1];
-    }
-    As[lane] = acc;
-    __syncthreads();
-    double row_c = 0.0, row_r = 0.0;
-#pragma unroll
-    for (int g = 0; g < 8; ++g) {
-        row_c += As[8 * g + c];
-        row_r += As[8 * g + r];
-    }
-    __syncthreads();
-    double a = new_row ? row_c : (new_col ? row_r : hold);
-    if (blockIdx.x == 0 && (new_row || new_col)) H[(int64_t)r * ldh + c] = a;
-    A0[r][c] = a;
-    if (lane == 0) lu_failed = 0;
-    double v = (r == c) ? 1.0 : 0.0;
-    if (warm) {
-        Vs[lane] = v_prev;
-        __syncthreads();
-        double gram = 0.0;
-#pragma unroll
-        for (int k = 0; k < 8; ++k) gram = fma(Vs[8 * k + r], Vs[8 * k + c], gram);
-        Ts[lane] = gram;
-        __syncthreads();
-        double vg = 0.0;
-#pragma unroll
-        for (int k = 0; k < 8; ++k) vg = fma(Vs[8 * r + k], Ts[8 * k + c], vg);
-        v = 1.5 * v_prev - 0.5 * vg;
-        __syncthreads();
-        Vs[lane] = v;
-        As[lane] = a;
-        __syncthreads();
-        double hv = 0.0;
-#pragma unroll
-        for (int k = 0; k < 8; ++k) hv = fma(As[8 * r + k], Vs[8 * k + c], hv);
-        Ts[lane] = hv;
-        __syncthreads();
-        double vhv = 0.0;
-#pragma unroll
-        for (int k = 0; k < 8; ++k) vhv = fma(Vs[8 * k + r], Ts[8 * k + c], vhv);
-        __syncthreads();
-        Ts[lane] = vhv;
-        __syncthreads();
-        a = 0.5 * (vhv + Ts[8 * c + r]);
-        __syncthreads();
-    }
-    const double fro = nbx_wave_sum_dpp(a * a);
-    diis_jacobi8(a, v, m, fro, lane, As, Vs);
-    As[lane] = a;
-    Vs[lane] = v;
-    if (blockIdx.x == 0) {
-        state[DIIS_STATE_HALF + lane] = v;
-        if (lane == 0) state[DIIS_STATE_HALF + 64] = __longlong_as_double(DIIS_STATE_MAGIC);
-        if (lane == 1) state[DIIS_STATE_HALF + 65] = (double)m;
-    }
-    __syncthreads();
-    const bool singular = __any(r == c && r < m && fabs(a) < 1e-14);
-    if (!singular) {
-        if (lane < m) rhs_s[lane] = (lane == 0) ? 1.0 : 0.0;
-        __syncthreads();
-        for (int k = 0; k < m; ++k) {
-            double best = (lane >= k && lane < m) ? fabs(A0[lane][k]) : -1.0;
-            int piv = lane;
-#pragma unroll
-            for (int o = 4; o > 0; o >>= 1) {
-                const double ob = __shfl_xor(best, o);
-                const int op = __shfl_xor(piv, o);
-                if (ob > best || (ob == best && op < piv)) {
-                    best = ob;
-                    piv = op;
-                }
-            }
-            best = nbx_readlane_f64(best, 0);
-            piv = __builtin_amdgcn_readlane(piv, 0);
-            if (best == 0.0) {
-                if (lane == 0) lu_failed = 1;
-                break;
-            }
-            if (piv != k) {
-                if (lane < m) {
-                    const double tmp = A0[k][lane];
-                    A0[k][lane] = A0[piv][lane];
-                    A0[piv][lane] = tmp;
-                }
-                if (lane == 0) {
-                    const double tmp = rhs_s[k];
-                    rhs_s[k] = rhs_s[piv];
-                    rhs_s[piv] = tmp;
-                }
-            }
-            __syncthreads();
-            const double inv = 1.0 / A0[k][k];
-            const bool below = r > k && r < m, right = c > k && c < m;
-            double upd = 0.0, rupd = 0.0;
-            if (below && right) upd = A0[r][c] - (A0[r][k] * inv) * A0[k][c];
-            if (below && c == 0) rupd = rhs_s[r] - (A0[r][k] * inv) * rhs_s[k];
-            __syncthreads();
-            if (below && right) A0[r][c] = upd;
-            if (below && c == 0) rhs_s[r] = rupd;
-            __syncthreads();
-        }
-        __syncthreads();
-        if (!lu_failed) {
-            for (int i = m - 1; i >= 0; --i) {
-                const double t = nbx_wave_sum_dpp((lane > i && lane < m) ? A0[i][lane] * c_out[lane] : 0.0);
-                if (lane == 0) c_out[i] = (rhs_s[i] - t) / A0[i][i];
-                __syncthreads();
-            }
-        }
-        __syncthreads();
-    }
-    if (singular || lu_failed) {
-        const double w = As[9 * c], v0 = Vs[c];
-        const bool keep = c < m && (!singular || fabs(w) > 1e-14);
-        const double t = nbx_sum8_dpp(keep ? v * (1.0 / w) * v0 : 0.0);
-        if (c == 0 && r < m) c_out[r] = t;
-        __syncthreads();
-    }
-    if (blockIdx.x == 0 && lane >= 1 && lane < m) coef[lane - 1] = c_out[lane];
+    diis_solve8<true>(partial, nblocks, nd, slot, H, ldh, coef, state + DIIS_STATE_HALF, hold, v_prev, warm,
+                      blockIdx.x == 0, L);
     double cf[7];
 #pragma unroll
-    for (int k = 0; k < 7; ++k) cf[k] = (k < nd) ? c_out[k + 1] : 0.0;
+    for (int k = 0; k < 7; ++k) cf[k] = (k < nd) ? L.c_out[k + 1] : 0.0;
 #pragma unroll
     for (int j = 0; j < DIIS8_PER_LANE; ++j) {
         const int64_t i = i0 + 64 * j;
@@ -928,6 +959,132 @@
             for (int k = 0; k < 7; ++k)
                 if (k < nd) t = fma(cf[k], xv[j][k], t);
             out[i] = t;
+        }
+    }
+}
+
+constexpr int DIIS_FUSED_BLOCKS = 128;
+constexpr int DIIS_FUSED_PER_THREAD = 4;
+constexpr int64_t DIIS_FUSED_MAX_N = (int64_t)DIIS_FUSED_BLOCKS * 256 * DIIS_FUSED_PER_THREAD;
+constexpr int DIIS_FUSED_SPINS = 1 << 20;
+__global__ __launch_bounds__(256) void diis_fused_kernel(int64_t n, int nd, int slot, const double* __restrict__ x,
+                                                         const double* err, double* xprev, double* xs, double* es,
+                                                         double* partial, double* H, int ldh, double* coef,
+                                                         double* state, int* counter, int anti_n) {
+    __shared__ double red[4][8];
+    __shared__ diis8_lds L;
+    const int tid = threadIdx.x, wave = tid >> 6, lane = tid & 63;
+    const int nblocks = gridDim.x;
+    int* arrived = counter;
+    int* departed = counter + 1;
+    const int64_t i0 = (int64_t)blockIdx.x * 256 + tid, step = (int64_t)nblocks * 256;
+    double xn[DIIS_FUSED_PER_THREAD], e0[DIIS_FUSED_PER_THREAD], e1[DIIS_FUSED_PER_THREAD];
+    double ek[DIIS_FUSED_PER_THREAD][7], xv[DIIS_FUSED_PER_THREAD][7];
+#pragma unroll
+    for (int j = 0; j < DIIS_FUSED_PER_THREAD; ++j) {
+        xn[j] = e0[j] = e1[j] = 0.0;
+#pragma unroll
+        for (int k = 0; k < 7; ++k) ek[j][k] = xv[j][k] = 0.0;
+        if (j * step < n) {
+            const int64_t i = i0 + j * step, ic = i < n ? i : n - 1;
+            xn[j] = x[ic];
+            if (anti_n > 0) {
+                const int64_t a2 = (int64_t)anti_n * anti_n, bb = ic / a2, rc = ic - bb * a2;
+                const int64_t r = rc / anti_n, c = rc - r * anti_n;
+                e0[j] = err[bb * a2 + c * anti_n + r];
+                e1[j] = err[ic];
+            } else {
+                e0[j] = (err != nullptr) ? err[ic] : xprev[ic];
+            }
+#pragma unroll
+            for (int k = 0; k < 7; ++k) {
+                if (k < nd && k != slot) {
+                    ek[j][k] = es[(int64_t)k * n + ic];
+                    xv[j][k] = xs[(int64_t)k * n + ic];
+                }
+            }
+        }
+    }
+    double acc[7];
+#pragma unroll
+    for (int k = 0; k < 7; ++k) acc[k] = 0.0;
+#pragma unroll
+    for (int j = 0; j < DIIS_FUSED_PER_THREAD; ++j) {
+        const int64_t i = i0 + j * step;
+        const bool in = i < n;
+        const double xvv = xn[j];
+        const double e = (anti_n > 0) ? e0[j] - e1[j] : ((err != nullptr) ? e0[j] : xvv - e0[j]);
+#pragma unroll
+        for (int k = 0; k < 7; ++k) {
+            if (k < nd) {
+                const double t = fma(e, (k == slot) ? e : ek[j][k], acc[k]);
+                acc[k] = in ? t : acc[k];
+            }
+            if (k == slot) xv[j][k] = xvv;
+        }
+        if (in) {
+            xs[(int64_t)slot * n + i] = xvv;
+            es[(int64_t)slot * n + i] = e;
+        }
+    }
+#pragma unroll
+    for (int k = 0; k < 7; ++k) {
+        if (k < nd) {
+            const double t = nbx_wave_sum_dpp(acc[k]);
+            if (lane == 0) red[wave][k] = t;
+        }
+    }
+    __syncthreads();
+    if (wave == 0) {
+        if (lane < nd)
+            __hip_atomic_store(partial + (int64_t)blockIdx.x * nd + lane,
+                               ((red[0][lane] + red[1][lane]) + red[2][lane]) + red[3][lane], __ATOMIC_RELAXED,
+                               __HIP_MEMORY_SCOPE_AGENT);
+        const int r = lane >> 3, c = lane & 7, m = nd + 1;
+        const bool inside = r < m && c < m;
+        const bool new_row = inside && r == slot + 1 && c >= 1, new_col = inside && c == slot + 1 && r >= 1;
+        const double hold = (inside && !new_row && !new_col) ? H[(int64_t)r * ldh + c] : 0.0;
+        const double* prev = state + DIIS_STATE_HALF;
+        const double v_prev = prev[lane];
+        const bool warm = __double_as_longlong(prev[64]) == DIIS_STATE_MAGIC && prev[65] <= (double)(nd + 1);
+        int spins = 0;
+        if (lane == 0) {
+            asm volatile("s_waitcnt vmcnt(0)" ::: "memory");
+            __hip_atomic_fetch_add(arrived, 1, __ATOMIC_RELAXED, __HIP_MEMORY_SCOPE_AGENT);
+            while (__hip_atomic_load(arrived, __ATOMIC_RELAXED, __HIP_MEMORY_SCOPE_AGENT) < nblocks &&
+                   ++spins < DIIS_FUSED_SPINS)
+                __builtin_amdgcn_s_sleep(2);
+        }
+        const bool expired = __builtin_amdgcn_readfirstlane(spins) >= DIIS_FUSED_SPINS;
+        asm volatile("" ::: "memory");
+        if (expired) {
+            if (lane < 8) L.c_out[lane] = __longlong_as_double(0x7ff8000000000000ll);
+            if (lane < nd) coef[lane] = __longlong_as_double(0x7ff8000000000000ll);
+        } else {
+            diis_solve8<false>(partial, nblocks, nd, slot, H, ldh, coef, state + DIIS_STATE_HALF, hold, v_prev, warm,
+                               blockIdx.x == 0, L);
+        }
+    }
+    __syncthreads();
+    double cf[7];
+#pragma unroll
+    for (int k = 0; k < 7; ++k) cf[k] = (k < nd) ? L.c_out[k + 1] : 0.0;
+#pragma unroll
+    for (int j = 0; j < DIIS_FUSED_PER_THREAD; ++j) {
+        const int64_t i = i0 + j * step;
+        if (i < n) {
+            double t = 0.0;
+#pragma unroll
+            for (int k = 0; k < 7; ++k)
+                if (k < nd) t = fma(cf[k], xv[j][k], t);
+            xprev[i] = t;
+        }
+    }
+    if (tid == 0) {
+        const int left = __hip_atomic_fetch_add(departed, 1, __ATOMIC_RELAXED, __HIP_MEMORY_SCOPE_AGENT);
+        if (left == nblocks - 1) {
+            __hip_atomic_store(arrived, 0, __ATOMIC_RELAXED, __HIP_MEMORY_SCOPE_AGENT);
+            __hip_atomic_store(departed, 0, __ATOMIC_RELAXED, __HIP_MEMORY_SCOPE_AGENT);
         }
     }
 }
@@ -1230,8 +1387,15 @@
     NBX_CHECK_ARG(anti_n == 0 || (d_err != nullptr && anti_n > 0 && n % (anti_n * anti_n) == 0));
     NBX_CHECK_ARG(space >= 1 && space <= DIIS_MAX_SPACE && slot >= 0 && slot < space && nd >= 1 && nd <= space &&
                   slot < nd);
-    const unsigned blocks = grid1d(n, 256, 128);
+    const unsigned blocks = grid1d(n, 256, DIIS_FUSED_BLOCKS);
     NBX_CHECK_ARG((int64_t)blocks * nd <= NBX_SCRATCH_DOUBLES - 64);
+    if (nd <= 7 && n <= DIIS_FUSED_MAX_N && (int)blocks <= ctx->compute_units) {
+        hipLaunchKernelGGL(diis_fused_kernel, dim3(blocks), dim3(256), 0, ctx->stream, n, (int)nd, (int)slot, d_x, d_err,
+                           d_xprev, d_xs, d_es, ctx->d_scratch, d_h, (int)(space + 1), d_coef, d_coef + space,
+                           ctx->d_counters + NBX_COUNTERS - 4, (int)anti_n);
+        NBX_LAUNCH_CHECK();
+        return NBX_OK;
+    }
     hipLaunchKernelGGL(diis_push_kernel, dim3(blocks), dim3(256), 0, ctx->stream, n, (int)nd, (int)slot, d_x,
                        d_xprev, d_err, d_xs, d_es, ctx->d_scratch, d_coef + space, (int)anti_n);
     NBX_LAUNCH_CHECK();
diff --git a/nbed_amd/csrc/jk_m8.hip b/nbed_amd/csrc/jk_m8.hip
--- a/nbed_amd/csrc/jk_m8.hip
+++ b/nbed_amd/csrc/jk_m8.hip
@@ -492,11 +492,125 @@
     jout[i] = j;
 }
 
+template <class G>
+struct M8Fock {
+    const double *kpf, *j2sum, *jhalf, *hv;
+    double j, k, v;
+    __device__ __forceinline__ double at(int r, int c) {
+        constexpr int N = G::N;
+        const int hi = r > c ? r : c, lo = r > c ? c : r;
+        j = jhalf[r * N + c] + j2sum[m8_stage_index<G>(hi, lo)];
+        k = kpf[r * N + c] + kpf[c * N + r];
+        v = j - k;
+        return hv[r * N + c] + v;
+    }
+};
+
+template <class G>
+__global__ __launch_bounds__(64) void m8_finish_huz_kernel(const double* __restrict__ kpf, const double* __restrict__ j2sum,
+                                                           const double* __restrict__ jhalf, const double* __restrict__ hvm,
+                                                           const double* __restrict__ DS, double kappa,
+                                                           double* __restrict__ jout, double* __restrict__ kout,
+                                                           double* __restrict__ fock, double* __restrict__ vhf,
+                                                           double* __restrict__ hz, double* __restrict__ fock_out) {
+    typedef double v4f64 __attribute__((ext_vector_type(4)));
+    constexpr int N = G::N, n2 = N * N;
+    __shared__ double t2[16][17], hvs[16][17];
+    const int ti = blockIdx.y, tj = blockIdx.x, x = blockIdx.z;
+    if (tj > ti) return;
+    DS += x * n2;
+    hz += x * n2;
+    fock_out += x * n2;
+    M8Fock<G> fe{kpf + x * n2, j2sum, jhalf, hvm + x * n2, 0.0, 0.0, 0.0};
+    const int lane = threadIdx.x, fr = lane & 15, fk = lane >> 4;
+    const int ri = ti * 16 + fr, rj = tj * 16 + fr;
+    const bool oki = ri < N, okj = rj < N;
+    const int ric = oki ? ri : 0, rjc = okj ? rj : 0;
+    const bool diag = ti == tj, owner = tj == 0;
+    double fo[4], fm[4];
+#pragma unroll
+    for (int r = 0; r < 4; ++r) {
+        const int row = min(ti * 16 + fk + 4 * r, N - 1), col = min(tj * 16 + fr, N - 1);
+        fo[r] = fe.at(row, col);
+        const int mrow = min(tj * 16 + fk + 4 * r, N - 1), mcol = min(ti * 16 + fr, N - 1);
+        fm[r] = fe.at(mrow, mcol);
+    }
+    v4f64 acc1 = {0.0, 0.0, 0.0, 0.0}, acc2 = {0.0, 0.0, 0.0, 0.0};
+    constexpr int FH_STEPS = 10;
+    for (int k0 = 0; k0 < N; k0 += 4 * FH_STEPS) {
+        double a1[FH_STEPS], b1[FH_STEPS], a2[FH_STEPS], b2[FH_STEPS], j1[FH_STEPS], k1[FH_STEPS], v1[FH_STEPS];
+#pragma unroll
+        for (int j = 0; j < FH_STEPS; ++j) {
+            const int k = k0 + 4 * j + fk;
+            const bool in = k < N;
+            const int kc = in ? k : N - 1;
+            const double f1 = fe.at(ric, kc);
+            j1[j] = fe.j;
+            k1[j] = fe.k;
+            v1[j] = fe.v;
+            const double f2 = fe.at(rjc, kc);
+            a1[j] = (in && oki) ? f1 : 0.0;
+            b1[j] = (in && okj) ? DS[kc * N + rjc] : 0.0;
+            a2[j] = (in && okj && !diag) ? f2 : 0.0;
+            b2[j] = (in && oki && !diag) ? DS[kc * N + ric] : 0.0;
+        }
+        if (owner) {
+#pragma unroll
+            for (int j = 0; j < FH_STEPS; ++j) {
+                const int k = k0 + 4 * j + fk;
+                if (k < N && oki) {
+                    const int o = ri * N + k;
+                    kout[x * n2 + o] = k1[j];
+                    fock[x * n2 + o] = a1[j];
+                    vhf[x * n2 + o] = v1[j];
+                    if (x == 0) jout[o] = j1[j];
+                }
+            }
+        }
+#pragma unroll
+        for (int j = 0; j < FH_STEPS; ++j) {
+            if (k0 + 4 * j < N) {
+                acc1 = __builtin_amdgcn_mfma_f64_16x16x4f64(a1[j], b1[j], acc1, 0, 0, 0);
+                if (!diag) acc2 = __builtin_amdgcn_mfma_f64_16x16x4f64(a2[j], b2[j], acc2, 0, 0, 0);
+            }
+        }
+    }
+    if (diag) acc2 = acc1;
+#pragma unroll
+    for (int r = 0; r < 4; ++r) t2[fk + 4 * r][fr] = acc2[r];
+    __syncthreads();
+    double val[4];
+#pragma unroll
+    for (int r = 0; r < 4; ++r) {
+        val[r] = -kappa * (acc1[r] + t2[fr][fk + 4 * r]);
+        hvs[fk + 4 * r][fr] = val[r];
+    }
+    __syncthreads();
+#pragma unroll
+    for (int r = 0; r < 4; ++r) {
+        const int row = ti * 16 + fk + 4 * r, col = tj * 16 + fr;
+        if (row < N && col < N) {
+            const int o = row * N + col;
+            hz[o] = val[r];
+            fock_out[o] = fo[r] + val[r];
+        }
+        if (!diag) {
+            const int mrow = tj * 16 + fk + 4 * r, mcol = ti * 16 + fr;
+            if (mrow < N && mcol < N) {
+                const int o = mrow * N + mcol;
+                const double v = hvs[fr][fk + 4 * r];
+                hz[o] = v;
+                fock_out[o] = fm[r] + v;
+            }
+        }
+    }
+}
+
 size_t m8_align256(size_t x) { return (x + 255) & ~(size_t)255; }
 
 struct M8Plan {
     int wgs, S, lmax;
-    size_t wt_off, k1_off, k2_off, jp_off, js_off, kpf_off, total, lds_bytes;
+    size_t wt_off, k1_off, k2_off, jp_off, js_off, kpf_off, jh_off, total, lds_bytes;
 };
 
 template <class G>
@@ -563,14 +677,17 @@
     pl.jp_off = off; off += m8_align256((size_t)pl.wgs * jlen * sizeof(double));
     pl.js_off = off; off += m8_align256(jlen * sizeof(double));
     pl.kpf_off = off; off += m8_align256((size_t)(ndm * G::N * G::N) * sizeof(double));
+    pl.jh_off = off; off += m8_align256((size_t)(G::N * G::N) * sizeof(double));
     pl.total = off;
     return pl;
 }
 
 template <int NB, int LP>
 int m8_run(nbx_ctx* ctx, int64_t p0, int64_t p1, const double* d_packed, const double* d_dm, int64_t ndm, double* d_jk,
-           void* d_work, const double* d_hv, double* d_fock, double* d_vhf, const double* d_wt_in) {
+           void* d_work, const double* d_hv, double* d_fock, double* d_vhf, const double* d_wt_in, const double* d_ds,
+           double kappa, double* d_hz, double* d_fock2) {
     using G = M8Geom<NB, LP>;
+    const bool huz = d_hz != nullptr;
     const int64_t np = p1 - p0, N = G::N, n2 = N * N;
     const M8Plan pl = m8_plan<G>(p0, np, ndm);
     int wgs_;
@@ -586,6 +703,7 @@
     double* jp = reinterpret_cast<double*>(base + pl.jp_off);
     double* js = reinterpret_cast<double*>(base + pl.js_off);
     double* kpf = reinterpret_cast<double*>(base + pl.kpf_off);
+    double* jfull = huz ? reinterpret_cast<double*>(base + pl.jh_off) : d_jk;
     if (np < N) {
         const int rc = nbx_memset(ctx, d_jk, 0, (size_t)n2 * sizeof(double));
         if (rc != NBX_OK) return rc;
@@ -615,10 +733,10 @@
         }
         if (ndm == 2)
             hipLaunchKernelGGL((jk_m8_kernel<NB, 2, LP>), dim3((unsigned)pl.wgs), dim3(M8_THREADS), pl.lds_bytes, ctx->stream,
-                               d_packed, d_dm, wt, d_jk, k1, k2, jp, t_begin, rg, pl.S);
+                               d_packed, d_dm, wt, jfull, k1, k2, jp, t_begin, rg, pl.S);
         else
             hipLaunchKernelGGL((jk_m8_kernel<NB, 1, LP>), dim3((unsigned)pl.wgs), dim3(M8_THREADS), pl.lds_bytes, ctx->stream,
-                               d_packed, d_dm, wt, d_jk, k1, k2, jp, t_begin, rg, pl.S);
+                               d_packed, d_dm, wt, jfull, k1, k2, jp, t_begin, rg, pl.S);
     }
     NBX_LAUNCH_CHECK();
     {
@@ -627,6 +745,13 @@
         hipLaunchKernelGGL(m8_reduce_kernel<G>, dim3((unsigned)(nkb + jblocks)), dim3(512), 0, ctx->stream, k1, k2, jp, kpf, js,
                            (int)p0, (int)np, (int)ndm, t_begin, rg, pl.wgs, pl.S);
         NBX_LAUNCH_CHECK();
+    }
+    if (huz) {
+        const unsigned g = (unsigned)nbx_cdiv(N, 16);
+        hipLaunchKernelGGL(m8_finish_huz_kernel<G>, dim3(g, g, 2), dim3(64), 0, ctx->stream, kpf, js, jfull, d_hv, d_ds, kappa, d_jk,
+                           d_jk + n2, d_fock, d_vhf, d_hz, d_fock2);
+        NBX_LAUNCH_CHECK();
+        return NBX_OK;
     }
     hipLaunchKernelGGL(m8_finish_kernel<G>, dim3((unsigned)nbx_cdiv(n2, 256)), dim3(256), 0, ctx->stream, kpf, js, d_jk, d_jk + n2,
                        (int)ndm, d_hv, d_fock, d_vhf);
@@ -717,8 +842,20 @@
               double* d_jk, void* d_work, const double* d_hv, double* d_fock, double* d_vhf, const double* d_wt) {
     NBX_CHECK_ARG(nbx_jk_m8_covers(N));
 #define M8_CASE_run(NB_) \
-    case NB_: return m8_run<NB_, M8_LP(NB_)>(ctx, p0, p1, d_packed, d_dm, ndm, d_jk, d_work, d_hv, d_fock, d_vhf, d_wt);
+    case NB_: return m8_run<NB_, M8_LP(NB_)>(ctx, p0, p1, d_packed, d_dm, ndm, d_jk, d_work, d_hv, d_fock, d_vhf, d_wt, nullptr, 0.0, nullptr, nullptr);
     M8_DISPATCH(N, run)
 #undef M8_CASE_run
     return NBX_E_UNSUPPORTED;
 }
+
+int nbx_jk_m8_huz(nbx_ctx* ctx, int64_t N, const double* d_packed, const double* d_dm, double* d_jk, void* d_work,
+                  const double* d_hv, double* d_fock, double* d_vhf, const double* d_wt, const double* d_ds, double kappa,
+                  double* d_hz, double* d_fock2) {
+    NBX_CHECK_ARG(nbx_jk_m8_covers(N));
+    NBX_CHECK_ARG(d_packed && d_dm && d_jk && d_work && d_hv && d_fock && d_vhf && d_ds && d_hz && d_fock2);
+#define M8_CASE_huz(NB_) \
+    case NB_: return m8_run<NB_, M8_LP(NB_)>(ctx, 0, N, d_packed, d_dm, 2, d_jk, d_work, d_hv, d_fock, d_vhf, d_wt, d_ds, kappa, d_hz, d_fock2);
+    M8_DISPATCH(N, huz)
+#undef M8_CASE_huz
+    return NBX_E_UNSUPPORTED;
+}
diff --git a/nbed_amd/csrc/nbx_common.h b/nbed_amd/csrc/nbx_common.h
--- a/nbed_amd/csrc/nbx_common.h
+++ b/nbed_amd/csrc/nbx_common.h
@@ -27,6 +27,7 @@
     double* d_scratch;
     double* h_pinned;
     int* d_counters;
+    int compute_units = 0;
     bool profiling = false;
     unsigned prof_mask = ~0u;
     int prof_every = 1;
@@ -67,13 +68,15 @@
     return batch * 2 * ((m + 15) / 16) * ((n + 15) / 16) * 2;
 }
 
+bool nbx_jk_m8_covers(int64_t N);
+int nbx_jk_m8_huz(nbx_ctx* ctx, int64_t N, const double* d_packed, const double* d_dm, double* d_jk, void* d_work,
+                  const double* d_hv, double* d_fock, double* d_vhf, const double* d_wt, const double* d_ds, double kappa,
+                  double* d_hz, double* d_fock2);
+
 int nbx_density_scalars_launch(nbx_ctx* ctx, int64_t nao, const double* d_hcore, int hcore_ndim, const double* d_vemb,
                                const double* d_vhf, const double* d_hz, const double* d_c, int64_t nocc_a, int64_t nocc_b,
                                double* d_dm_out, const double* d_dm_old, double* d_out, const int* d_tail, int64_t tail_n,
                                double* d_dts);
-int nbx_diis_update_anti(nbx_ctx* ctx, int64_t n, int64_t space, int64_t slot, int64_t nd, const double* d_x,
-                         const double* d_err, int64_t anti_n, double* d_xprev, double* d_xs, double* d_es, double* d_h,
-                         double* d_coef);
 int nbx_cycle_scalars_launch(nbx_ctx* ctx, int64_t nao, const double* d_hcore, int hcore_ndim, const double* d_vemb,
                              const double* d_vhf, const double* d_hz, const double* d_dm, const double* d_dm_old,
                              double* d_out, const int* d_tail, int64_t tail_n, double* d_dts, const double* d_dtail,
@@ -123,6 +126,7 @@
 
 constexpr int NBX_SCRATCH_DOUBLES = 4096;
 constexpr int NBX_COUNTERS = 1024;
+constexpr int NBX_COUNTERS_BATCH = NBX_COUNTERS - 4;
 
 void nbx_set_error(const char* fmt, ...);
 
diff --git a/nbed_amd/csrc/scf_cycle.hip b/nbed_amd/csrc/scf_cycle.hip
--- a/nbed_amd/csrc/scf_cycle.hip
+++ b/nbed_amd/csrc/scf_cycle.hip
@@ -18,7 +18,7 @@
 static int huz_cycle_rest(nbx_ctx* ctx, const nbx_huz_state* st, const double* d_dm_in, const double* d_c_in,
                           double* d_dm_out, double* d_c_out, double* d_v_out, double* d_w_out, double* d_hz_out,
                           int mode, int refine_iters, int diis_mode, int diis_slot, int diis_nd, double* h_out,
-                          int* d_status_out);
+                          int* d_status_out, bool hz_done = false);
 
 static int cycle_density(nbx_ctx* ctx, int64_t N, int64_t nocc_a, int64_t nocc_b, const double* d_c, double* d_dm) {
     const int64_t n2 = N * N;
@@ -68,6 +68,20 @@
     const int64_t N = st->nao;
     int rc;
 
+    if (st->jk_kind == NBX_HUZ_JK_PACKED && huz_whole_tensor(st) && nbx_jk_m8_covers(N)) {
+        NBX_CHECK_ARG(st->d_packed && d_hz_out != st->d_fock && st->d_fock2 != st->d_fock);
+        NBX_CHECK_ARG((reinterpret_cast<uintptr_t>(st->d_packed) & 15) == 0 && (reinterpret_cast<uintptr_t>(st->d_jk_work) & 15) == 0);
+        const size_t need = nbx_jk_packed_worksize(N, 0, N, 2);
+        if (st->jk_work_bytes < need) {
+            nbx_set_error("nbx_huz_cycle: workspace %zu < %zu bytes", (size_t)st->jk_work_bytes, need);
+            return NBX_E_NOMEM;
+        }
+        rc = nbx_jk_m8_huz(ctx, N, st->d_packed, d_dm_in, st->d_jk, st->d_jk_work, st->d_hv, st->d_fock, st->d_vhf,
+                           (dts_ready && st->d_dts) ? st->d_dts : nullptr, st->d_ds, 1.0, d_hz_out, st->d_fock2);
+        if (rc != NBX_OK) return rc;
+        return huz_cycle_rest(ctx, st, d_dm_in, d_c_in, d_dm_out, d_c_out, d_v_out, d_w_out, d_hz_out, mode, refine_iters,
+                              diis_mode, diis_slot, diis_nd, h_out, d_status_out, true);
+    }
     if (st->jk_kind == NBX_HUZ_JK_PACKED && huz_whole_tensor(st)) {
         NBX_CHECK_ARG(st->d_packed);
         rc = nbx_jk_packed_fock(ctx, N, st->d_packed, d_dm_in, st->d_hv, st->d_jk, st->d_fock, st->d_vhf, st->d_jk_work,
@@ -92,12 +106,12 @@
 static int huz_cycle_rest(nbx_ctx* ctx, const nbx_huz_state* st, const double* d_dm_in, const double* d_c_in,
                           double* d_dm_out, double* d_c_out, double* d_v_out, double* d_w_out, double* d_hz_out,
                           int mode, int refine_iters, int diis_mode, int diis_slot, int diis_nd, double* h_out,
-                          int* d_status_out) {
+                          int* d_status_out, bool hz_done) {
     NBX_CHECK_ARG(mode == 0 || mode == 1 || mode == 2);
     NBX_CHECK_ARG(diis_mode >= 0 && diis_mode <= 2);
     const int64_t N = st->nao, n2 = N * N;
     int rc;
-    rc = nbx_huzinaga_fused(ctx, N, 2, st->d_fock, st->d_ds, 1.0, d_hz_out, st->d_fock2);
+    rc = hz_done ? NBX_OK : nbx_huzinaga_fused(ctx, N, 2, st->d_fock, st->d_ds, 1.0, d_hz_out, st->d_fock2);
     if (rc != NBX_OK) return rc;
 
     const double* f_use = st->d_fock2;
```

Result: no change. 4416 (median of 6 runs) (+0.3%).
